# picoexperiment/AutoBub3hs

Hardware: AMD Instinct MI355X
Metric: frames/s end-to-end detect @1280x1024 8-bit (higher is better)
Workload: dtype u8

## Files before the change

### autobub3hs_amd/_lib.py

```python
import ctypes as C
import os
import subprocess

HERE = os.path.dirname(os.path.abspath(__file__))
SO = os.path.join(HERE, "libabub_hip.so")
HEADER = os.path.join(os.path.dirname(HERE), "include", "abub_hip.h")


class Job(C.Structure):
    _fields_ = [("cur", C.c_uint32), ("ref", C.c_uint32), ("model", C.c_uint32), ("out", C.c_uint32)]


class TrigSeg(C.Structure):
    _fields_ = [("hist", C.c_void_p), ("pending", C.c_void_p), ("first", C.c_int32), ("count", C.c_int32)]


class TrigStack(C.Structure):
    _fields_ = [("seg0", C.c_uint32), ("nseg", C.c_uint32), ("F", C.c_int32), ("start", C.c_int32), ("tss", C.c_int32),
                ("first_bad", C.c_int32)]


def build(force=False):
    srcs = [os.path.join(HERE, "csrc", f) for f in os.listdir(os.path.join(HERE, "csrc"))
            if f.endswith((".hip", ".h", ".hpp")) or f == "Makefile"] + [HEADER]
    stale = force or not os.path.exists(SO) or any(os.path.getmtime(s) > os.path.getmtime(SO) for s in srcs)
    if stale:
        subprocess.check_call(["make", "-C", os.path.join(HERE, "csrc"), "-s"])
    return SO


_vp, _i, _sz = C.c_void_p, C.c_int, C.c_size_t
SIGNATURES = {
    "abub_last_error": (C.c_char_p, []),
    "abub_device_count": (_i, []),
    "abub_device_info": (_i, [_i, C.c_char_p, _i, C.POINTER(_i), C.POINTER(C.c_uint64)]),
    "abub_sigma6_dev": (_i, [_vp, _vp, _sz, _vp]),
    "abub_fill_stack_jobs_dev": (_i, [_vp, _i, _i, _i, _i, _i, _i, _vp]),
    "abub_diff_hist_dev": (_i, [_vp, _vp, _vp, _i, _i, _i, _vp, _vp, _i, _vp]),
    "abub_diff_roi_dev": (_i, [_vp, _vp, _vp, _i, _i, _i, _i, _i, _i, _vp, _vp, _vp]),
    "abub_train_dev": (_i, [_vp, _vp, _i, _i, _i, _vp, _vp, _vp]),
    "abub_pair_hist_dev": (_i, [_vp, _vp, _i, _i, _i, _vp, _vp]),
    "abub_posttrig_dev": (_i, [_vp, _vp, _vp, _vp, _i, _i, _i, _vp, _vp, _vp]),
    "abub_fg_compact_dev": (_i, [_vp, _i, _i, _i, _vp, _vp, _i, _vp, _vp]),
    "abub_fast_path": (_i, [_i]),
    "abub_scratch_release": (_i, [_vp]),
    "abub_bound_counts_dev": (_i, [_vp, C.POINTER(C.c_uint32)]),
    "abub_diff_hist_chained_dev": (_i, [_vp, _vp, _vp, _i, _i, _i, _vp, _i, _i, _vp]),
    "abub_diff_hist_chained_store_dev": (_i, [_vp, _vp, _vp, _i, _i, _i, _vp, _vp, _i, _i, _vp]),
    "abub_k2_set_option": (_i, [C.c_char_p, _i]),
    "abub_k2_deferred_ok": (_i, [_i, _i]),
    "abub_k3_set_option": (_i, [C.c_char_p, _i]),
    "abub_k2_pieces_cap": (_sz, [_i, _i, _i]),
    "abub_png_raw_stride": (_sz, [_i, _i]),
    "abub_png_decode_dev": (_i, [_vp, _sz, _vp, _i, _vp, _i, _vp, _i, _i, _i, _vp, _sz, _vp, _sz, _vp, _sz, _vp, _vp]),
    "abub_diff_hist_chained_deferred_dev": (_i, [_vp, _vp, _vp, _i, _i, _i, _vp, _i, _i, _vp, C.c_uint32, _vp, _vp, _vp]),
    "abub_diff_hist_pieces_dev": (_i, [_vp, _vp, _vp, _i, _i, _i, _vp, _vp, _vp, _vp, _vp]),
    "abub_diff_hist_compact_dev": (_i, [_vp, _vp, _vp, _i, _i, _i, _vp, _vp, _vp, _vp, C.c_uint32, _vp, C.c_uint32, _vp]),
    "abub_posttrig_compact_dev": (_i, [_vp, _vp, _vp, _vp, _i, _i, _i, _vp, _vp, _vp, _vp, C.c_uint32, _vp, C.c_uint32, _vp]),
    "abub_pairs_group_dev": (_i, [_vp, _vp, C.c_uint32, _i, _vp, _vp, _vp, _vp, _vp]),
    "abub_pairs_group_hist_dev": (_i, [_vp, _vp, C.c_uint32, _i, _vp, _vp, _vp, _vp, _vp, _vp, _vp]),
    "abub_fg_compact_pairs_dev": (_i, [_vp, _i, _i, _i, _vp, _vp, C.c_uint32, _vp, _vp]),
    "abub_match_ccorr_dev": (_i, [_vp, _i, _i, _vp, _i, _i, _vp, _vp, _vp]),
    "abub_subsat_hist_dev": (_i, [_vp, _vp, _i, _i, _vp, _vp]),
    "abub_match_ccorr_batch_dev": (_i, [_vp, _i, _i, _vp, _i, _vp, _i, _i, _vp, _vp, _vp]),
    "abub_match_best_batch_dev": (_i, [_vp, _i, _i, _vp, _i, _vp, _i, _i, _vp, _vp, _sz, _vp]),
    "abub_match_best_scratch_bytes": (_sz, [_i, _i, _i, _i, _i]),
    "abub_binarize_thr_dev": (_i, [_vp, _vp, _i, _i, _i, _vp, _vp]),
    "abub_label_blobs_dev": (_i, [_vp, _vp, _vp, C.c_uint32, _i, _i, _i, _vp, _vp, _vp, _vp, C.c_uint32, _vp, _vp, _vp, _vp,
                                  C.c_uint32, _vp, _vp, _sz, _vp]),
    "abub_label_blobs_scratch_bytes": (_sz, [_i, _i, _i, C.c_uint32, _i]),
    "abub_trace_contours_dev": (_i, [_vp, _vp, C.c_uint32, _i, _i, _i, _vp, _vp, _vp, _vp, C.c_uint32, _vp, _vp, C.c_uint32,
                                     _vp, _vp, _sz, _vp]),
    "abub_trace_contours_scratch_bytes": (_sz, [_i, C.c_uint32]),
    "abub_trace_contours_limits": (_i, [C.POINTER(_i), C.POINTER(_i)]),
    "abub_trigger_search_dev": (_i, [_vp, _vp, _i, _i, _i, _i, _vp, _sz, _vp, _vp, _i, _vp]),
    "abub_trigger_search_desc_bytes": (_sz, [_i, _i]),
    "abub_trigger_clear_pending_dev": (_i, [_vp, _vp, _sz, _vp]),
    "abub_trigger_search_limits": (_i, [C.POINTER(_i), C.POINTER(_i)]),
    "abub_ctx_create": (_i, [C.POINTER(_vp), _i, _i, _i, _i]),
    "abub_ctx_destroy": (None, [_vp]),
    "abub_ctx_train": (_i, [_vp, C.POINTER(_vp), _i, _vp, _vp]),
    "abub_ctx_pair_hist": (_i, [_vp, _vp, _vp, _vp]),
    "abub_ctx_set_model": (_i, [_vp, _vp, _vp]),
    "abub_ctx_upload_stack": (_i, [_vp, C.POINTER(_vp), _i]),
    "abub_ctx_diff_hist_batch": (_i, [_vp, _i, _i, _i, _vp]),
    "abub_ctx_diff_frame": (_i, [_vp, _i, _i, _vp, _vp]),
    "abub_ctx_diff_frame_roi": (_i, [_vp, _i, _i, _i, _i, _i, _i, _vp, _vp]),
    "abub_ctx_posttrig": (_i, [_vp, _i, _vp, _vp]),
    "abub_ctx_foreground": (_i, [_vp, _i, _vp, _i, C.POINTER(_i)]),
    "abub_ctx_match_template": (_i, [_vp, _i, _vp, _i, _i, _vp, _vp]),
    "abub_ctx_subtract_image": (_i, [_vp, _vp, _vp]),
    "abub_ctx_set_image": (_i, [_vp, _vp]),
    "abub_ctx_fetch_image": (_i, [_vp, _vp]),
}

_lib = None


def lib():
    global _lib
    if _lib is None:
        if not os.path.exists(SO):
            raise RuntimeError(
                f"{SO} is missing: build it with `python -c 'import __graft_entry__ as g; g.build()'` "
                "(there is no CPU fallback for the hot path)")
        try:
            import torch
        except ImportError:
            pass
        L = C.CDLL(SO)
        for name, (res, args) in SIGNATURES.items():
            fn = getattr(L, name)
            fn.restype = res
            fn.argtypes = args
        _lib = L
    return _lib


class AbubError(RuntimeError):
    pass


def check(rc, what=""):
    if rc != 0:
        raise AbubError(f"{what} failed rc={rc}: {lib().abub_last_error().decode(errors='replace')}")
```

### autobub3hs_amd/csrc/abub_dev.hpp

```cpp
#pragma once
#include <hip/hip_runtime.h>
#include <stdint.h>
#include <stdio.h>
#include <stdlib.h>
#include <string.h>

#include <map>
#include <mutex>
#include <utility>

#include "../../include/abub_hip.h"

int abub_set_err_(int code, const char *what, hipError_t e);
static int set_err(int code, const char *what, hipError_t e = hipSuccess) { return abub_set_err_(code, what, e); }
#define HIPCHK(x)                                   \
    do {                                            \
        hipError_t e_ = (x);                        \
        if (e_ != hipSuccess)                       \
            return set_err(ABUB_E_HIP, #x, e_);     \
    } while (0)

typedef unsigned short u16x2 __attribute__((ext_vector_type(2)));
typedef short s16x2 __attribute__((ext_vector_type(2)));

// ... 293 lines not shown
                                                     const uint2 *__restrict__ glist, const uint32_t *__restrict__ gcount,
                                                     uint32_t gcap, const int32_t *__restrict__ cthr, uint32_t *pairs,
                                                     uint32_t pcap, uint32_t *pcount, uint32_t slot_base)
{
    __shared__ uint32_t wtot[4], bbase;
    __shared__ uint32_t lh[4][256];
    uint32_t n = *gcount;
    if (n > gcap)
        n = gcap;
    const size_t P = (size_t)W * H;
    const uint32_t ngroups = (uint32_t)W / 4;
    const int tid = threadIdx.x, lane = tid & 63, wv = tid >> 6;
    uint32_t KE = (n + gridDim.x * 256u - 1u) / (gridDim.x * 256u);
    KE = KE < 1u ? 1u : (KE > SUSL_UB ? (uint32_t)SUSL_UB : KE);
    const uint32_t PER = 256u * KE;
#pragma unroll
    for (int q = 0; q < 4; q++)
        lh[wv][4 * lane + q] = 0;
    for (uint32_t e0 = blockIdx.x * PER; e0 < n; e0 += gridDim.x * PER) {
        uint32_t Ov[SUSL_UB], pix0[SUSL_UB], slot[SUSL_UB];
        int thr[SUSL_UB];
        uint32_t c = 0;
        uint32_t job0 = 0xffffffffu;
        {
            const uint32_t ef = e0 + (uint32_t)(wv * 64) * KE;
            if (ef < n)
                job0 = glist[ef].x;
            job0 = (uint32_t)__builtin_amdgcn_readfirstlane((int)job0);
        }
        uint2 ens[SUSL_UB];
        abub_job jbs[SUSL_UB];
#pragma unroll
        for (int u = 0; u < SUSL_UB; u++) {
            const uint32_t e = e0 + (uint32_t)tid * KE + (uint32_t)u;
            ens[u] = make_uint2(0xffffffffu, 0u);
            if ((uint32_t)u < KE && e < n)
                ens[u] = glist[e];
        }
#pragma unroll
        for (int u = 0; u < SUSL_UB; u++)
            jbs[u] = jobs[ens[u].x != 0xffffffffu ? ens[u].x : 0u];
#pragma unroll
        for (int u = 0; u < SUSL_UB; u++) {
            Ov[u] = 0;
            pix0[u] = 0;
            slot[u] = 0;
            thr[u] = 255;
            const uint2 en = ens[u];
            if (en.x != 0xffffffffu) {
                const abub_job jb = jbs[u];
                const int y = (int)(en.y / ngroups), x0 = (int)(en.y % ngroups) * 4;
                uint32_t packed;
                if (KIND == 2)
                    packed = k2_exact_group(frames + (size_t)jb.cur * P, frames + (size_t)jb.ref * P,
                                            sigma6 + (size_t)jb.model * P, y, x0, W, H);
                else
                    packed = k3_exact_group(frames + (size_t)jb.cur * P, mu + (size_t)jb.model * P,
                                            sigma6 + (size_t)jb.model * P, y, x0, W, H);
                if (COMPACT)
                    thr[u] = compact_thr(cthr, jb.out);
#pragma unroll
                for (int q = 0; q < 4; q++) {
                    const uint32_t v = (packed >> (8 * q)) & 0xffu;
                    if (v) {
                        if (en.x == job0)
                            atomicAdd(&lh[wv][v], 1u);
                        else
                            atomicAdd(&hist[(size_t)jb.out * 256 + v], 1u);
                    }
                    c += COMPACT && (int)v > thr[u];
                }
                if (STORE)
                    *reinterpret_cast<uint32_t *>(img + (size_t)jb.out * P + (size_t)y * W + x0) = packed;
                Ov[u] = packed;
                pix0[u] = (uint32_t)(y * W + x0);
                slot[u] = jb.out + slot_base;
            }
        }
        if (job0 != 0xffffffffu) {
            wave_lds_fence();
            const size_t hb = (size_t)jobs[job0].out * 256;
#pragma unroll
            for (int q = 0; q < 4; q++) {
                const uint32_t cnt = lh[wv][4 * lane + q];
                if (cnt) {
                    atomicAdd(&hist[hb + 4 * lane + q], cnt);
                    lh[wv][4 * lane + q] = 0;
                }
            }
            wave_lds_fence();
        }
        if (COMPACT) {
            uint32_t inc = c;
#pragma unroll
            for (int o = 1; o < 64; o <<= 1) {
                const uint32_t t = __shfl_up(inc, o);
                if (lane >= o)
                    inc += t;
            }
            if (lane == 63)
                wtot[wv] = inc;
            __syncthreads();
            if (tid == 0) {
                const uint32_t tot = wtot[0] + wtot[1] + wtot[2] + wtot[3];
                bbase = tot ? atomicAdd(pcount, tot) : 0u;
            }
            __syncthreads();
            uint32_t pos = bbase + inc - c;
            for (int w = 0; w < wv; w++)
                pos += wtot[w];
#pragma unroll
            for (int u = 0; u < SUSL_UB; u++)
#pragma unroll
                for (int q = 0; q < 4; q++) {
                    const uint32_t v = (Ov[u] >> (8 * q)) & 0xffu;
                    if ((int)v > thr[u]) {
                        if (pos < pcap) {
                            pairs[2 * (size_t)pos] = slot[u] | (v << 24);
                            pairs[2 * (size_t)pos + 1] = pix0[u] + q;
                        }
                        ++pos;
                    }
                }
            __syncthreads();
        }
    }
}

static inline int pick_ndw(int W)
{
    if (W < 4 || (W & 3))
        return 0;
    int nd = W / 4;
    for (int ndw = 1; ndw <= 8; ndw++)
        if (nd % ndw == 0 && nd / ndw <= 64)
            return ndw;
    return 0;
}

void *abub_k2_scratch(hipStream_t st, size_t bytes, std::unique_lock<std::mutex> &hold);
static inline void *k2_scratch(hipStream_t st, size_t bytes, std::unique_lock<std::mutex> &hold) { return abub_k2_scratch(st, bytes, hold); }

struct CompactArgs {
    const int32_t *cthr;
    uint32_t *pairs;
    uint32_t cap;
    uint32_t *count;
    uint32_t slot_base;
    int chain_len = 0, chain_stride = 0;
    uint2 *df_pieces = nullptr;
    uint32_t df_cap = 0;
    uint32_t *df_count = nullptr;
    uint8_t *df_incomplete = nullptr;
};
```

### autobub3hs_amd/csrc/abub_k2.hip

```cpp
#include "abub_dev.hpp"

template <int NDW>
struct K2Acc {
    uint32_t pa0[2 * NDW], pa1[2 * NDW], pa2[2 * NDW];
    uint32_t na0[2 * NDW], na1[2 * NDW], na2[2 * NDW];
};
template <int NDW>
struct K2Row {
    uint32_t hp[2 * NDW], hn[2 * NDW];
};

template <int NDW>
__device__ __forceinline__ void k2_planes(const RowIn<NDW> &in, uint32_t (&Xp)[2 * NDW], uint32_t (&Xn)[2 * NDW])
{
#pragma unroll
    for (int d = 0; d < NDW; d++) {
        uint32_t c0 = widen_lo(in.c[d]), c1 = widen_hi(in.c[d]);
        uint32_t r0 = widen_lo(in.r[d]), r1 = widen_hi(in.r[d]);
        uint32_t s0 = widen_lo(in.s[d]), s1 = widen_hi(in.s[d]);
        Xp[2 * d] = pk_subsat(c0, r0 + s0);
        Xn[2 * d] = pk_subsat(r0, c0 + s0);
        Xp[2 * d + 1] = pk_subsat(c1, r1 + s1);
        Xn[2 * d + 1] = pk_subsat(r1, c1 + s1);
    }
// ... 410 lines not shown
            const uint32_t below = __builtin_amdgcn_mbcnt_hi((uint32_t)(b >> 32), __builtin_amdgcn_mbcnt_lo((uint32_t)b, 0u));
            if (mine[g]) {
#pragma unroll
                for (int q = 0; q < nq; q++)
                    pend[base + (uint32_t)nq * below + q] = code0 + q;
            }
            base += (uint32_t)nq * (uint32_t)__builtin_popcountll(b);
        }
    }
    J.npend = base;
}

template <bool COMPACT>
__device__ __forceinline__ void k2b_tail(const uint32_t *pend, uint32_t npend, const abub_job jb, const uint8_t *__restrict__ frames,
                                         const uint8_t *__restrict__ sigma6, int W, int H, uint32_t *__restrict__ hist,
                                         uint8_t *__restrict__ diff, const Compact &cp, int lane)
{
    if (npend == 0)
        return;
    wave_lds_fence();
    const size_t P = (size_t)W * H;
    const uint32_t ngroups = (uint32_t)W / 4;
    const uint8_t *cur = frames + (size_t)jb.cur * P;
    const uint8_t *ref = frames + (size_t)jb.ref * P;
    const uint8_t *sg = sigma6 + (size_t)jb.model * P;
    const uint32_t nloop = COMPACT ? (npend + 63u) & ~63u : npend;
#pragma unroll 1
    for (uint32_t e = lane; e < nloop; e += 64) {
        uint32_t packed = 0, pix0 = 0;
        if (e < npend) {
            const uint32_t code = pend[e];
            const int y = (int)(code / ngroups), x0 = (int)(code % ngroups) * 4;
            packed = k2_exact_group(cur, ref, sg, y, x0, W, H);
#pragma unroll
            for (int k = 0; k < 4; k++) {
                const uint32_t d = (packed >> (8 * k)) & 0xffu;
                if (d)
                    atomicAdd(&hist[(size_t)jb.out * 256 + d], 1u);
            }
            if (diff)
                *reinterpret_cast<uint32_t *>(diff + (size_t)jb.out * P + (size_t)y * W + x0) = packed;
            pix0 = (uint32_t)(y * W + x0);
        }
        if (COMPACT) {
            uint32_t c = 0;
#pragma unroll
            for (int k = 0; k < 4; k++)
                c += (int)((packed >> (8 * k)) & 0xffu) > cp.thr;
            uint32_t pos = compact_reserve(cp, c);
#pragma unroll
            for (int k = 0; k < 4; k++)
                compact_put(cp, pos, (packed >> (8 * k)) & 0xffu, pix0 + k);
        }
    }
}

template <int NDW, bool COMPACT>
__global__ __launch_bounds__(64) void k2_bound_scan(const uint8_t *__restrict__ frames,
                                                    const uint8_t *__restrict__ sigma6,
                                                    const abub_job *__restrict__ jobs, int W, int H,
                                                    int rows_per_chunk, int nchunks, uint32_t budget,
                                                    uint2 *__restrict__ units, uint32_t *__restrict__ nunits,
                                                    uint32_t *__restrict__ hist, uint8_t *__restrict__ diff,
                                                    const int32_t *__restrict__ cthr, uint32_t *pairs, uint32_t pcap,
                                                    uint32_t *pcount, uint32_t slot_base, SusList gl,
                                                    uint8_t *__restrict__ incomplete)
{
    constexpr int NP = 2 * NDW;
    __shared__ uint32_t pend[K2B_PEND];
    const int lane = threadIdx.x;
    const int unit = blockIdx.x;
    const int job = unit / nchunks;
    const int chunk = unit - job * nchunks;
    const abub_job jb = jobs[job];
    const size_t P = (size_t)W * H;
    const uint8_t *cur = frames + (size_t)jb.cur * P;
    const uint8_t *ref = frames + (size_t)jb.ref * P;
    const uint8_t *sg = sigma6 + (size_t)jb.model * P;
    const int nl = W / (4 * NDW);
    const bool active = lane < nl;
    const int xoff = active ? lane * 4 * NDW : 0;
    const int y0 = chunk * rows_per_chunk;
    int y1 = y0 + rows_per_chunk;
    if (y1 > H)
        y1 = H;
    const int T = y1 - y0 + 4;
    const uint32_t ngroups = (uint32_t)W / 4;

    ScanMap<NDW, false> map;
    map.init(W);
    K2BoundJob<NDW> J;
#pragma unroll
    for (int g = 0; g < K2BoundJob<NDW>::NG; g++)
#pragma unroll
        for (int q = 0; q < 4; q++)
            J.P[q][0][g] = J.P[q][K2BoundJob<NDW>::CASCADE ? 1 : 0][g] = 0;
    J.npend = J.hot = 0;
    J.jidx = (uint32_t)job;
    J.handover = -1;

    RowIn<NDW> ring[2];
    k2_load_row<NDW>(ring[0], cur, ref, sg, reflect101(y0 - 2, H), W, xoff);
    const int Tpad = (T + 1) & ~1;
    for (int t = 0; t < Tpad && J.handover < 0; t += 2) {
#pragma unroll
        for (int u = 0; u < 2; u++) {
            const int tt = t + u;
            int tn = tt + 1 < T ? tt + 1 : T - 1;
            k2_load_row<NDW>(ring[u ^ 1], cur, ref, sg, reflect101(y0 - 2 + tn, H), W, xoff);
            if (J.handover < 0) {
                uint32_t Xp[NP], Xn[NP];
                k2_planes<NDW>(ring[u], Xp, Xn);
                uint32_t m[NDW];
#pragma unroll
                for (int g = 0; g < NDW; g++)
                    m[g] = (Xp[2 * g] + Xn[2 * g]) + (Xp[2 * g + 1] + Xn[2 * g + 1]);
                k2b_row<NDW, false>(J, u, m, tt >= 4 && tt < T, y0 + tt - 4, map, lane, ngroups, budget, pend, gl);
            }
        }
    }
    if (J.handover >= 0)
        k2b_hand_over(units, nunits, (uint32_t)unit, J.handover, y1, lane, incomplete, (uint32_t)job);
    if (J.npend) {
        wave_lds_fence();
        uint32_t gb = 0;
        if (sus_reserve(J.npend, gl.list, gl.count, gl.cap, gb, lane)) {
            sus_copy_out(pend, J.npend, J.jidx, gl.list, gb, lane);
            return;
        }
    }
    Compact cp;
    cp.pairs = COMPACT ? pairs : nullptr;
    cp.count = pcount;
    cp.cap = pcap;
    cp.slot = jb.out + slot_base;
    cp.thr = COMPACT ? compact_thr(cthr, jb.out) : 255;
    k2b_tail<COMPACT>(pend, J.npend, jb, frames, sigma6, W, H, hist, diff, cp, lane);
}

#define K2C_MAXW 8
#ifndef K2C_DEFAULT_WG
#define K2C_DEFAULT_WG 1
#endif
#ifndef K2C_DEFAULT_SYNC
#define K2C_DEFAULT_SYNC 0
#endif
template <int NDW, int K, bool SPLIT, int PF = 1>
__global__ __launch_bounds__(64 * K2C_MAXW) void k2_sad_chain(const uint8_t *__restrict__ frames,
                                                   const uint8_t *__restrict__ sigma6,
                                                   const abub_job *__restrict__ jobs, int L, int S, int nwgs, int W,
                                                   int H, int rows_per_chunk, int nchunks, uint32_t budget,
                                                   uint2 *__restrict__ units, uint32_t *__restrict__ nunits,
                                                   uint32_t *__restrict__ hist, uint8_t *__restrict__ diff, SusList gl,
                                                   int syncD, uint8_t *__restrict__ incomplete)
{
    using Job = K2BoundJob<NDW, false, true>;
    extern __shared__ uint32_t k2c_lds[];
    const int NW = (int)(blockDim.x >> 6);
    const int lane = (int)(threadIdx.x & 63u);
    const int wave = __builtin_amdgcn_readfirstlane((int)(threadIdx.x >> 6));
    uint32_t(*pend)[K2B_PEND] = reinterpret_cast<uint32_t(*)[K2B_PEND]>(k2c_lds + (size_t)wave * K * K2B_PEND);
    const int progBase = NW * K * K2B_PEND;
#define K2C_PUBLISH(V)                                                                                         \
    {                                                                                                          \
        if (NW > 1 && lane == 0)                                                                               \
            __hip_atomic_store(&k2c_lds[progBase + wave], (uint32_t)(V), __ATOMIC_RELAXED, __HIP_MEMORY_SCOPE_WORKGROUP); \
    }
    const int chunk = blockIdx.x % nchunks;
    const int bs = blockIdx.x / nchunks;
    const int blk = bs / nwgs;
    int wg = bs - blk * nwgs;
    int r = 0, nr = 0, ns = 0;
    for (r = 0; r < S; r++) {
        nr = (L - r + S - 1) / S;
        ns = (nr + K - 1) / K;
        const int nw = (ns + NW - 1) / NW;
        if (wg < nw)
            break;
        wg -= nw;
    }
    const int slot = wg * NW + wave;
    if (r >= S || slot >= ns) {
        K2C_PUBLISH(0x7fffffff);
        return;
    }
    const int k = nr - slot * K < K ? nr - slot * K : K;
    Job J[K];
    abub_job jb[K];
    const uint32_t jidx0 = (uint32_t)(blk * L + r + S * slot * K);
#pragma unroll
    for (int t = 0; t < K; t++)
        jb[t] = jobs[jidx0 + (uint32_t)(S * (t < k ? t : k - 1))];
    const int y0 = chunk * rows_per_chunk;
    int y1 = y0 + rows_per_chunk;
    if (y1 > H)
        y1 = H;
    bool chained = true;
#pragma unroll
    for (int t = 1; t < K; t++)
        if (t < k && (jb[t].ref != jb[t - 1].cur || jb[t].model != jb[0].model))
            chained = false;
    if (!chained) {
#pragma unroll
        for (int t = 0; t < K; t++)
            if (t < k)
                k2b_hand_over(units, nunits, (jidx0 + (uint32_t)(S * t)) * (uint32_t)nchunks + (uint32_t)chunk, y0, y1, lane, incomplete,
                              jidx0 + (uint32_t)(S * t));
        K2C_PUBLISH(0x7fffffff);
        return;
    }
    const size_t P = (size_t)W * H;
    const uint8_t *fp[K + 1];
    fp[0] = frames + (size_t)jb[0].ref * P;
#pragma unroll
    for (int t = 0; t < K; t++)
        fp[t + 1] = frames + (size_t)jb[t].cur * P;
    const uint8_t *sg = sigma6 + (size_t)jb[0].model * P;
    ScanMap<NDW, SPLIT> map;
    map.init(W);
    const int T = y1 - y0 + 4;
    const uint32_t ngroups = (uint32_t)W / 4;
#pragma unroll
    for (int t = 0; t < K; t++) {
#pragma unroll
        for (int g = 0; g < Job::NG; g++)
#pragma unroll
            for (int q = 0; q < 4; q++)
                J[t].P[q][0][g] = 0;
#pragma unroll
        for (int g = 0; g < Job::NG; g++)
            J[t].Mp[0][g] = J[t].Mp[1][g] = 0;
        J[t].npend = J[t].hot = 0;
        J[t].handover = t < k ? -1 : 0x7fffffff;
    }
    constexpr int RING = PF + 1, U = (RING % 2 == 0) ? RING : 2 * RING;
    uint32_t raw[RING][K + 2][NDW];
#define K2C_LOAD(SL, Y)                                                                       \
    {                                                                                         \
        const size_t o_ = (size_t)(Y) * W;                                                    \
        _Pragma("unroll") for (int f = 0; f <= K; f++) map.load(raw[SL][f], fp[f] + o_, lane); \
        map.load(raw[SL][K + 1], sg + o_, lane);                                              \
    }
#pragma unroll
    for (int q = 0; q < PF; q++) {
        const int tq = q < T ? q : T - 1;
        K2C_LOAD(q, reflect101(y0 - 2 + tq, H));
    }
    const int Tpad = (T + U - 1) / U * U;
    for (int t0 = 0; t0 < Tpad; t0 += U) {
        bool all_done = true;
#pragma unroll
        for (int t = 0; t < K; t++)
            all_done = all_done && J[t].handover >= 0;
        if (all_done)
            break;
        if (NW > 1) {
            K2C_PUBLISH(t0);
            if (syncD > 0) {
                for (;;) {
                    int mn = 0x7fffffff;
                    for (int w = 0; w < NW; w++) {
                        const int pw_ = (int)__hip_atomic_load(&k2c_lds[progBase + w], __ATOMIC_RELAXED, __HIP_MEMORY_SCOPE_WORKGROUP);
                        mn = pw_ < mn ? pw_ : mn;
                    }
                    if (t0 <= __builtin_amdgcn_readfirstlane(mn) + syncD)
                        break;
                    __builtin_amdgcn_s_sleep(8);
                }
            }
        }
#pragma unroll
        for (int uu = 0; uu < U; uu++) {
            const int tt = t0 + uu;
            const int tn = tt + PF < T ? tt + PF : T - 1;
            K2C_LOAD((uu + PF) % RING, reflect101(y0 - 2 + tn, H));
            const int u = uu % RING;
            const int par = uu & 1;
            const bool emit = tt >= 4 && tt < T;
            const int y = y0 + tt - 4;
            uint32_t s8[2 * NDW];
#pragma unroll
            for (int d = 0; d < NDW; d++) {
                s8[2 * d] = widen8_lo(raw[u][K + 1][d]);
                s8[2 * d + 1] = widen8_hi(raw[u][K + 1][d]);
            }
#pragma unroll
            for (int h = 1; h <= K; h += 2) {
                const bool ja = J[h - 1].handover < 0, jc = h < K && J[h < K ? h : K - 1].handover < 0;
                if (!(ja || jc))
                    continue;
                uint32_t HI[NDW], LO[NDW], nS[NDW];
#pragma unroll
                for (int d = 0; d < NDW; d++) {
                    const uint32_t r0 = widen8_lo(raw[u][h][d]), r1 = widen8_hi(raw[u][h][d]);
                    HI[d] = pack8(pk_addsat(r0, s8[2 * d]), pk_addsat(r1, s8[2 * d + 1]));
                    LO[d] = pack8(pk_subsat(r0, s8[2 * d]), pk_subsat(r1, s8[2 * d + 1]));
                    nS[d] = 0u - __builtin_amdgcn_sad_u8(HI[d], LO[d], 0u);
                }
#pragma unroll
                for (int q = 0; q < 2; q++) {
                    const int t = h - 1 + q, fc = q ? h + 1 : h - 1;
                    if (t >= K)
                        continue;
                    if (J[t].handover < 0) {
                        uint32_t m[NDW];
#pragma unroll
                        for (int d = 0; d < NDW; d++)
                            m[d] = __builtin_amdgcn_sad_u8(raw[u][fc][d], LO[d], __builtin_amdgcn_sad_u8(raw[u][fc][d], HI[d], nS[d]));
// ... 85 lines not shown
        for (int i = 0; i < 5; i++) {
            uint32_t rowacc = 0;
#pragma unroll
            for (int j = 0; j < 5; j++)
                rowacc += w[j] * tile[(ly + i) * (G_TW + 4) + lx + j];
            acc += w[i] * rowacc;
        }
        acc += 0x00800080u;
        int a = (acc >> 8) & 0xff, b = acc >> 24;
        int d = a > b ? a - b : b - a;
        if (diff)
            diff[(size_t)jb.out * P + (size_t)(y + ry) * W + (x + rx)] = (uint8_t)d;
        if (d)
            atomicAdd(&lh[d], 1u);
    }
    __syncthreads();
    uint32_t v = lh[tid];
    if (v && tid)
        atomicAdd(&hist[(size_t)jb.out * 256 + tid], v);
}

template <int NDW, int PF>
static void launch_k2_rows_pf(const uint8_t *frames, const uint8_t *sigma6, const abub_job *jobs,
                              int njobs, int W, int H, int R, int nchunks, uint32_t *hist, uint8_t *diff,
                              const CompactArgs &ca, hipStream_t st)
{
    dim3 grid((unsigned)njobs * nchunks), block(64);
#define K2_LAUNCH(ST, CO)                                                                                        \
    hipLaunchKernelGGL((k2_rows<NDW, ST, PF, CO>), grid, block, 0, st, frames, sigma6, jobs, W, H, R, nchunks, \
                       hist, diff, ca.cthr, ca.pairs, ca.cap, ca.count, ca.slot_base, nullptr, nullptr)
    if (ca.cthr) {
        if (diff)
            K2_LAUNCH(true, true);
        else
            K2_LAUNCH(false, true);
    } else {
        if (diff)
            K2_LAUNCH(true, false);
        else
            K2_LAUNCH(false, false);
    }
#undef K2_LAUNCH
}

struct K2Options {
    int bound = 1;
    int chain = -1;
    int budget = 512;
    int pf = 1;
    int scanpf = -1;
    int split = 1;
    int list = 0;
    int wg = -1;
    int sync = -1;
    int chunks = 0;
    bool loaded = false;
};
static K2Options g_k2opt;
static std::mutex g_k2optMu;
static K2Options k2_options()
{
    std::lock_guard<std::mutex> lock(g_k2optMu);
    if (!g_k2opt.loaded) {
        if (const char *e = getenv("ABUB_K2_BOUND"))
            g_k2opt.bound = atoi(e);
        if (const char *e = getenv("ABUB_K2_CHAIN"))
            g_k2opt.chain = atoi(e);
        if (const char *e = getenv("ABUB_K2_BUDGET"))
            if (atoi(e) > 0)
                g_k2opt.budget = atoi(e);
        if (const char *e = getenv("ABUB_K2_PF"))
            g_k2opt.pf = atoi(e);
        if (const char *e = getenv("ABUB_K2_SPLIT"))
            g_k2opt.split = atoi(e);
        if (const char *e = getenv("ABUB_K2_LIST"))
            g_k2opt.list = atoi(e);
        if (const char *e = getenv("ABUB_K2_WG"))
            g_k2opt.wg = atoi(e);
        if (const char *e = getenv("ABUB_K2_SYNC"))
            g_k2opt.sync = atoi(e);
        if (const char *e = getenv("ABUB_K2_SCANPF"))
            g_k2opt.scanpf = atoi(e);
        if (const char *e = getenv("ABUB_K2_CHUNKS"))
            if (atoi(e) >= 0 && atoi(e) <= K_MAX_CHUNKS)
                g_k2opt.chunks = atoi(e);
        g_k2opt.loaded = true;
    }
    return g_k2opt;
}

extern "C" int abub_k2_set_option(const char *name, int value)
{
    if (!name)
        return set_err(ABUB_E_INVALID, "abub_k2_set_option: null name");
    (void)k2_options();
    std::lock_guard<std::mutex> lock(g_k2optMu);
    if (!strcmp(name, "bound"))
        g_k2opt.bound = value;
    else if (!strcmp(name, "chain"))
        g_k2opt.chain = value;
    else if (!strcmp(name, "budget") && value > 0)
        g_k2opt.budget = value;
    else if (!strcmp(name, "pf"))
        g_k2opt.pf = value;
    else if (!strcmp(name, "split"))
        g_k2opt.split = value;
    else if (!strcmp(name, "list"))
        g_k2opt.list = value;
    else if (!strcmp(name, "wg"))
        g_k2opt.wg = value;
    else if (!strcmp(name, "sync"))
        g_k2opt.sync = value;
    else if (!strcmp(name, "scanpf"))
        g_k2opt.scanpf = value;
    else if (!strcmp(name, "chunks") && value >= 0 && value <= K_MAX_CHUNKS)
        g_k2opt.chunks = value;
    else
        return set_err(ABUB_E_INVALID, "abub_k2_set_option: unknown option or bad value");
    return ABUB_OK;
}

template <int NDW>
static int launch_k2_rows(const uint8_t *frames, const uint8_t *sigma6, const abub_job *jobs,
                           int njobs, int W, int H, int R, int nchunks, uint32_t *hist, uint8_t *diff,
                           const CompactArgs &ca, hipStream_t st)
{
    const K2Options opt = k2_options();
    if (opt.bound && (size_t)H * (size_t)(W / 4) < ((size_t)1 << 32) && H < 65536) {
        if (diff)
            HIPCHK(hipMemsetAsync(diff, 0, (size_t)njobs * (size_t)W * (size_t)H, st));
        const size_t nunits = (size_t)njobs * nchunks;
        const uint32_t budget = (uint32_t)(opt.budget < K2B_PEND ? opt.budget : K2B_PEND);
        const size_t unitCap = nunits * (size_t)((R + K2B_SUB - 1) / K2B_SUB);
        const size_t unitBytes = (unitCap * sizeof(uint2) + 255) & ~(size_t)255;
        size_t gcap = (size_t)njobs * 1024;
        gcap = gcap < ((size_t)1 << 16) ? ((size_t)1 << 16) : (gcap > ((size_t)1 << 24) ? ((size_t)1 << 24) : gcap);
        if (!opt.list)
            gcap = 0;
        const size_t bytes = 256 + unitBytes + gcap * sizeof(uint2) + 256;
        std::unique_lock<std::mutex> hold;
        uint8_t *scr = (uint8_t *)k2_scratch(st, bytes, hold);
        if (!scr)
            return set_err(ABUB_E_HIP, "abub_diff_hist_dev: scratch allocation failed");
        uint32_t *counters = (uint32_t *)scr;
        uint2 *units = (uint2 *)(scr + 256);
        uint32_t *npieces = counters;
        const bool deferred = ca.df_pieces != nullptr;
        if (deferred) {
            if (diff || ca.cthr || !ca.df_count || !ca.df_incomplete || (size_t)ca.df_cap < unitCap)
                return set_err(ABUB_E_INVALID, "deferred pieces: trigger-only launches with a list of abub_k2_pieces_cap() entries");
            units = ca.df_pieces;
            npieces = ca.df_count;
            HIPCHK(hipMemsetAsync(npieces, 0, sizeof(uint32_t), st));
            HIPCHK(hipMemsetAsync(ca.df_incomplete, 0, (size_t)njobs, st));
        }
        SusList gl;
        gl.list = gcap ? (uint2 *)(scr + 256 + unitBytes) : nullptr;
        gl.count = counters + 32;
        gl.cap = (uint32_t)gcap;
        const unsigned tgrid = (unsigned)((gcap + 256 * SUSL_UB - 1) / (256 * SUSL_UB) < 2048 ? (gcap + 256 * SUSL_UB - 1) / (256 * SUSL_UB) : 2048);
        HIPCHK(hipMemsetAsync(counters, 0, 256, st));
        const int L = ca.chain_len, S = ca.chain_stride;
        const int chainK = opt.chain < 0 ? 4 : opt.chain;
        if (chainK >= 2 && L > 0 && S > 0 && S <= 8 && njobs % L == 0 && !ca.cthr) {
            const int Kc = chainK >= 3 ? 4 : 2;
            const int NW = opt.wg < 0 ? K2C_DEFAULT_WG : (opt.wg < 1 ? 1 : (opt.wg > K2C_MAXW ? K2C_MAXW : opt.wg));
            int nwgs = 0;
            for (int r = 0; r < S; r++) {
                const int nr = (L - r + S - 1) / S;
                const int ns = nr > 0 ? (nr + Kc - 1) / Kc : 0;
                nwgs += (ns + NW - 1) / NW;
            }
            const dim3 grid((unsigned)((size_t)(njobs / L) * nwgs * nchunks));
            const size_t ldsBytes = ((size_t)NW * Kc * K2B_PEND + 64) * sizeof(uint32_t);
            const int syncD = opt.sync < 0 ? K2C_DEFAULT_SYNC : opt.sync;
            constexpr bool CAN_SPLIT = NDW >= 5 && NDW <= 7;
            const bool split = CAN_SPLIT && opt.split;
            const bool pf2 = NDW == 5 && split && Kc == 4 && (opt.scanpf < 0 || opt.scanpf == 2);
#define K2C_ARGS frames, sigma6, jobs, L, S, nwgs, W, H, R, nchunks, budget, units, npieces, hist, diff, gl, syncD, ca.df_incomplete
#define K2C_LAUNCH_SP(KK, SP, PFD) \
    hipLaunchKernelGGL((k2_sad_chain<NDW, KK, SP, PFD>), grid, dim3(64 * NW), ldsBytes, st, K2C_ARGS)
#define K2C_LAUNCH(KK)                                                                                              \
    if (split) {                                                                                                    \
        K2C_LAUNCH_SP(KK, CAN_SPLIT, 1);                                                                            \
    } else {                                                                                                        \
        K2C_LAUNCH_SP(KK, false, 1);                                                                                \
    }
            if (pf2) {
                if constexpr (NDW == 5)
                    K2C_LAUNCH_SP(4, true, 2);
            } else if (Kc == 4) {
                K2C_LAUNCH(4);
            } else {
                K2C_LAUNCH(2);
            }
#undef K2C_LAUNCH_SP
#undef K2C_ARGS
#undef K2C_LAUNCH
        } else {
#define K2S_LAUNCH(CO)                                                                                              \
    hipLaunchKernelGGL((k2_bound_scan<NDW, CO>), dim3((unsigned)nunits), dim3(64), 0, st, frames, sigma6, jobs, W, H, \
                       R, nchunks, budget, units, npieces, hist, diff, ca.cthr, ca.pairs, ca.cap, ca.count,         \
                       ca.slot_base, gl, ca.df_incomplete)
            if (ca.cthr) {
                K2S_LAUNCH(true);
            } else {
                K2S_LAUNCH(false);
            }
#undef K2S_LAUNCH
        }
        if (gl.list) {
#define K2T_LAUNCH(CO, ST)                                                                                          \
    hipLaunchKernelGGL((sus_tail_list<2, CO, ST>), dim3(tgrid), dim3(256), 0, st, frames, (const uint8_t *)nullptr,  \
                       sigma6, jobs, W, H, hist, diff, gl.list, gl.count, gl.cap, ca.cthr, ca.pairs, ca.cap, ca.count, \
                       ca.slot_base)
            if (ca.cthr) {
                if (diff) {
                    K2T_LAUNCH(true, true);
                } else {
                    K2T_LAUNCH(true, false);
                }
            } else {
                if (diff) {
                    K2T_LAUNCH(false, true);
                } else {
                    K2T_LAUNCH(false, false);
                }
            }
#undef K2T_LAUNCH
        }
        if (deferred)
            return ABUB_OK;
        const unsigned g3 = (unsigned)(unitCap < 4096 ? unitCap : 4096);
#define K2R_LAUNCH(ST, CO)                                                                                          \
    hipLaunchKernelGGL((k2_rows<NDW, ST, 1, CO>), dim3(g3), dim3(64), 0, st, frames, sigma6, jobs, W, H, R, nchunks, \
                       hist, diff, ca.cthr, ca.pairs, ca.cap, ca.count, ca.slot_base, units, counters)
        if (ca.cthr) {
            if (diff)
                K2R_LAUNCH(true, true);
            else
                K2R_LAUNCH(false, true);
        } else {
            if (diff)
                K2R_LAUNCH(true, false);
            else
                K2R_LAUNCH(false, false);
        }
#undef K2R_LAUNCH
        return ABUB_OK;
    }
    if (ca.df_pieces)
        return set_err(ABUB_E_INVALID, "deferred pieces need the bound-and-verify pass (option \"bound\" on)");
    if (opt.pf == 2)
        launch_k2_rows_pf<NDW, 2>(frames, sigma6, jobs, njobs, W, H, R, nchunks, hist, diff, ca, st);
    else
        launch_k2_rows_pf<NDW, 1>(frames, sigma6, jobs, njobs, W, H, R, nchunks, hist, diff, ca, st);
    return ABUB_OK;
}

static int k2_auto_rows(int njobs, int H)
{
    int nch = 8;
    if ((long long)njobs * nch < 8192)
        nch = (8192 + njobs - 1) / njobs;
    const int chunks = k2_options().chunks;
    if (chunks > 0)
        nch = chunks;
    nch = (nch + 7) / 8 * 8;
    int R = (H + nch - 1) / nch;
    if (R < 16)
        R = 16;
    return R;
}

static int diff_hist_impl(const uint8_t *frames, const uint8_t *sigma6, const abub_job *jobs, int njobs,
                          int W, int H, uint32_t *hist, uint8_t *diff, int rows_per_chunk,
                          const CompactArgs &ca, void *stream)
{
    if (!frames || !sigma6 || !jobs || !hist || W <= 0 || H <= 0 || njobs < 0 || rows_per_chunk < 0)
        return set_err(ABUB_E_INVALID, "abub_diff_hist_dev: bad arguments");
    if (njobs == 0)
        return ABUB_OK;
    hipStream_t st = (hipStream_t)stream;
    HIPCHK(hipMemsetAsync(hist, 0, (size_t)njobs * 256 * sizeof(uint32_t), st));
    int ndw = pick_ndw(W);
    if (ndw) {
        const int R = rows_per_chunk ? rows_per_chunk : k2_auto_rows(njobs, H);
        int nchunks = (H + R - 1) / R;
        int rc = ABUB_OK;
        switch (ndw) {
        case 1: rc = launch_k2_rows<1>(frames, sigma6, jobs, njobs, W, H, R, nchunks, hist, diff, ca, st); break;
        case 2: rc = launch_k2_rows<2>(frames, sigma6, jobs, njobs, W, H, R, nchunks, hist, diff, ca, st); break;
        case 3: rc = launch_k2_rows<3>(frames, sigma6, jobs, njobs, W, H, R, nchunks, hist, diff, ca, st); break;
        case 4: rc = launch_k2_rows<4>(frames, sigma6, jobs, njobs, W, H, R, nchunks, hist, diff, ca, st); break;
        case 5: rc = launch_k2_rows<5>(frames, sigma6, jobs, njobs, W, H, R, nchunks, hist, diff, ca, st); break;
        case 6: rc = launch_k2_rows<6>(frames, sigma6, jobs, njobs, W, H, R, nchunks, hist, diff, ca, st); break;
        case 7: rc = launch_k2_rows<7>(frames, sigma6, jobs, njobs, W, H, R, nchunks, hist, diff, ca, st); break;
        default: rc = launch_k2_rows<8>(frames, sigma6, jobs, njobs, W, H, R, nchunks, hist, diff, ca, st); break;
        }
        if (rc != ABUB_OK)
            return rc;
    } else {
        if (ca.cthr)
            return set_err(ABUB_E_INVALID, "fused compaction needs the fast path (W % 4 == 0, W <= 2048)");
        abub_job dummy = {0, 0, 0, 0};
        dim3 grid((W + G_TW - 1) / G_TW, (H + G_TH - 1) / G_TH, njobs), block(256);
        if (grid.z > 65535)
            return set_err(ABUB_E_INVALID, "abub_diff_hist_dev: too many jobs for the generic kernel");
        hipLaunchKernelGGL(k2_generic, grid, block, 0, st, frames, sigma6, jobs, dummy, 0, W, H, 0, 0,
                           W, H, hist, diff);
    }
    HIPCHK(hipGetLastError());
    hipLaunchKernelGGL(k_hist_bin0, dim3(njobs), dim3(64), 0, st, hist, (uint32_t)((size_t)W * H));
    HIPCHK(hipGetLastError());
    return ABUB_OK;
}

extern "C" int abub_diff_hist_dev(const uint8_t *frames, const uint8_t *sigma6, const abub_job *jobs,
                                  int njobs, int W, int H, uint32_t *hist, uint8_t *diff,
                                  int rows_per_chunk, void *stream)
{
    CompactArgs ca = {nullptr, nullptr, 0, nullptr, 0};
    return diff_hist_impl(frames, sigma6, jobs, njobs, W, H, hist, diff, rows_per_chunk, ca, stream);
}

extern "C" int abub_diff_hist_chained_dev(const uint8_t *frames, const uint8_t *sigma6, const abub_job *jobs,
                                          int njobs, int W, int H, uint32_t *hist, int chain_len, int chain_stride,
                                          void *stream)
{
    if (chain_len < 0 || chain_stride < 0)
        return set_err(ABUB_E_INVALID, "abub_diff_hist_chained_dev: bad arguments");
    CompactArgs ca = {nullptr, nullptr, 0, nullptr, 0};
    ca.chain_len = chain_len;
    ca.chain_stride = chain_stride;
    return diff_hist_impl(frames, sigma6, jobs, njobs, W, H, hist, nullptr, 0, ca, stream);
}

extern "C" int abub_diff_hist_chained_store_dev(const uint8_t *frames, const uint8_t *sigma6, const abub_job *jobs,
                                                int njobs, int W, int H, uint32_t *hist, uint8_t *diff, int chain_len,
                                                int chain_stride, void *stream)
{
    if (chain_len < 0 || chain_stride < 0 || !diff)
        return set_err(ABUB_E_INVALID, "abub_diff_hist_chained_store_dev: bad arguments");
    CompactArgs ca = {nullptr, nullptr, 0, nullptr, 0};
    ca.chain_len = chain_len;
    ca.chain_stride = chain_stride;
    return diff_hist_impl(frames, sigma6, jobs, njobs, W, H, hist, diff, 0, ca, stream);
}

extern "C" size_t abub_k2_pieces_cap(int njobs, int W, int H)
{
    if (njobs <= 0 || H <= 0)
        return 0;
    const int R = k2_auto_rows(njobs, H), nchunks = (H + R - 1) / R;
    return (size_t)njobs * nchunks * (size_t)((R + K2B_SUB - 1) / K2B_SUB);
}

extern "C" int abub_k2_deferred_ok(int W, int H)
{
    return W > 0 && H > 0 && H < 65536 && (size_t)H * (size_t)(W / 4) < ((size_t)1 << 32) && pick_ndw(W) != 0 &&
           k2_options().bound != 0;
}

extern "C" int abub_diff_hist_chained_deferred_dev(const uint8_t *frames, const uint8_t *sigma6, const abub_job *jobs, int njobs,
                                                   int W, int H, uint32_t *hist, int chain_len, int chain_stride,
                                                   void *pieces, uint32_t pieces_cap, uint32_t *npieces,
                                                   uint8_t *incomplete, void *stream)
{
    if (chain_len < 0 || chain_stride < 0 || !pieces || !npieces || !incomplete || !pick_ndw(W) || !k2_options().bound)
        return set_err(ABUB_E_INVALID, "abub_diff_hist_chained_deferred_dev: bad arguments (or no bound-and-verify pass for this width)");
    CompactArgs ca = {nullptr, nullptr, 0, nullptr, 0};
    ca.chain_len = chain_len;
    ca.chain_stride = chain_stride;
    ca.df_pieces = (uint2 *)pieces;
    ca.df_cap = pieces_cap;
    ca.df_count = npieces;
    ca.df_incomplete = incomplete;
    return diff_hist_impl(frames, sigma6, jobs, njobs, W, H, hist, nullptr, 0, ca, stream);
}

template <int NDW>
static void launch_pieces(const uint8_t *frames, const uint8_t *sigma6, const abub_job *jobs, int W, int H, int R, int nchunks,
                          uint32_t *hist, const uint2 *pieces, const uint32_t *npieces, const uint8_t *want, unsigned grid,
                          hipStream_t st)
{
    hipLaunchKernelGGL((k2_rows<NDW, false, 1, false>), dim3(grid), dim3(64), 0, st, frames, sigma6, jobs, W, H, R, nchunks, hist,
                       (uint8_t *)nullptr, (const int32_t *)nullptr, (uint32_t *)nullptr, 0u, (uint32_t *)nullptr, 0u, pieces,
                       npieces, want);
}

extern "C" int abub_diff_hist_pieces_dev(const uint8_t *frames, const uint8_t *sigma6, const abub_job *jobs, int njobs, int W,
                                         int H, uint32_t *hist, const void *pieces_, const uint32_t *npieces,
                                         const uint8_t *want, void *stream)
{
    const uint2 *pieces = (const uint2 *)pieces_;
    if (!frames || !sigma6 || !jobs || !hist || !pieces || !npieces || !want || njobs <= 0 || W <= 0 || H <= 0)
        return set_err(ABUB_E_INVALID, "abub_diff_hist_pieces_dev: bad arguments");
    const int ndw = pick_ndw(W);
    if (!ndw)
        return set_err(ABUB_E_INVALID, "abub_diff_hist_pieces_dev: no fast path for this width");
    hipStream_t st = (hipStream_t)stream;
    const int R = k2_auto_rows(njobs, H), nchunks = (H + R - 1) / R;
    const size_t cap = abub_k2_pieces_cap(njobs, W, H);
    const unsigned grid = (unsigned)(cap < 4096 ? cap : 4096);
    switch (ndw) {
    case 1: launch_pieces<1>(frames, sigma6, jobs, W, H, R, nchunks, hist, pieces, npieces, want, grid, st); break;
    case 2: launch_pieces<2>(frames, sigma6, jobs, W, H, R, nchunks, hist, pieces, npieces, want, grid, st); break;
    case 3: launch_pieces<3>(frames, sigma6, jobs, W, H, R, nchunks, hist, pieces, npieces, want, grid, st); break;
    case 4: launch_pieces<4>(frames, sigma6, jobs, W, H, R, nchunks, hist, pieces, npieces, want, grid, st); break;
    case 5: launch_pieces<5>(frames, sigma6, jobs, W, H, R, nchunks, hist, pieces, npieces, want, grid, st); break;
    case 6: launch_pieces<6>(frames, sigma6, jobs, W, H, R, nchunks, hist, pieces, npieces, want, grid, st); break;
    case 7: launch_pieces<7>(frames, sigma6, jobs, W, H, R, nchunks, hist, pieces, npieces, want, grid, st); break;
    default: launch_pieces<8>(frames, sigma6, jobs, W, H, R, nchunks, hist, pieces, npieces, want, grid, st); break;
    }
    HIPCHK(hipGetLastError());
    hipLaunchKernelGGL(k_hist_bin0, dim3(njobs), dim3(64), 0, st, hist, (uint32_t)((size_t)W * H), want, jobs);
    HIPCHK(hipGetLastError());
    return ABUB_OK;
}

extern "C" int abub_fast_path(int W) { return pick_ndw(W) != 0; }

extern "C" int abub_diff_hist_compact_dev(const uint8_t *frames, const uint8_t *sigma6, const abub_job *jobs,
                                          int njobs, int W, int H, uint32_t *hist, uint8_t *diff,
                                          const int32_t *cthr, uint32_t *pairs, uint32_t cap,
                                          uint32_t *count, uint32_t slot_base, void *stream)
{
    if (!cthr || !pairs || !count || cap == 0)
        return set_err(ABUB_E_INVALID, "abub_diff_hist_compact_dev: bad arguments");
    CompactArgs ca = {cthr, pairs, cap, count, slot_base};
    return diff_hist_impl(frames, sigma6, jobs, njobs, W, H, hist, diff, 0, ca, stream);
}

extern "C" int abub_diff_roi_dev(const uint8_t *cur, const uint8_t *ref, const uint8_t *sigma6, int W,
                                 int H, int rx, int ry, int rw, int rh, uint8_t *diff, uint32_t *hist,
                                 void *stream)
{
    if (!cur || !ref || !sigma6 || !diff || !hist || W <= 0 || H <= 0 || rx < 0 || ry < 0 ||
        rw < 0 || rh < 0 || rx + rw > W || ry + rh > H)
        return set_err(ABUB_E_INVALID, "abub_diff_roi_dev: bad arguments");
    hipStream_t st = (hipStream_t)stream;
    size_t P = (size_t)W * H;
    HIPCHK(hipMemsetAsync(diff, 0, P, st));
    HIPCHK(hipMemsetAsync(hist, 0, 256 * sizeof(uint32_t), st));
    if (rw > 0 && rh > 0) {
        abub_job jb = {0, 0, 0, 0};
        dim3 grid((rw + G_TW - 1) / G_TW, (rh + G_TH - 1) / G_TH, 1), block(256);
        ptrdiff_t dref = ref - cur;
        if (dref % (ptrdiff_t)P != 0 || dref < 0)
            return set_err(ABUB_E_INVALID, "abub_diff_roi_dev: ref must follow cur in the same slab at a multiple of W*H");
        jb.ref = (uint32_t)(dref / (ptrdiff_t)P);
        hipLaunchKernelGGL(k2_generic, grid, block, 0, st, cur, sigma6, (const abub_job *)nullptr, jb, 1,
                           W, H, rx, ry, rw, rh, hist, diff);
        HIPCHK(hipGetLastError());
    }
    hipLaunchKernelGGL(k_hist_bin0, dim3(1), dim3(64), 0, st, hist, (uint32_t)P);
    HIPCHK(hipGetLastError());
    return ABUB_OK;
}
```

### autobub3hs_amd/csrc/abub_trigger.hip

```cpp
#include "abub_dev.hpp"

#define TRIG_MAXF 512
#define TRIG_MAXSEG 32
#define TRIG_BC 64
#define TRIG_PITCH 65

namespace {

struct TrigShared {
    uint32_t tile[64 * TRIG_PITCH];
    long long baseS[256], baseS2[256];
    int prevM[256];
    long long prevQ[256];
    const uint32_t *row[TRIG_MAXF];
    double sig[3][TRIG_MAXF];
    int8_t loc[TRIG_MAXF];
    uint8_t rd[TRIG_MAXF];
};

__device__ __forceinline__ double trig_term(double sig, float count, long long S, long long S2, int n0)
{
    const double mean = (double)S / n0;
    const double sd = sqrt((double)S2 / n0 - mean * mean);
    if ((double)count != mean || sd > 0)
        sig += ((double)count - mean) / sd;
    if (sig < 0)
        sig = 0;
    return sig;
}

__device__ __forceinline__ long long wave_scan_incl(long long v, int lane)
{
#pragma unroll
    for (int d = 1; d < 64; d <<= 1) {
        const long long o = __shfl_up(v, d, 64);
        if (lane >= d)
            v += o;
    }
    return v;
}

template <int PASS>
__device__ __forceinline__ void trig_pass(TrigShared &sh, int nf, int P, int tss, int n, float thr, int lane)
{
    for (int b = lane; b < 256; b += 64) {
        sh.baseS[b] = 0;
        sh.baseS2[b] = 0;
        sh.prevM[b] = 0;
        sh.prevQ[b] = 0;
    }
    __syncthreads();
    for (int base = 1; base < nf; base += 64) {
        const int j = base + lane;
        const bool active = j < nf;
        bool need1 = false, need2 = false;
        if (PASS == 1) {
            if (active && j - 1 >= 2 && j - 1 != n - 1)
                need1 = (float)sh.sig[0][j - 1] > thr;
            if (active && j - 2 >= 2)
                need2 = (float)sh.sig[0][j - 2] > thr;
        }
        int rem = P, firstOver = -1, lastbin = 0;
        double s0 = 0, s1 = 0, s2 = 0;
        bool done = !active || rem <= 0;
        int visited = 0;
        for (int cb = 0; cb < 256 / TRIG_BC; ++cb) {
            if (__ballot(!done) == 0)
                break;
            __syncthreads();
#pragma unroll 8
            for (int r = 0; r < 64; ++r) {
                const uint32_t *p = base + r < nf ? sh.row[base + r] : nullptr;
                sh.tile[r * TRIG_PITCH + lane] = p ? p[cb * TRIG_BC + lane] : 0u;
            }
            __syncthreads();
            for (int bb = 0; bb < TRIG_BC; ++bb) {
                if (__ballot(!done) == 0)
                    break;
                const int bin = cb * TRIG_BC + bb;
                visited = bin + 1;
                const bool live = !done;
                const float count = live ? (float)sh.tile[lane * TRIG_PITCH + bb] : 0.f;
                const int ci = (int)count;
                const long long m = ci, q = (long long)(int)((unsigned)ci * (unsigned)ci);
                const long long S = sh.baseS[bin] + wave_scan_incl(m, lane);
                const long long S2 = sh.baseS2[bin] + wave_scan_incl(q, lane);
                long long mp = __shfl_up(m, 1, 64), qp = __shfl_up(q, 1, 64);
                if (lane == 0) {
                    mp = sh.prevM[bin];
                    qp = sh.prevQ[bin];
                }
                if (lane == 63) {
                    sh.baseS[bin] = S;
                    sh.baseS2[bin] = S2;
                    sh.prevM[bin] = ci;
                    sh.prevQ[bin] = q;
                }
                if (live) {
                    if (bin > 1) {
                        if (PASS == 0)
                            s0 = trig_term(s0, count, S, S2, j);
                        else {
                            if (need1)
                                s1 = trig_term(s1, count, S - m, S2 - q, j - 1);
                            if (need2)
                                s2 = trig_term(s2, count, S - m - mp, S2 - q - qp, j - 2);
                        }
                    }
                    if (PASS == 0) {
                        if (s0 > 3.5 && firstOver < 0)
                            firstOver = bin;
                        lastbin = bin;
                    }
                    rem = (int)((float)rem - count);
                    done = rem <= 0;
                }
            }
        }
        for (int b = visited + lane; b < 256; b += 64) {
            sh.prevM[b] = 0;
            sh.prevQ[b] = 0;
        }
        if (active) {
            if (PASS == 0) {
                int t = max(firstOver - 1, lastbin - 1);
                if (t < 2)
                    t = 2;
                if (t > 3 || tss < 6)
                    t = 3;
                sh.sig[0][j] = s0;
                sh.loc[j] = (int8_t)t;
            } else {
                sh.sig[1][j] = s1;
                sh.sig[2][j] = s2;
            }
        }
        __syncthreads();
    }
}

__global__ __launch_bounds__(64) void k_trigger_search(const abub_trig_stack *__restrict__ stacks,
                                                       const abub_trig_seg *__restrict__ segs, int nsegs, int P,
                                                       abub_trig_result *__restrict__ out, double *__restrict__ sig_main,
                                                       int sig_pitch)
{
    __shared__ TrigShared sh;
    const int lane = threadIdx.x;
    const abub_trig_stack sd = stacks[blockIdx.x];
    const int n = min(max(sd.F, 0), TRIG_MAXF);
    abub_trig_result res;
    res.state = ABUB_TRIG_DONE;
    res.status = -3;
    res.trig = 0;
    res.loc_thres = -1;
    res.need_frame = 0;
    res.evaluated = 0;
    res.sig = 0.f;
    res.reserved = 0;
    if (n < 5) {
        res.status = -9;
        if (lane == 0)
            out[blockIdx.x] = res;
        return;
    }
    const int start = max(sd.start, 1), tss = sd.tss;
    const int firstBad = min(max(sd.first_bad, 0), n);
    float thr = 3.5f;
    if (tss < 6)
        thr = (float)((double)thr * (5 / 3.5));

    for (int j = lane; j < n; j += 64) {
        sh.rd[j] = 1;
        sh.row[j] = nullptr;
    }
    __syncthreads();
    const uint32_t seg1 = min(sd.seg0 + min(sd.nseg, (uint32_t)TRIG_MAXSEG), (uint32_t)nsegs);
    for (uint32_t k = sd.seg0; k < seg1; ++k) {
        const abub_trig_seg sg = segs[k];
        for (int q = lane; q < sg.count; q += 64) {
            const int j = sg.first + q;
            if (j < 1 || j >= n || j >= firstBad || !sg.hist)
                continue;
            const bool pend = sg.pending && sg.pending[q];
            sh.rd[j] = pend ? 2 : 0;
            sh.row[j] = pend ? nullptr : sg.hist + (size_t)q * 256;
        }
    }
    __syncthreads();
    int u = n;
    for (int b0 = 1; b0 < n && u == n; b0 += 64) {
        const int j = b0 + lane;
        const unsigned long long bad = __ballot(j < n && j < firstBad && sh.rd[j] != 0);
        if (bad)
            u = b0 + __ffsll((long long)bad) - 1;
    }
    const int nf = min(u, max(firstBad, 1));

    trig_pass<0>(sh, nf, P, tss, n, thr, lane);
    bool any = false;
    for (int b0 = 2; b0 < nf; b0 += 64) {
        const int i = b0 + lane;
        any = any || __ballot(i < nf && i != n - 1 && (float)sh.sig[0][i] > thr) != 0;
    }
    if (any)
        trig_pass<1>(sh, nf, P, tss, n, thr, lane);
    if (lane != 0)
        return;

    auto needs = [&](int frame) {
        res.state = sh.rd[frame] == 2 ? ABUB_TRIG_NEED_FINAL : ABUB_TRIG_NEED_FRAMES;
        res.status = -3;
        res.trig = 0;
        res.loc_thres = -1;
        res.need_frame = frame;
        res.evaluated = 0;
        res.sig = 0.f;
    };
    double *sm = sig_main ? sig_main + (size_t)blockIdx.x * sig_pitch : nullptr;
    bool stop = false;
    if (u < n && u < start) {
        needs(u);
        stop = true;
    }
    for (int i = start; i < n && !stop; ++i) {
        if (i >= firstBad) {
            res.status = -9;
            break;
        }
        if (i >= u) {
            needs(i);
            break;
        }
        float single = (float)sh.sig[0][i];
        res.loc_thres = sh.loc[i];
        res.sig = single;
        ++res.evaluated;
        if (single > thr && i >= 2 && i != n - 1) {
            double maxSoFar = single;
            for (int ii = 1; ii <= 2 && ii + i < n; ++ii) {
                if (i + ii >= firstBad) {
                    res.state = ABUB_TRIG_BAD_LOOKAHEAD;
                    stop = true;
                    break;
                }
                if (i + ii >= u) {
                    needs(i + ii);
                    stop = true;
                    break;
                }
                single = (float)sh.sig[ii][i + ii];
                if (single / (thr / 3.5 * 5) + single / maxSoFar <= 3)
                    break;
                else if (ii == 2) {
                    res.status = 0;
                    res.trig = i;
                }
                if (single > maxSoFar)
                    maxSoFar = single;
            }
            if (res.status == 0)
                break;
        }
    }
    for (int i = start; sm && i < start + res.evaluated && i < sig_pitch; ++i)
        sm[i] = sh.sig[0][i];
    out[blockIdx.x] = res;
}

__global__ __launch_bounds__(256) void k_trigger_clear_pending(uint8_t *__restrict__ pending, const uint8_t *__restrict__ done, size_t n)
{
    const size_t j = (size_t)blockIdx.x * 256 + threadIdx.x;
    if (j < n && done[j])
        pending[j] = 0;
}

}

extern "C" int abub_trigger_clear_pending_dev(uint8_t *pending, const uint8_t *done, size_t n, void *stream)
{
    if (!pending || !done || n > 0x7fffffffu * (size_t)256)
        return set_err(ABUB_E_INVALID, "abub_trigger_clear_pending_dev: bad arguments");
    if (n == 0)
        return ABUB_OK;
    hipLaunchKernelGGL(k_trigger_clear_pending, dim3((unsigned)((n + 255) / 256)), dim3(256), 0, (hipStream_t)stream, pending, done, n);
    HIPCHK(hipGetLastError());
    return ABUB_OK;
}

extern "C" int abub_trigger_search_limits(int *max_frames, int *max_segs)
{
    if (max_frames)
        *max_frames = TRIG_MAXF;
    if (max_segs)
        *max_segs = TRIG_MAXSEG;
    return ABUB_OK;
}

extern "C" size_t abub_trigger_search_desc_bytes(int nstacks, int nsegs)
{
    if (nstacks <= 0 || nsegs < 0)
        return 0;
    return (((size_t)nstacks * sizeof(abub_trig_stack) + 255) & ~(size_t)255) + (size_t)nsegs * sizeof(abub_trig_seg) + 256;
}

extern "C" int abub_trigger_search_dev(const abub_trig_stack *stacks, const abub_trig_seg *segs, int nstacks, int nsegs, int W,
                                       int H, void *desc, size_t desc_bytes, abub_trig_result *out, double *sig_main,
                                       int sig_pitch, void *stream)
{
    static_assert(sizeof(abub_trig_result) == 32 && sizeof(abub_trig_stack) == 24 && sizeof(abub_trig_seg) == 24, "record layout");
    if (!stacks || !out || !desc || nstacks < 0 || nsegs < 0 || (nsegs > 0 && !segs) || W <= 0 || H <= 0 ||
        (size_t)W * H > 0x7fffffffu || (sig_main && sig_pitch <= 0))
        return set_err(ABUB_E_INVALID, "abub_trigger_search_dev: bad arguments");
    if (nstacks == 0)
        return ABUB_OK;
    if (((uintptr_t)desc & 255) || desc_bytes < abub_trigger_search_desc_bytes(nstacks, nsegs))
        return set_err(ABUB_E_INVALID, "abub_trigger_search_dev: descriptor scratch too small or not 256-byte aligned");
    for (int s = 0; s < nstacks; ++s) {
        const abub_trig_stack &t = stacks[s];
        if (t.F < 0 || t.F > TRIG_MAXF)
            return set_err(ABUB_E_INVALID, "abub_trigger_search_dev: a stack has more frames than abub_trigger_search_limits allows");
        if (t.nseg > TRIG_MAXSEG)
            return set_err(ABUB_E_INVALID, "abub_trigger_search_dev: a stack has more segments than abub_trigger_search_limits allows");
        if ((uint64_t)t.seg0 + t.nseg > (uint64_t)nsegs || (sig_main && t.F > sig_pitch))
            return set_err(ABUB_E_INVALID, "abub_trigger_search_dev: bad stack descriptor");
        int end = 0;
        for (uint32_t k = t.seg0; k < t.seg0 + t.nseg; ++k) {
            const abub_trig_seg &g = segs[k];
            if (g.count < 0 || g.first < end || g.count > 0x7fffffff - g.first || (g.count > 0 && !g.hist))
                return set_err(ABUB_E_INVALID, "abub_trigger_search_dev: segments must be ascending and must not overlap");
            end = g.first + g.count;
        }
    }
    hipStream_t st = (hipStream_t)stream;
    abub_trig_stack *dst = (abub_trig_stack *)desc;
    abub_trig_seg *dsg = (abub_trig_seg *)((uint8_t *)desc + (((size_t)nstacks * sizeof(abub_trig_stack) + 255) & ~(size_t)255));
    HIPCHK(hipMemcpyAsync(dst, stacks, (size_t)nstacks * sizeof(abub_trig_stack), hipMemcpyHostToDevice, st));
    if (nsegs > 0)
        HIPCHK(hipMemcpyAsync(dsg, segs, (size_t)nsegs * sizeof(abub_trig_seg), hipMemcpyHostToDevice, st));
    hipLaunchKernelGGL(k_trigger_search, dim3(nstacks), dim3(64), 0, st, dst, dsg, nsegs, (int)((size_t)W * H), out, sig_main,
                       sig_pitch);
    HIPCHK(hipGetLastError());
    return ABUB_OK;
}
```

### autobub3hs_amd/hip.py

```python
import torch

from . import _lib


def _ptr(t):
    return None if t is None else t.data_ptr()


def _stream():
    return torch.cuda.current_stream().cuda_stream


def _need_cuda(*ts):
    for t in ts:
        if t is not None and not t.is_cuda:
            raise _lib.AbubError("device-pointer launcher called with a CPU tensor (no CPU fallback)")
        if t is not None and not t.is_contiguous():
            raise _lib.AbubError("tensor must be contiguous")


def sigma6(sigma):
    _need_cuda(sigma)
    out = torch.empty_like(sigma)
    _lib.check(_lib.lib().abub_sigma6_dev(_ptr(sigma), _ptr(out), sigma.numel(), _stream()), "abub_sigma6_dev")
    return out


def stack_jobs(nstacks, F, first, count, ref_offset, nmodels, device):
    jobs = torch.empty((nstacks * count, 4), dtype=torch.int32, device=device)
    _lib.check(_lib.lib().abub_fill_stack_jobs_dev(_ptr(jobs), nstacks, F, first, count, ref_offset,
                                                   nmodels, _stream()), "abub_fill_stack_jobs_dev")
    return jobs


def make_jobs(rows, device):
    return torch.tensor(list(rows), dtype=torch.int64).to(torch.int32).reshape(-1, 4).to(device)


def diff_hist(frames, sigma6_, jobs, W, H, store=False, rows_per_chunk=0, hist=None, diff=None, chain=None):
    _need_cuda(frames, sigma6_, jobs)
    n = jobs.shape[0]
    if hist is None:
        hist = torch.empty((n, 256), dtype=torch.int32, device=frames.device)
    if store and diff is None:
        diff = torch.empty((n, H, W), dtype=torch.uint8, device=frames.device)
    if chain is not None:
        assert rows_per_chunk == 0
        if store:
            _lib.check(_lib.lib().abub_diff_hist_chained_store_dev(_ptr(frames), _ptr(sigma6_), _ptr(jobs), n, W, H,
                                                                   _ptr(hist), _ptr(diff), int(chain[0]), int(chain[1]),
                                                                   _stream()), "abub_diff_hist_chained_store_dev")
            return hist, diff
        _lib.check(_lib.lib().abub_diff_hist_chained_dev(_ptr(frames), _ptr(sigma6_), _ptr(jobs), n, W, H, _ptr(hist),
                                                         int(chain[0]), int(chain[1]), _stream()),
                   "abub_diff_hist_chained_dev")
        return hist, None
    _lib.check(_lib.lib().abub_diff_hist_dev(_ptr(frames), _ptr(sigma6_), _ptr(jobs), n, W, H, _ptr(hist),
                                             _ptr(diff) if store else None, rows_per_chunk, _stream()),
               "abub_diff_hist_dev")
    return hist, (diff if store else None)


def diff_hist_deferred(frames, sigma6_, jobs, W, H, chain):
    _need_cuda(frames, sigma6_, jobs)
    n = jobs.shape[0]
    hist = torch.empty((n, 256), dtype=torch.int32, device=frames.device)
    cap = int(_lib.lib().abub_k2_pieces_cap(n, W, H))
    pieces = torch.empty((max(cap, 1), 2), dtype=torch.int32, device=frames.device)
    npieces = torch.zeros((1,), dtype=torch.int32, device=frames.device)
    incomplete = torch.empty((n,), dtype=torch.uint8, device=frames.device)
    _lib.check(_lib.lib().abub_diff_hist_chained_deferred_dev(_ptr(frames), _ptr(sigma6_), _ptr(jobs), n, W, H, _ptr(hist),
                                                              int(chain[0]), int(chain[1]), _ptr(pieces), cap, _ptr(npieces),
                                                              _ptr(incomplete), _stream()),
               "abub_diff_hist_chained_deferred_dev")
    return hist, (pieces, npieces, incomplete)


def diff_hist_pieces(frames, sigma6_, jobs, W, H, hist, state, want):
    _need_cuda(frames, sigma6_, jobs, want)
    pieces, npieces, _ = state
    _lib.check(_lib.lib().abub_diff_hist_pieces_dev(_ptr(frames), _ptr(sigma6_), _ptr(jobs), jobs.shape[0], W, H, _ptr(hist),
                                                    _ptr(pieces), _ptr(npieces), _ptr(want), _stream()),
               "abub_diff_hist_pieces_dev")
    return hist


def k2_set_option(name, value):
    _lib.check(_lib.lib().abub_k2_set_option(name.encode(), int(value)), "abub_k2_set_option")


def k3_set_option(name, value):
    _lib.check(_lib.lib().abub_k3_set_option(name.encode(), int(value)), "abub_k3_set_option")


def bound_counts(stream=None):
    import ctypes as C

    st = torch.cuda.current_stream().cuda_stream if stream is None else stream
    out = (C.c_uint32 * 2)()
    _lib.check(_lib.lib().abub_bound_counts_dev(st, out), "abub_bound_counts_dev")
    return int(out[0]), int(out[1])


def diff_roi(slab, cur, ref, sigma6_, W, H, roi):
    _need_cuda(slab, sigma6_)
    rx, ry, rw, rh = roi
    diff = torch.empty((H, W), dtype=torch.uint8, device=slab.device)
    hist = torch.empty((256,), dtype=torch.int32, device=slab.device)
    P = W * H
    base = slab.data_ptr()
    _lib.check(_lib.lib().abub_diff_roi_dev(base + cur * P, base + ref * P, _ptr(sigma6_), W, H, rx, ry, rw, rh,
                                            _ptr(diff), _ptr(hist), _stream()), "abub_diff_roi_dev")
    return diff, hist


def train(frames, W, H, idx=None):
    _need_cuda(frames, idx)
    N = frames.shape[0] if idx is None else idx.numel()
    mu = torch.empty((H, W), dtype=torch.uint8, device=frames.device)
    sg = torch.empty((H, W), dtype=torch.uint8, device=frames.device)
    _lib.check(_lib.lib().abub_train_dev(_ptr(frames), _ptr(idx), N, W, H, _ptr(mu), _ptr(sg), _stream()),
               "abub_train_dev")
    return mu, sg


def pair_hist(frames, pairs, W, H):
    _need_cuda(frames, pairs)
    n = pairs.shape[0]
    hist = torch.empty((n, 256), dtype=torch.int32, device=frames.device)
    _lib.check(_lib.lib().abub_pair_hist_dev(_ptr(frames), _ptr(pairs), n, W, H, _ptr(hist), _stream()),
               "abub_pair_hist_dev")
    return hist


def posttrig(frames, mu, sigma6_, jobs, W, H, store=True):
    _need_cuda(frames, mu, sigma6_, jobs)
    n = jobs.shape[0]
    hist = torch.empty((n, 256), dtype=torch.int32, device=frames.device)
    img = torch.empty((n, H, W), dtype=torch.uint8, device=frames.device) if store else None
    _lib.check(_lib.lib().abub_posttrig_dev(_ptr(frames), _ptr(mu), _ptr(sigma6_), _ptr(jobs), n, W, H,
                                            _ptr(hist), _ptr(img), _stream()), "abub_posttrig_dev")
    return hist, img


def fg_compact(img, thr, cap):
    _need_cuda(img, thr)
    n, H, W = img.shape
    idx = torch.empty((n, cap), dtype=torch.int32, device=img.device)
    cnt = torch.empty((n,), dtype=torch.int32, device=img.device)
    _lib.check(_lib.lib().abub_fg_compact_dev(_ptr(img), n, W, H, _ptr(thr), _ptr(idx), cap, _ptr(cnt),
                                              _stream()), "abub_fg_compact_dev")
    return idx, cnt



def binarize_thr(hist, tozero, W, H):
    _need_cuda(hist, tozero)
    n = tozero.numel()
    thr = torch.empty((n,), dtype=torch.int32, device=hist.device)
    _lib.check(_lib.lib().abub_binarize_thr_dev(_ptr(hist), _ptr(tozero), n, W, H, _ptr(thr), _stream()),
               "abub_binarize_thr_dev")
    return thr


def label_blobs(offsets, idx, val, thr, min_box_area, W, H, cap=None, comp=True, in_cap=None):
    _need_cuda(offsets, idx, val, thr, min_box_area)
    n = thr.numel()
    dev = idx.device
    in_cap = int(idx.numel()) if in_cap is None else int(in_cap)
    cap = max(in_cap, 1) if cap is None else int(cap)
    L = _lib.lib()
    need = int(L.abub_label_blobs_scratch_bytes(n, W, H, in_cap, 1 if comp else 0))
    scratch = torch.empty((max(need, 1),), dtype=torch.uint8, device=dev)
    out = {"kept_off": torch.empty((n + 1,), dtype=torch.int32, device=dev),
           "kept_idx": torch.empty((cap,), dtype=torch.int32, device=dev),
           "ncomp": torch.empty((n,), dtype=torch.int32, device=dev),
           "nkept_comp": torch.empty((n,), dtype=torch.int32, device=dev),
           "comp_off": torch.empty((n + 1,), dtype=torch.int32, device=dev),
           "comp": torch.empty((cap, 6), dtype=torch.int32, device=dev) if comp else None,
           "stats": torch.empty((4,), dtype=torch.int32, device=dev)}
    _lib.check(L.abub_label_blobs_dev(_ptr(offsets), _ptr(idx), _ptr(val), in_cap, n, W, H, _ptr(thr), _ptr(min_box_area),
                                      _ptr(out["kept_off"]), _ptr(out["kept_idx"]), cap, _ptr(out["ncomp"]),
                                      _ptr(out["nkept_comp"]), _ptr(out["comp_off"]), _ptr(out["comp"]), cap if comp else 0,
                                      _ptr(out["stats"]), _ptr(scratch), scratch.numel(), _stream()),
               "abub_label_blobs_dev")
    return out

def trace_contours_limits():
    import ctypes as C
    mp, mc = C.c_int(0), C.c_int(0)
    _lib.check(_lib.lib().abub_trace_contours_limits(C.byref(mp), C.byref(mc)), "abub_trace_contours_limits")
    return mp.value, mc.value


def trace_contours(kept_off, kept_idx, W, H, cont_cap=None, pts_cap=None, in_cap=None):
    _need_cuda(kept_off, kept_idx)
    n = kept_off.numel() - 1
    dev = kept_idx.device
    in_cap = int(kept_idx.numel()) if in_cap is None else int(in_cap)
    cont_cap = max(in_cap, 1) if cont_cap is None else int(cont_cap)
    pts_cap = max(4 * in_cap, 1) if pts_cap is None else int(pts_cap)
    L = _lib.lib()
    need = int(L.abub_trace_contours_scratch_bytes(n, in_cap))
    scratch = torch.empty((max(need, 1),), dtype=torch.uint8, device=dev)
    out = {"status": torch.empty((n,), dtype=torch.int32, device=dev),
           "ncont": torch.empty((n,), dtype=torch.int32, device=dev),
           "cont_off": torch.empty((n + 1,), dtype=torch.int32, device=dev),
           "cont_npts": torch.empty((cont_cap,), dtype=torch.int32, device=dev),
           "pt_off": torch.empty((n + 1,), dtype=torch.int32, device=dev),
           "pts": torch.empty((pts_cap,), dtype=torch.int32, device=dev),
           "stats": torch.empty((4,), dtype=torch.int32, device=dev)}
    _lib.check(L.abub_trace_contours_dev(_ptr(kept_off), _ptr(kept_idx), in_cap, n, W, H, _ptr(out["status"]),
                                         _ptr(out["ncont"]), _ptr(out["cont_off"]), _ptr(out["cont_npts"]), cont_cap,
                                         _ptr(out["pt_off"]), _ptr(out["pts"]), pts_cap, _ptr(out["stats"]), _ptr(scratch),
                                         scratch.numel(), _stream()), "abub_trace_contours_dev")
    return out

def trigger_search_limits():
    import ctypes as C
    mf, ms = C.c_int(0), C.c_int(0)
    _lib.check(_lib.lib().abub_trigger_search_limits(C.byref(mf), C.byref(ms)), "abub_trigger_search_limits")
    return mf.value, ms.value


TRIG_DONE, TRIG_NEED_FRAMES, TRIG_NEED_FINAL, TRIG_BAD_LOOKAHEAD = 0, 1, 2, 3


def trigger_search(stacks, W, H, sig_main=True):
    import ctypes as C
    import struct
    n = len(stacks)
    nseg = sum(len(s["segs"]) for s in stacks)
    st = (_lib.TrigStack * max(n, 1))()
    sg = (_lib.TrigSeg * max(nseg, 1))()
    k = 0
    dev = None
    for i, s in enumerate(stacks):
        st[i].seg0, st[i].nseg, st[i].F, st[i].tss = k, len(s["segs"]), s["F"], s["tss"]
        st[i].start, st[i].first_bad = s.get("start", 1), s.get("first_bad", s["F"])
        for first, hist, pending in s["segs"]:
            _need_cuda(hist, pending)
            dev = hist.device
            sg[k].hist, sg[k].pending, sg[k].first, sg[k].count = _ptr(hist), _ptr(pending), first, hist.shape[0]
            k += 1
    if dev is None:
        dev = torch.device("cuda")
    L = _lib.lib()
    nbytes = int(L.abub_trigger_search_desc_bytes(n, nseg))
    desc = torch.empty((max(nbytes, 1),), dtype=torch.uint8, device=dev)
    out = torch.zeros((max(n, 1), 8), dtype=torch.int32, device=dev)
    pitch = max([s["F"] for s in stacks] + [1])
    sm = torch.full((max(n, 1), pitch), float("nan"), dtype=torch.float64, device=dev) if sig_main else None
    _lib.check(L.abub_trigger_search_dev(C.addressof(st), C.addressof(sg), n, nseg, W, H, _ptr(desc), desc.numel(), _ptr(out),
                                         _ptr(sm), pitch, _stream()), "abub_trigger_search_dev")
    rows = out.cpu().numpy()
    names = ("state", "status", "trig", "loc_thres", "need_frame", "evaluated")
    res = []
    for i in range(n):
        r = {k_: int(rows[i, j]) for j, k_ in enumerate(names)}
        r["sig"] = struct.unpack("<f", struct.pack("<i", int(rows[i, 6])))[0]
        res.append(r)
    return res, (sm[:n] if sig_main else None)


def png_parse(data, W, H):
    import struct
    if len(data) < 33 or data[:8] != b"\x89PNG\r\n\x1a\n":
        return None
    o, segs, pal, hdr, end = 8, [], None, None, False
    while not end and o + 12 <= len(data):
        ln, = struct.unpack(">I", data[o:o + 4])
        typ = data[o + 4:o + 8]
        if o + 12 + ln > len(data):
            return None
        if typ == b"IHDR" and ln >= 13:
            hdr = struct.unpack(">IIBBBBB", data[o + 8:o + 21])
        elif typ == b"PLTE":
            pal = data[o + 8:o + 8 + ln]
        elif typ == b"IDAT":
            segs.append((o + 8, ln))
        elif typ == b"IEND":
            end = True
        o += 12 + ln
    if hdr is None or not segs or hdr[0] != W or hdr[1] != H or hdr[2] != 8 or hdr[3] not in (0, 3) or hdr[6] != 0:
        return None
    lut = None
    if hdr[3] == 3:
        n = min(len(pal or b"") // 3, 256)
        lut = bytes(((pal[3 * i] * 9797 + pal[3 * i + 1] * 19234 + pal[3 * i + 2] * 3737 + 16384) >> 15) & 255 if i < n else 0
                    for i in range(256))
    return segs, lut


def png_decode(files, W, H, device="cuda:0"):
    import numpy as np
    n = len(files)
    frames_np = np.zeros((max(n, 1), 8), dtype=np.uint32)
    segs, luts, blob, zoff = [], [], bytearray(), 0
    status_pre = np.zeros(n, dtype=np.int32)
    P = W * H
    for i, data in enumerate(files):
        parsed = png_parse(data, W, H)
        base = len(blob)
        if parsed is None:
            status_pre[i] = -1
            frames_np[i] = (len(segs), 0, zoff, 0, 0xFFFFFFFF, 0, (i * P) & 0xFFFFFFFF, (i * P) >> 32)
            zoff += 16
            continue
        sg, lut = parsed
        zlen = sum(l for _, l in sg)
        li = 0xFFFFFFFF
        if lut is not None:
            li = len(luts)
            luts.append(lut)
        frames_np[i] = (len(segs), len(sg), zoff, zlen, li, 0, (i * P) & 0xFFFFFFFF, (i * P) >> 32)
        segs += [(base + o, l) for o, l in sg]
        blob += data
        blob += b"\0" * ((-len(blob)) % 4)
        zoff += ((zlen + 15) & ~15) + 16
    blob += b"\0" * 8
    dev = torch.device(device)
    d_files = torch.frombuffer(bytearray(blob), dtype=torch.uint8).to(dev)
    d_frames = torch.from_numpy(frames_np.view(np.int32).copy()).to(dev)
    d_segs = torch.tensor(segs if segs else [(0, 0)], dtype=torch.int64).to(torch.int32).to(dev) if True else None
    d_luts = torch.frombuffer(bytearray(b"".join(luts) if luts else bytes(256)), dtype=torch.uint8).to(dev)
    stride = int(_lib.lib().abub_png_raw_stride(W, H))
    d_z = torch.empty((max(zoff, 16),), dtype=torch.uint8, device=dev)
    d_raw = torch.empty((max(n, 1) * stride,), dtype=torch.uint8, device=dev)
    out = torch.zeros((max(n, 1), H, W), dtype=torch.uint8, device=dev)
    status = torch.full((max(n, 1),), 99, dtype=torch.int32, device=dev)
    _lib.check(_lib.lib().abub_png_decode_dev(_ptr(d_files), d_files.numel(), _ptr(d_frames), n, _ptr(d_segs), len(segs),
                                              _ptr(d_luts), len(luts), W, H, _ptr(d_z), d_z.numel(), _ptr(d_raw), d_raw.numel(),
                                              _ptr(out), out.numel(), _ptr(status), _stream()), "abub_png_decode_dev")
    st = status.cpu().numpy()[:n].copy()
    st[status_pre != 0] = -1
    return out[:n], st


def match_terms(frames, frame_idx, tmpl):
    _need_cuda(frames, frame_idx, tmpl)
    H, W = frames.shape[-2:]
    th, tw = tmpl.shape
    n = frame_idx.numel()
    num = torch.empty((n, H - th + 1, W - tw + 1), dtype=torch.int64, device=frames.device)
    w2 = torch.empty_like(num)
    _lib.check(_lib.lib().abub_match_ccorr_batch_dev(_ptr(frames), W, H, _ptr(frame_idx), n, _ptr(tmpl), tw, th,
                                                     _ptr(num), _ptr(w2), _stream()), "abub_match_ccorr_batch_dev")
    return num, w2


def match_best(frames, frame_idx, tmpl, scratch=None):
    _need_cuda(frames, frame_idx, tmpl)
    H, W = frames.shape[-2:]
    th, tw = tmpl.shape
    n = frame_idx.numel()
    need = _lib.lib().abub_match_best_scratch_bytes(W, H, tw, th, n)
    if scratch is None:
        scratch = torch.empty(max(need, 1), dtype=torch.uint8, device=frames.device)
    out = torch.empty((n, 2), dtype=torch.float32, device=frames.device)
    _lib.check(_lib.lib().abub_match_best_batch_dev(_ptr(frames), W, H, _ptr(frame_idx), n, _ptr(tmpl), tw, th,
                                                    _ptr(out), _ptr(scratch), scratch.numel(), _stream()),
               "abub_match_best_batch_dev")
    return out
```

### autobub3hs_amd/host.py

```python
import ctypes as C
import os
import subprocess

import numpy as np

HERE = os.path.dirname(os.path.abspath(__file__))
SO = os.path.join(HERE, "libabub_host.so")

_u8p = C.POINTER(C.c_uint8)
_u32p = C.POINTER(C.c_uint32)
_u64p = C.POINTER(C.c_uint64)
_ip = C.POINTER(C.c_int)
_fp = C.POINTER(C.c_float)
_dp = C.POINTER(C.c_double)
_vp, _i, _s = C.c_void_p, C.c_int, C.c_char_p
SIGNATURES = {
    "abh_run_new": (_vp, []),
    "abh_run_open": (_vp, [_i, _s, _s, _s]),
    "abh_run_free": (None, [_vp]),
    "abh_run_events": (_s, [_vp]),
    "abh_run_frames": (_s, [_vp, _s, _i]),
    "abh_run_image": (_i, [_vp, _s, _s, _u8p, _i, _ip, _ip]),
    "abh_run_add_event": (_i, [_vp, _s, _i, _u8p, _i, _i, _i, _u8p]),
    "abh_train": (_i, [_vp, _i, _ip, _ip, _u8p, _u8p]),
    "abh_train_device": (_i, [_vp, _i, _ip, _ip, _u8p, _u8p, _i, _dp]),
    "abh_set_model": (_i, [_vp, _i, _u8p, _u8p, _i, _i, _i]),
    "abh_probe_frame_stats": (_i, [_vp, _s, _i, _u8p, _i, _i, _i, _dp]),
    "abh_run_batched": (_i, [_vp, _i, _s, _s, _s] + [_i] * 7 + [_dp]),
    "abh_analyze": (_i, [_vp, _s, _i, _s]),
    "abh_last_error": (_s, [_vp]),
    "abh_run_last": (_vp, [_vp]),
    "abh_result_state": (None, [_vp, _ip]),
    "abh_result_error": (_s, [_vp]),
    "abh_result_ndesc": (_i, [_vp, _i]),
    "abh_result_desc": (None, [_vp, _i, _i, _dp]),
    "abh_result_ndz": (_i, [_vp, _i]),
    "abh_result_dz": (C.c_float, [_vp, _i, _i]),
    "abh_result_dzdt": (C.c_float, [_vp, _i]),
    "abh_result_drdt": (C.c_float, [_vp, _i]),
    "abh_imdecode": (_i, [_u8p, _i, _u8p, _i, _ip, _ip]),
    "abh_png_walk": (_i, [_u8p, _i, _i, _i, _u32p, _i, _ip, _ip, _u8p]),
    "abh_imwrite": (_i, [_s, _u8p, _i, _i]),
    "abh_write_header": (None, [_s, _s, _i, _i]),
    "abh_event_to_file": (_i, [_vp, _s, _i, _i, _s, _s, _s, _i]),
    "abh_writer_probe": (None, [_s, _s, _i, _i, _i, _ip, _ip, _ip, _ip, _dp]),
    "abh_contours": (_i, [_u32p, _i, _i, _i, _ip, _ip, _i, _i]),
    "abh_binarize_threshold": (_i, [_u32p, _i, _i]),
    "abh_entropy": (C.c_float, [_u32p, _i, _i]),
    "abh_blob_stats": (None, [_ip, _i, _dp]),
    "abh_best_match": (None, [_u64p, _u64p, _i, _i, _u8p, _i, _i, _fp, _fp]),
    "abh_sig_new": (_vp, []),
    "abh_sig_free": (None, [_vp]),
    "abh_sig_eval": (C.c_double, [_vp, _u32p, _i, _i, _i, _ip]),
    "abh_pipe_new": (_vp, [_i] * 6 + [_ip, _i, _s]),
    "abh_pipe_free": (None, [_vp]),
    "abh_pipe_error": (_s, []),
    "abh_pipe_set_sigma": (None, [_vp, _vp]),
    "abh_pipe_run": (_i, [_vp] * 5),
    "abh_pipe_run_host": (_i, [_vp] * 4),
    "abh_pipe_stack": (_vp, [_vp, _i]),
    "abh_pipe_timing": (_i, [_vp, _dp]),
    "abh_pipe_set_option": (_i, [_vp, _s, _i]),
    "abh_pipe_blob_stats": (None, [_vp, _dp]),
    "abh_pipe_contour_stats": (None, [_vp, _dp]),
    "abh_pipe_trigger_stats": (None, [_vp, _dp]),
    "abh_pipe_trigger_totals": (None, [_dp]),
    "abh_pipe_bellows": (None, [_vp, _dp]),
}
_lib = None


def build(force=False):
    from . import _lib as hiplib

    hiplib.build(force)
    subprocess.check_call(["make", "-C", os.path.join(HERE, "host"), "-s"])
    return SO


def lib():
    global _lib
    if _lib is None:
        if not os.path.exists(SO):
            raise RuntimeError(f"{SO} is missing: run __graft_entry__.build()")
        from . import _lib as hiplib

        hiplib.lib()
        L = C.CDLL(SO)
        for name, (res, args) in SIGNATURES.items():
            fn = getattr(L, name)
            fn.restype = res
            fn.argtypes = args
        _lib = L
    return _lib


DESC_KEYS = ("x", "y", "w", "h", "area", "radius", "m00", "m10", "m01", "cx", "cy")


def _read_result(res, with_dz):
    L = lib()
    o = (C.c_int * 6)()
    L.abh_result_state(res, o)
    state = {"trig": o[1], "status": o[2], "ok": bool(o[4]), "loc_thres": o[3]}
    bubbles = []
    buf = (C.c_double * len(DESC_KEYS))()
    for b in range(o[5]):
        descs = []
        for d in range(L.abh_result_ndesc(res, b)):
            L.abh_result_desc(res, b, d, buf)
            dd = dict(zip(DESC_KEYS, list(buf)))
            for k in ("x", "y", "w", "h"):
                dd[k] = int(dd[k])
            descs.append(dd)
        bub = {"desc": descs, "dzdt": L.abh_result_dzdt(res, b), "drdt": L.abh_result_drdt(res, b)}
        if with_dz:
            bub["dz"] = [L.abh_result_dz(res, b, i) for i in range(L.abh_result_ndz(res, b))]
        bubbles.append(bub)
    return o[0], state, bubbles, L.abh_result_error(res).decode()


class Run:

    def __init__(self, kind=None, run_folder="", image_folder="Images", image_format="cam%d_image%u.png"):
        L = lib()
        if kind is None:
            self._h = L.abh_run_new()
        else:
            self._h = L.abh_run_open(0 if kind == "raw" else 1, run_folder.encode(), image_folder.encode(),
                                     image_format.encode())
            if not self._h:
                raise RuntimeError(f"cannot open run source {run_folder!r} (status -10 upstream)")

    def events(self):
        return [e for e in lib().abh_run_events(self._h).decode().split("\n") if e]

    def frames(self, event, cam):
        return [f for f in lib().abh_run_frames(self._h, str(event).encode(), cam).decode().split("\n") if f]

    def image(self, event, frame, cap=1 << 22):
        buf = np.empty(cap, np.uint8)
        w, h = C.c_int(), C.c_int()
        rc = lib().abh_run_image(self._h, str(event).encode(), frame.encode(), buf.ctypes.data_as(_u8p), cap,
                                 C.byref(w), C.byref(h))
        img = buf[: w.value * h.value].reshape(h.value, w.value).copy() if w.value * h.value else None
        return rc, img

    def close(self):
        if self._h:
            lib().abh_run_free(self._h)
            self._h = None

    def __del__(self):
        try:
            self.close()
        except Exception:
            pass

    def add_event(self, event, cam, frames, ok=None):
        frames = np.ascontiguousarray(frames, dtype=np.uint8)
        F, H, W = frames.shape
        okp = None
        if ok is not None:
            ok = np.ascontiguousarray(ok, dtype=np.uint8)
            okp = ok.ctypes.data_as(_u8p)
        lib().abh_run_add_event(self._h, str(event).encode(), cam, frames.ctypes.data_as(_u8p), F, W, H, okp)
        self._shape = (H, W)

    def train(self, cam, shape=None):
        H, W = shape if shape is not None else self._shape
        mu = np.zeros((H, W), np.uint8)
        sg = np.zeros((H, W), np.uint8)
        st, tss = C.c_int(), C.c_int()
        rc = lib().abh_train(self._h, cam, C.byref(st), C.byref(tss), mu.ctypes.data_as(_u8p), sg.ctypes.data_as(_u8p))
        if rc != 0:
            raise RuntimeError(lib().abh_last_error(self._h).decode())
        return st.value, tss.value, mu, sg

    def train_on_gpu(self, ncams, shape=None):
        H, W = shape if shape is not None else self._shape
        L = lib()
        mu = np.zeros((ncams, H, W), np.uint8)
        sg = np.zeros((ncams, H, W), np.uint8)
        st = np.zeros(ncams, np.int32)
        tss = np.zeros(ncams, np.int32)
        stats = np.zeros(4, np.float64)
        rc = L.abh_train_device(self._h, ncams, st.ctypes.data_as(_ip), tss.ctypes.data_as(_ip), mu.ctypes.data_as(_u8p),
                                sg.ctypes.data_as(_u8p), H * W, stats.ctypes.data_as(_dp))
        if rc < 0:
            raise RuntimeError(L.abh_last_error(self._h).decode())
        self.train_path = "device" if rc == 0 else "host"
        self.train_stats = {"frames_gpu_decoded": int(stats[0]), "frames_host_decoded": int(stats[1]),
                            "decode_launches": int(stats[2]), "seconds": float(stats[3])}
        return [(int(st[c]), int(tss[c]), mu[c], sg[c]) for c in range(ncams)]

    def set_model(self, cam, mu, sigma, tss):
        mu = np.ascontiguousarray(mu, dtype=np.uint8)
        sigma = np.ascontiguousarray(sigma, dtype=np.uint8)
        H, W = mu.shape
        lib().abh_set_model(self._h, cam, mu.ctypes.data_as(_u8p), sigma.ctypes.data_as(_u8p), W, H, int(tss))

    def probe_frame_stats(self, event, cam, imgs):
        L = lib()
        imgs = np.ascontiguousarray(imgs, dtype=np.uint8)
        n, H, W = imgs.shape
        out = np.zeros((n, 3), np.float64)
        rc = L.abh_probe_frame_stats(self._h, str(event).encode(), cam, imgs.ctypes.data_as(_u8p), n, W, H,
                                     out.ctypes.data_as(_dp))
        if rc != 0:
            raise RuntimeError(f"abh_probe_frame_stats rc={rc}: " + L.abh_last_error(self._h).decode())
        return out

    def run_batched(self, ncams, outdir, run_number, frame_offset, maskdir="", ngpus=1, nthreads=16, decode_threads=16,
                    batch_mb=0, shard=(0, 1)):
        L = lib()
        st = (C.c_double * 13)()
        rc = L.abh_run_batched(self._h, ncams, maskdir.encode(), outdir.encode(), run_number.encode(), frame_offset, ngpus,
                               nthreads, decode_threads, batch_mb, shard[0], shard[1], st)
        if rc != 0:
# ... 47 lines not shown
                                 outdir.encode(), run_number.encode(), frame_offset)
    if rc != 0:
        raise RuntimeError("abh_event_to_file failed")


def writer_probe(outdir, run_number, frame_offset, event, cams):
    L = lib()
    n = len(cams)
    status = (C.c_int * n)(*[c[0] for c in cams])
    frame0 = (C.c_int * n)(*[c[1] for c in cams])
    nbub = (C.c_int * n)(*[len(c[2]) for c in cams])
    nd = [len(b) for c in cams for b in c[2]]
    ndesc = (C.c_int * max(1, len(nd)))(*nd)
    rows = [float(v) for c in cams for b in c[2] for d in b for v in d]
    desc = (C.c_double * max(1, len(rows)))(*rows)
    L.abh_writer_probe(outdir.encode(), run_number.encode(), frame_offset, n, event, status, frame0, nbub, ndesc, desc)


def contours_from_indices(idx, W, H):
    idx = np.ascontiguousarray(idx, dtype=np.uint32)
    npts = np.zeros(4096, np.int32)
    xy = np.zeros((1 << 18, 2), np.int32)
    n = lib().abh_contours(idx.ctypes.data_as(_u32p), len(idx), W, H, npts.ctypes.data_as(_ip),
                           xy.ctypes.data_as(_ip), len(npts), len(xy))
    if n < 0:
        raise RuntimeError("contour probe capacity exceeded")
    out, o = [], 0
    for k in range(n):
        out.append(xy[o:o + npts[k]].copy())
        o += npts[k]
    return out


def binarize_threshold(hist, P, tozero):
    hist = np.ascontiguousarray(hist, dtype=np.uint32)
    return int(lib().abh_binarize_threshold(hist.ctypes.data_as(_u32p), int(P), int(tozero)))


def entropy(hist, nbins, P):
    hist = np.ascontiguousarray(hist, dtype=np.uint32)
    return float(lib().abh_entropy(hist.ctypes.data_as(_u32p), nbins, int(P)))


def blob_stats(xy):
    xy = np.ascontiguousarray(xy, dtype=np.int32)
    out = (C.c_double * 8)()
    lib().abh_blob_stats(xy.ctypes.data_as(_ip), len(xy), out)
    return dict(zip(("x", "y", "w", "h", "area", "m00", "m10", "m01"), list(out)))


def best_match(num, wsum2, tmpl):
    L = lib()
    num = np.ascontiguousarray(num, dtype=np.uint64)
    wsum2 = np.ascontiguousarray(wsum2, dtype=np.uint64)
    tmpl = np.ascontiguousarray(tmpl, dtype=np.uint8)
    rh, rw = num.shape
    bx, by = C.c_float(), C.c_float()
    L.abh_best_match(num.ctypes.data_as(_u64p), wsum2.ctypes.data_as(_u64p), rw, rh, tmpl.ctypes.data_as(_u8p),
                     tmpl.shape[1], tmpl.shape[0], C.byref(bx), C.byref(by))
    return bx.value, by.value


def trigger_totals():
    out = (C.c_double * 2)()
    lib().abh_pipe_trigger_totals(out)
    return int(out[0]), int(out[1])


class Significance:
    def __init__(self, tss):
        self._h = lib().abh_sig_new()
        self.tss = tss
        self.loc_thres = C.c_int(3)

    def __call__(self, hist, P, store):
        hist = np.ascontiguousarray(hist, dtype=np.uint32)
        return float(lib().abh_sig_eval(self._h, hist.ctypes.data_as(_u32p), int(P), 1 if store else 0, self.tss,
                                        C.byref(self.loc_thres)))

    def __del__(self):
        try:
            lib().abh_sig_free(self._h)
        except Exception:
            pass


class Pipeline:

    def __init__(self, device, W, H, F, E, ncams, tss, nthreads=16, maskdir=""):
        L = lib()
        t = (C.c_int * len(tss))(*tss)
        self.S = E * ncams
        self._h = L.abh_pipe_new(device, W, H, F, E, ncams, t, nthreads, maskdir.encode())
        if not self._h:
            raise RuntimeError("abh_pipe_new failed (see stderr)")

    def close(self):
        if self._h:
            lib().abh_pipe_free(self._h)
            self._h = None

    def __del__(self):
        try:
            self.close()
        except Exception:
            pass

    def set_sigma(self, sigma):
        lib().abh_pipe_set_sigma(self._h, sigma.data_ptr() if hasattr(sigma, "data_ptr") else int(sigma))

    def run(self, frames, mu, sigma6, stream=0, sigma=None):
        p = [x.data_ptr() if hasattr(x, "data_ptr") else int(x) for x in (frames, mu, sigma6)]
        if sigma is not None:
            self.set_sigma(sigma)
        rc = lib().abh_pipe_run(self._h, p[0], p[1], p[2], stream)
        if rc != 0:
            raise RuntimeError("pipeline: " + lib().abh_pipe_error().decode())

    def run_host(self, frames_host, mu, sigma6):
        L = lib()
        p =[x.data_ptr() if hasattr(x, "data_ptr") else int(x) for x in (frames_host, mu, sigma6)]
        if L.abh_pipe_run_host(self._h, p[0], p[1], p[2]) != 0:
            raise RuntimeError("pipeline: " + L.abh_pipe_error().decode())

    def timing(self):
        out = (C.c_double * 12)()
        rounds = lib().abh_pipe_timing(self._h, out)
        return dict(zip(("stage1_ms", "stage2_ms", "stage3_ms", "stage4_ms", "total_ms", "s3_gpu_ms", "s3_list_ms",
                         "s3_bucket_ms", "pairs", "trigger_jobs", "dropin_stacks", "jobs_completed_on_demand"), list(out)),
                    rounds=rounds)

    def set_option(self, name, value):
        L = lib()
        if L.abh_pipe_set_option(self._h, name.encode(), int(value)) != 0:
            raise ValueError(L.abh_pipe_error().decode())

    def blob_stats(self):
        out = (C.c_double * 8)()
        lib().abh_pipe_blob_stats(self._h, out)
        v = list(out)
        keys = ("candidates", "foreground", "kept", "components", "kept_components", "large_slots")
        d = {k: int(x) for k, x in zip(keys, v)}
        d.update(otsu_ms=v[6], k4b_ms=v[7])
        return d

    def contour_stats(self):
        out = (C.c_double * 5)()
        lib().abh_pipe_contour_stats(self._h, out)
        v = list(out)
        d = {k: int(x) for k, x in zip(("traced", "host_route", "contours", "vertices"), v)}
        d["k5_ms"] = v[4]
        return d

    def trigger_stats(self):
        out = (C.c_double * 6)()
        lib().abh_pipe_trigger_stats(self._h, out)
        v = list(out)
        d = {k: int(x) for k, x in zip(("device", "host_route", "launches", "need_frames", "need_final"), v)}
        d["k6_ms"] = v[5]
        return d

    def bellows_stats(self):
        out = (C.c_double * 5)()
        lib().abh_pipe_bellows(self._h, out)
        v = list(out)
        return {"vetoed": int(v[0]), "match_jobs": int(v[1]), "match_launches": int(v[2]), "residual_images": int(v[3]),
                "veto_ms": v[4]}

    def result(self, s):
        return _read_result(lib().abh_pipe_stack(self._h, s), with_dz=False)

    def summary(self):
        L = lib()
        o = (C.c_int * 6)()
        out = []
        for s in range(self.S):
            L.abh_result_state(L.abh_pipe_stack(self._h, s), o)
            out.append((o[0], o[1], o[5]))
        return out


class PipelineRing:

    def __init__(self, n, device, W, H, F, E, ncams, tss, nthreads=16, maskdir=""):
        self.device = device
        self.pipes = [Pipeline(device, W, H, F, E, ncams, tss, nthreads=nthreads, maskdir=maskdir) for _ in range(max(1, n))]

    def close(self):
        for p in self.pipes:
            p.close()

    def run_batches(self, batches, mu, sigma6, stream=0, on_done=None, host=False):
        import threading

        n = len(self.pipes)
        tms, errs = [], []
        lock = threading.Lock()

        def drive(i):
            try:
                try:
                    import torch

                    torch.cuda.set_device(self.device)
                except ImportError:
                    pass
                for k in range(i, len(batches), n):
                    if host:
                        self.pipes[i].run_host(batches[k], mu, sigma6)
                    else:
                        self.pipes[i].run(batches[k], mu, sigma6, stream)
                    if on_done:
                        on_done(k, self.pipes[i])
                    with lock:
                        tms.append(self.pipes[i].timing())
            except BaseException as e:
                errs.append(e)

        if n == 1:
            drive(0)
        else:
            th = [threading.Thread(target=drive, args=(i,)) for i in range(n)]
            for t in th:
                t.start()
            for t in th:
                t.join()
        if errs:
            raise errs[0]
        return tms
```

### autobub3hs_amd/host/pipeline.cpp

```cpp
#include <algorithm>
#include <atomic>
#include <condition_variable>
#include <deque>
#include <functional>
#include <mutex>
#include <cstdio>
#include <cstdlib>
#include <cstring>
#include <exception>
#include <memory>
#include <stdexcept>
#include <string>
#include <thread>
#include <vector>

#include <hip/hip_runtime_api.h>

#include "AlgorithmTraining/Trainer.hpp"
#include "AnalyzerUnit.hpp"
#include "BubbleLocalizer/L3Localizer.hpp"
#include "ParseFolder/Parser.hpp"
#include "common/CommonParameters.h"
#include "PICOFormatWriter/PICOFormatWriterV4.hpp"
#include "devctx.hpp"
// ... 94 lines not shown
        int k = 0;
        while (k + 1 < nblocks && i >= bstart[k + 1])
            ++k;
        if (!bh[k]) {
            needBlock = k;
            needPieces = false;
            throw NeedMoreFrames();
        }
        if (inc[k] && inc[k][i - bstart[k]]) {
            needBlock = k;
            needPieces = true;
            needFrame = i;
            throw NeedMoreFrames();
        }
        return bh[k] + (size_t)(i - bstart[k]) * 256;
    }
    const uint32_t *find(int kind, int i, int ref)
    {
        for (size_t k = 0; k < planned.size(); ++k)
            if (planned[k].kind == kind && planned[k].i == i && (kind == 1 || planned[k].ref == ref)) {
                cur = &planned[k];
                return roundHists + (size_t)planned[k].slot * 256;
            }
        throw std::runtime_error("BatchEventData: image was not planned for this round");
    }
    const uint32_t *diffFrame(int i, int ref, cv::Mat *) override { return find(0, i, ref); }
    const uint32_t *diffFrameROI(int, int, cv::Rect, cv::Mat *) override
    {
        throw std::runtime_error("BatchEventData: ROI diff is not available in the batched path");
    }
    const uint32_t *postTrig(int i, cv::Mat *) override { return find(1, i, 0); }
    void matchTerms(int, const cv::Mat &, std::vector<unsigned long long> &, std::vector<unsigned long long> &) override
    {
        throw NeedsDropInPath("bellows veto requested in the batched path");
    }
    const uint32_t *subtractFromCurrent(const cv::Mat &) override
    {
        throw NeedsDropInPath("bellows veto requested in the batched path");
    }
    static bool same(const cv::Rect &a, const cv::Rect &b)
    {
        return a.x == b.x && a.y == b.y && a.width == b.width && a.height == b.height;
    }
    MatchMemo *findMatch(int i, const cv::Mat &templ)
    {
        for (MatchMemo &m : matches)
            if (m.frame == i && sameTemplate(m.templ, templ))
                return &m;
        return nullptr;
    }
    void requestMatch(int i, const cv::Mat &templ)
    {
        if (!findMatch(i, templ))
            matches.push_back(MatchMemo{i, templ, false, cv::Point2f()});
    }
    cv::Point2f bestMatch(int i, const cv::Mat &templ) override
    {
        if (bellowsDropIn)
            throw NeedsDropInPath("bellows veto requested in the batched path");
        if (MatchMemo *m = findMatch(i, templ))
            if (m->ready)
                return m->xy;
        requestMatch(i, templ);
        for (const PlannedImage &p : planned)
            if (p.kind == 0 && p.i == i)
                requestMatch(p.ref, templ);
        throw NeedBellows();
    }
    const uint32_t *bellowsResidual(int trig, int pre, const cv::Mat &templ, cv::Rect rt, cv::Rect rp, cv::Rect roi) override
    {
        if (bellowsDropIn)
            throw NeedsDropInPath("bellows veto requested in the batched path");
        for (ResidualMemo &r : residuals)
            if (r.trig == trig && r.pre == pre && same(r.rt, rt) && same(r.rp, rp) && same(r.roi, roi) && r.templ.data == templ.data) {
                if (!r.ready)
                    throw NeedBellows();
                cur = &r.img;
                return r.hist;
            }
        ResidualMemo r{};
        r.trig = trig;
        r.pre = pre;
        r.rt = rt;
        r.rp = rp;
        r.roi = roi;
        r.templ = templ;
        r.ready = false;
        residuals.push_back(r);
        throw NeedBellows();
    }
    void foreground(int thr, std::vector<uint32_t> &idx) override
    {
        if (!cur || cur->thr != thr)
            throw std::runtime_error("BatchEventData::foreground: threshold differs from the planned one");
        const PlannedImage &p = *cur;
        idx.clear();
        for (uint32_t k = 0; k < p.nfg; ++k)
            if ((int)p.fgv[k] > thr)
                idx.push_back(p.fg[k]);
    }
    void foregroundKept(int thr, int minBoxArea, std::vector<uint32_t> &idx) override
    {
        if (!cur || cur->thr != thr || cur->minBox != minBoxArea)
            throw std::runtime_error("BatchEventData::foregroundKept: threshold or min box area differs from the planned one");
        const PlannedImage &p = *cur;
        if (!p.kept) {
            foreground(thr, idx);
            return;
        }
        if (p.otsuMismatch)
            throw std::runtime_error("BatchEventData::foregroundKept: device Otsu threshold differs from the host's");
        if (!p.keptShipped)
            throw std::runtime_error("BatchEventData::foregroundKept: the kept pixels of a traced image stayed on the device");
        idx.assign(p.kept, p.kept + p.nkept);
    }
    bool contoursKept(int thr, int minBoxArea, std::vector<std::vector<cv::Point>> &out) override
    {
        if (!cur || cur->thr != thr || cur->minBox != minBoxArea)
            throw std::runtime_error("BatchEventData::contoursKept: threshold or min box area differs from the planned one");
        const PlannedImage &p = *cur;
        if (!p.traced)
            return false;
        if (p.otsuMismatch)
            throw std::runtime_error("BatchEventData::contoursKept: device Otsu threshold differs from the host's");
        out.resize(p.ncont);
        const uint32_t *q = p.cpts;
        for (uint32_t k = 0; k < p.ncont; ++k) {
            std::vector<cv::Point> &c = out[k];
            c.resize(p.cnp[k]);
            for (uint32_t v = 0; v < p.cnp[k]; ++v, ++q)
                c[v] = cv::Point((int)(*q & 0xffffu), (int)(*q >> 16));
        }
        return true;
    }
};

struct StackState : StackResult {
    StackState()
    {
        loc_thres = 3;
        ok = 1;
    }
    std::unique_ptr<L3Localizer> analyzer;
    BatchEventData data;
    bool done = false;
    bool localize = false;
    bool dropIn = false;
    bool needMore = false;
    bool needBellows = false;
    bool trigReady = false;
    abub_trig_result trigRes{};
    const uint32_t *dbh[BatchEventData::MAXB] = {nullptr};
    const uint8_t *dinc[BatchEventData::MAXB] = {nullptr};
    bool vetoed = false;
};

class WorkerPool {
public:
    explicit WorkerPool(int nthreads)
    {
        for (int t = 0; t < nthreads; ++t)
            workers.emplace_back([this]() { workerLoop(); });
    }
    ~WorkerPool()
    {
        {
            std::lock_guard<std::mutex> lock(mu);
            stop = true;
        }
        cv.notify_all();
        for (auto &t : workers)
            t.join();
    }
    void parallelFor(int n, const std::function<void(int)> &fn)
    {
        if (n <= 0)
            return;
        if (n == 1 || workers.empty()) {
            for (int i = 0; i < n; ++i)
                fn(i);
            return;
        }
        auto batch = std::make_shared<Batch>();
        batch->n = n;
        batch->fn = &fn;
        batch->remaining = n;
        {
            std::lock_guard<std::mutex> lock(mu);
            batches.push_back(batch);
        }
        cv.notify_all();
        runBatch(*batch);
        std::unique_lock<std::mutex> lock(mu);
        batch->done.wait(lock, [&] { return batch->remaining == 0; });
        for (auto it = batches.begin(); it != batches.end(); ++it)
            if (it->get() == batch.get()) {
                batches.erase(it);
                break;
            }
    }

private:
    struct Batch {
        int n = 0;
        const std::function<void(int)> *fn = nullptr;
        std::atomic<int> next{0};
        int remaining = 0;
        std::condition_variable done;
    };
    void runBatch(Batch &b)
    {
        int finished = 0;
        for (;;) {
            const int i = b.next.fetch_add(1);
            if (i >= b.n)
                break;
            (*b.fn)(i);
            ++finished;
        }
        if (finished) {
            std::lock_guard<std::mutex> lock(mu);
            b.remaining -= finished;
            if (b.remaining == 0)
                b.done.notify_all();
        }
    }
    void workerLoop()
    {
        std::unique_lock<std::mutex> lock(mu);
        for (;;) {
            std::shared_ptr<Batch> pick;
            for (auto &b : batches)
                if (b->next.load() < b->n) {
                    pick = b;
                    break;
                }
            if (pick) {
                lock.unlock();
                runBatch(*pick);
                lock.lock();
                continue;
            }
            if (stop)
                return;
            cv.wait(lock);
        }
    }
    std::mutex mu;
    std::condition_variable cv;
    std::deque<std::shared_ptr<Batch>> batches;
    std::vector<std::thread> workers;
    bool stop = false;
};

}

struct CandidateList {
    uint32_t cap = 0;
    DeviceArray<uint32_t> pairs;
    DeviceArray<uint32_t> gscratch;
    Mirror<uint32_t> count, goff, gidx;
    Mirror<uint8_t> gval;
    int keptImages = 0, keptW = 0, keptH = 0;
    Mirror<uint32_t> kidx;
    DeviceArray<uint8_t> keptScratch;
    size_t keptScratchBytes = 0;

    void allocate(size_t nimg)
    {
        count.allocate(1);
        gscratch.allocate(2 * nimg);
        goff.allocate(nimg + 1);
    }
    void grow(uint32_t c)
    {
        cap = 0;
        pairs.allocate(2 * (size_t)c);
        gidx.allocate(c);
        gval.allocate(c);
        if (keptImages)
            growKept(c);
        cap = c;
    }
    void keep(int nimg, int W, int H)
    {
        keptImages = nimg;
        keptW = W;
        keptH = H;
        growKept(cap);
    }
    void growKept(uint32_t c)
    {
        keptScratchBytes = abub_label_blobs_scratch_bytes(keptImages, keptW, keptH, c, 0);
        if (keptScratchBytes == 0)
            throw std::runtime_error("RunPipeline: frame size not supported by the blob labelling");
        keptScratch.allocate(keptScratchBytes);
        kidx.allocate(c);
    }
    void group(int nimg, const uint32_t *d_hist, const int32_t *d_thr, hipStream_t s, const char *what)
    {
        check(abub_pairs_group_hist_dev(pairs, count.d, cap, nimg, gscratch, goff.d, gidx.d, gval.d, d_hist, d_thr, s), what);
    }
    void offsetsToHost(int nimg, hipStream_t s)
    {
        count.toHost(1, s);
        goff.toHost((size_t)nimg + 1, s);
    }
    bool fits(int attempt, const char *what)
    {
        const uint32_t n = *count.h;
        if (n <= cap)
            return true;
        if (attempt > 0 || n > (1u << 30))
            throw std::runtime_error(std::string("RunPipeline: ") + what);
        grow(n + n / 4 + 1024);
        return false;
    }
    void pairsToHost(hipStream_t s)
    {
        if (const uint32_t n = *count.h) {
            gidx.toHost(n, s);
            gval.toHost(n, s);
        }
    }
    void bind(PlannedImage &p, int k) const
    {
        p.fg = gidx.h + goff.h[k];
        p.fgv = gval.h + goff.h[k];
        p.nfg = goff.h[k + 1] - goff.h[k];
    }
};

struct PipeStats {
    double stage1Ms = 0, stage2Ms = 0, stage3Ms = 0, stage4Ms = 0, s3GpuMs = 0, s3ListMs = 0;
    int rounds = 0;
    uint32_t pairs = 0;
    double totalMs = 0;
    long long jobsLaunched = 0;
    long long jobsCompleted = 0;
    int dropIns = 0;
    int vetoed = 0, matchJobs = 0, matchLaunches = 0, residualImages = 0;
    double vetoMs = 0;
    long long blobCandidates = 0, blobForeground = 0, blobKept = 0, blobComponents = 0, blobKeptComponents = 0, blobLargeSlots = 0;
    double blobOtsuMs = 0, blobK4bMs = 0;
    long long contTraced = 0, contHost = 0, contContours = 0, contVertices = 0;
    double contK5Ms = 0;
    long long trigDevStacks = 0, trigHostStacks = 0, trigNeedFrames = 0, trigNeedFinal = 0, trigLaunches = 0;
    double trigK6Ms = 0;

    void reset() { *this = PipeStats(); }
    void merge(const PipeStats &g)
    {
        stage1Ms = std::max(stage1Ms, g.stage1Ms);
        stage2Ms = std::max(stage2Ms, g.stage2Ms);
        stage3Ms = std::max(stage3Ms, g.stage3Ms);
        stage4Ms = std::max(stage4Ms, g.stage4Ms);
        s3GpuMs = std::max(s3GpuMs, g.s3GpuMs);
        s3ListMs = std::max(s3ListMs, g.s3ListMs);
        rounds = std::max(rounds, g.rounds);
        pairs += g.pairs;
        vetoed += g.vetoed;
        matchJobs += g.matchJobs;
        matchLaunches += g.matchLaunches;
        residualImages += g.residualImages;
        vetoMs += g.vetoMs;
        blobCandidates += g.blobCandidates;
        blobForeground += g.blobForeground;
        blobKept += g.blobKept;
        blobComponents += g.blobComponents;
        blobKeptComponents += g.blobKeptComponents;
        blobLargeSlots += g.blobLargeSlots;
        blobOtsuMs += g.blobOtsuMs;
        blobK4bMs += g.blobK4bMs;
        contTraced += g.contTraced;
        contHost += g.contHost;
        contContours += g.contContours;
        contVertices += g.contVertices;
        contK5Ms += g.contK5Ms;
        trigDevStacks += g.trigDevStacks;
        trigHostStacks += g.trigHostStacks;
        trigNeedFrames += g.trigNeedFrames;
        trigNeedFinal += g.trigNeedFinal;
        trigK6Ms += g.trigK6Ms;
    }
};

struct Group {
    int s0 = 0, s1 = 0;
    Event stage1Done, kernelsDone, blockDone;
    struct Fetch {
        int first = 0, n = 0;
        size_t pieceOff = 0;
        bool deferred = false;
    };
    struct Block {
        Mirror<abub_job> jobs;
        Mirror<uint32_t> hist;
        DeviceArray<uint64_t> pieces;
        DeviceArray<uint32_t> pcount;
        Mirror<uint8_t> inc, want;
        size_t pieceCap = 0, pieceUsed = 0;
        int slots = 0;
        int used = 0;
        std::vector<Fetch> fetches;
    };
    std::vector<Block> blocks;
    Mirror<abub_job> jobs3;
    Mirror<uint32_t> hist3;
    DeviceArray<uint8_t> img;
    Mirror<int32_t> thr;
    CandidateList list;
    struct Blobs {
        bool ready = false;
        Mirror<int32_t> otsu, minbox;
        Mirror<uint32_t> koff, kstats;
        DeviceArray<uint32_t> ncomp, nkc, coff;
        Event ev[3];
    } blobs;
    struct Contours {
        bool ready = false;
        uint32_t inCap = 0, contCap = 0, ptsCap = 0;
        Mirror<uint32_t> status, ncont, coff, cnpts, poff, pts, cstats;
        DeviceArray<uint8_t> scratch;
        size_t scratchBytes = 0;
        Event ev[2];
    } contours;
    struct Trigger {
        bool ready = false, inflight = false;
        PinnedArray<abub_trig_stack> st;
        PinnedArray<abub_trig_seg> sg;
        DeviceArray<uint8_t> desc;
        size_t descBytes = 0;
        Mirror<abub_trig_result> res;
        std::vector<int> list;
        Event ev[2];
    } trig;
    struct Veto {
        int capJobs = 0;
        size_t scratchBytes = 0;
        Mirror<uint32_t> fidx;
        Mirror<float> xy;
        DeviceArray<uint8_t> scratch;
        int capImg = 0;
        Mirror<uint8_t> rend;
        DeviceArray<uint8_t> syn, img;
        DeviceArray<uint32_t> rhist;
        Mirror<uint32_t> hist;
        Mirror<abub_job> jobs;
        Mirror<int32_t> thr;
        CandidateList list;
        std::vector<std::pair<cv::Mat, DeviceArray<uint8_t>>> templates;
    } veto;
    int nthreads = 1;
    PipeStats stats;
    std::string error;
    Stream stream;
};

class RunPipeline {
public:
    int device, W, H, F, E, C, S, nthreads, ngroups;
    size_t P;
    std::vector<int> tss;
    std::string maskDir;
    DeviceArray<uint8_t> ownFrames;
    std::vector<Group> groups;
    std::unique_ptr<WorkerPool> pool;
    std::vector<int> blocks;
    bool deferPieces = false;
    bool bellowsDropIn = false;
    PipeStats stats;
    Stream stage1Stream;
    int chainStride = 0;
    bool ordered = true;
    int pairCap = 0;
    int blobs = 0;
    int contours = 0;
    int trigger = 0;
    bool trigOn = false;
    int trigMaxF = 0;
    std::mutex launchMu;
    std::vector<StackState> stacks;
    std::vector<std::unique_ptr<Trainer>> trainers;
    MemParser parser;
    std::vector<StackMeta> meta;
    MemParser metaParser;
    const uint8_t *d_sigmaRaw = nullptr;
    Stream copyStream;
    std::vector<Event> copied;
    bool waitCopies = false;

    void setStackMeta(std::vector<StackMeta> &&m)
    {
        if ((int)m.size() != S)
            throw std::runtime_error("RunPipeline::setStackMeta: one entry per stack expected");
        meta = std::move(m);
        metaParser = MemParser();
        for (int s = 0; s < S; ++s) {
            if ((int)meta[s].names.size() > F || meta[s].ok.size() != meta[s].names.size())
                throw std::runtime_error("RunPipeline::setStackMeta: stack longer than the pipeline's frame count");
            metaParser.AddNamedFrames(meta[s].eventID, s % C, meta[s].names);
        }
    }
    void writeEvent(int k, int eventNumber, OutputWriter &out)
    {
        StagedBubbles staged;
        for (int c = 0; c < C; ++c) {
            const StackState &ss = stacks[(size_t)k * C + c];
            if (!ss.error.empty())
                std::cout << ss.error << '\n';
            staged.stage(out, ss, c, eventNumber);
        }
        out.writeCameraOutput();
    }
    abub_job triggerJob(int s, int i, uint32_t out) const
    {
        const int c = s % C, off = refOffset(tss[c]);
        const int Fs = meta.empty() ? F : (int)meta[s].names.size();
        const int last = std::max(Fs - 1, 0);
        abub_job j;
        j.cur = (uint32_t)(s * F + std::min(i, last));
        j.ref = (uint32_t)(s * F + std::min(std::max(i - off, 0), last));
        j.model = (uint32_t)c;
        j.out = out;
        return j;
    }
    void bindBlock(Group::Block &B, int k, StackState &st_, int f, int q)
    {
        const Group::Fetch &fe = B.fetches[f];
        const size_t blen = (size_t)(blocks[k + 1] - blocks[k]), slot = (size_t)fe.first + q;
        st_.data.bh[k] = B.hist.h + slot * blen * 256;
        st_.data.inc[k] = fe.deferred ? B.inc.h + slot * blen : nullptr;
        st_.data.fetchOf[k] = f;
        st_.data.slotOf[k] = q;
    }
    void bindBlockDevice(Group::Block &B, int k, StackState &st_, int f, int q)
    {
        const Group::Fetch &fe = B.fetches[f];
        const size_t blen = (size_t)(blocks[k + 1] - blocks[k]), slot = (size_t)fe.first + q;
        st_.dbh[k] = B.hist.d + slot * blen * 256;
        st_.dinc[k] = fe.deferred ? B.inc.d + slot * blen : nullptr;
    }
    int stackFrames(int s) const { return meta.empty() ? F : (int)meta[s].names.size(); }
    bool trigHostRoute(int s) const { return stackFrames(s) > trigMaxF; }
    void launchSearch(Group &G, const std::vector<int> &list, hipStream_t stream)
    {
        Group::Trigger &T = G.trig;
        if (list.empty())
            return;
        if (T.inflight)
            throw std::runtime_error("RunPipeline: a trigger search was launched before the previous one was collected");
        const size_t ns = (size_t)(G.s1 - G.s0), nsg = ns * BatchEventData::MAXB;
        if (!T.ready) {
            T.st.allocate(ns);
            T.sg.allocate(nsg);
            T.descBytes = abub_trigger_search_desc_bytes((int)ns, (int)nsg);
            T.desc.allocate(T.descBytes);
            T.res.allocate(ns);
            T.ev[0].create(true);
            T.ev[1].create(true);
            T.ready = true;
        }
        const int nB = (int)blocks.size() - 1;
        uint32_t nseg = 0;
        for (size_t q = 0; q < list.size(); ++q) {
            const int s = list[q];
            const StackState &st_ = stacks[s];
            abub_trig_stack &d = T.st[q];
            const int Fs = stackFrames(s);
            d.seg0 = nseg;
            d.F = Fs;
            d.start = (st_.analyzer ? st_.analyzer->MatTrigFrame : 0) + 1;
            d.tss = tss[s % C];
            d.first_bad = Fs;
            if (!meta.empty())
                for (int i = 0; i < Fs; ++i)
                    if (!meta[s].ok[i]) {
                        d.first_bad = i;
                        break;
                    }
            for (int k = 0; k < nB; ++k)
                if (st_.dbh[k] && blocks[k + 1] > blocks[k]) {
                    abub_trig_seg &g = T.sg[nseg++];
                    g.hist = st_.dbh[k];
                    g.pending = st_.dinc[k];
                    g.first = blocks[k];
                    g.count = blocks[k + 1] - blocks[k];
                }
            d.nseg = nseg - d.seg0;
        }
        HIPOK(hipEventRecord(T.ev[0].get(), stream));
        check(abub_trigger_search_dev(T.st, T.sg, (int)list.size(), (int)nseg, W, H, T.desc, T.descBytes, T.res.d, nullptr, 0,
                                      stream),
              "trigger search K6");
        HIPOK(hipEventRecord(T.ev[1].get(), stream));
        T.res.toHost(list.size(), stream);
        T.list = list;
        T.inflight = true;
        ++stats.trigLaunches;
    }
    void collectSearch(Group &G)
    {
        Group::Trigger &T = G.trig;
        if (!T.inflight)
            return;
        for (size_t q = 0; q < T.list.size(); ++q) {
            StackState &st_ = stacks[T.list[q]];
            st_.trigRes = T.res.h[q];
            st_.trigReady = true;
        }
        float ms = 0;
        HIPOK(hipEventElapsedTime(&ms, T.ev[0].get(), T.ev[1].get()));
        G.stats.trigK6Ms += ms;
        T.inflight = false;
    }
    int launchBlock(Group::Block &B, int k, const std::vector<int> &list, const uint8_t *d_frames, const uint8_t *d_sigma6,
                    hipStream_t stream)
    {
        const int a = blocks[k], blen = blocks[k + 1] - blocks[k];
        const int first = B.used, n = (int)list.size();
        if (blen <= 0 || n == 0)
            return first;
        if (first + n > B.slots)
            throw std::runtime_error("RunPipeline: a frame block was requested twice for one stack");
        const size_t j0 = (size_t)first * blen;
        for (int q = 0; q < n; ++q)
            for (int i = 0; i < blen; ++i)
                B.jobs.h[j0 + (size_t)q * blen + i] = triggerJob(list[q], a + i, (uint32_t)((size_t)q * blen + i));
        abub_job *dj = B.jobs.d + j0;
        uint32_t *dh = B.hist.d + j0 * 256;
        const int nj = n * blen;
        B.jobs.toDevice(nj, stream, j0);
        Group::Fetch fe;
        fe.first = first;
        fe.n = n;
        const bool defer = deferPieces && abub_k2_deferred_ok(W, H);
        const size_t pcap = defer ? abub_k2_pieces_cap(nj, W, H) : 0;
        if (defer && B.fetches.size() < 64 && B.pieceUsed + pcap <= B.pieceCap) {
            fe.deferred = true;
            fe.pieceOff = B.pieceUsed;
            B.pieceUsed += pcap;
            check(abub_diff_hist_chained_deferred_dev(d_frames, d_sigma6, dj, nj, W, H, dh, blen, chainStride,
                                                      B.pieces + fe.pieceOff, (uint32_t)pcap, B.pcount + B.fetches.size(),
                                                      B.inc.d + j0, stream),
                  "trigger search K2 (deferred pieces)");
            B.inc.toHost(nj, stream, j0);
        } else {
            check(chainStride > 0 ? abub_diff_hist_chained_dev(d_frames, d_sigma6, dj, nj, W, H, dh, blen, chainStride, stream)
                                  : abub_diff_hist_dev(d_frames, d_sigma6, dj, nj, W, H, dh, nullptr, 0, stream),
                  "trigger search K2");
        }
        B.hist.toHost((size_t)nj * 256, stream, j0 * 256);
        B.fetches.push_back(fe);
        B.used = first + n;
        stats.jobsLaunched += nj;
        return first;
    }

    RunPipeline(int device_, int W_, int H_, int F_, int E_, int C_, const int *tss_, int nthreads_, const char *maskdir)
        : device(device_), W(W_), H(H_), F(F_), E(E_), C(C_), S(E_ * C_), nthreads(nthreads_), P((size_t)W_ * H_),
          tss(tss_, tss_ + C_), maskDir(maskdir ? maskdir : "")
    {
        if (W <= 0 || H <= 0 || F <= 0 || E <= 0 || C <= 0)
            throw std::runtime_error("RunPipeline: bad geometry");
        HIPOK(hipSetDevice(device));
        const char *eg = getenv("ABUB_PIPE_GROUPS");
        ngroups = eg ? atoi(eg) : 1;
        const char *ebw = getenv("ABUB_PIPE_BELLOWS");
        bellowsDropIn = ebw && std::string(ebw) == "dropin";
        const char *eo = getenv("ABUB_PIPE_ORDERED");
        ordered = eo ? atoi(eo) != 0 : true;
        const char *eb = getenv("ABUB_PIPE_BLOBS");
        blobs = eb ? atoi(eb) != 0 : 0;
        const char *ect = getenv("ABUB_PIPE_CONTOURS");
        contours = ect ? atoi(ect) != 0 : 0;
        const char *etr = getenv("ABUB_PIPE_TRIGGER");
        trigger = etr ? atoi(etr) != 0 : 0;
        int trigMaxSegs = 0;
        check(abub_trigger_search_limits(&trigMaxF, &trigMaxSegs), "abub_trigger_search_limits");
        if (trigMaxSegs < BatchEventData::MAXB)
            trigMaxF = 0;
        int prLow = 0, prHigh = 0;
        HIPOK(hipDeviceGetStreamPriorityRange(&prLow, &prHigh));
        stage1Stream.create(prLow);
        if (ngroups < 1)
            ngroups = 1;
        if (ngroups > S)
            ngroups = S;
        const int K = NumFramesBubbleTrack + 1;
        chainStride = chainStrideOf(tss.data(), C);
        groups.resize(ngroups);
        pool.reset(new WorkerPool(std::max(0, nthreads - ngroups)));
        {
            const char *el = getenv("ABUB_PIPE_LAZY");
            const bool lazy = el ? atoi(el) != 0 : true;
            const char *e0 = getenv("ABUB_PIPE_BLOCK0"), *e1 = getenv("ABUB_PIPE_BLOCK");
            int first = e0 && atoi(e0) > 0 ? atoi(e0) : F / 2 + 4, step = e1 && atoi(e1) > 0 ? atoi(e1) : std::max(4, F / 5);
            blocks.clear();
            blocks.push_back(1);
            if (lazy && F > 8)
                for (int b = std::min(first + 1, F); b < F && (int)blocks.size() < BatchEventData::MAXB; b += step)
                    blocks.push_back(b);
            blocks.push_back(std::max(F, 1));
            const char *ed = getenv("ABUB_PIPE_DEFER");
            deferPieces = (ed ? atoi(ed) != 0 : true) && chainStride > 0 && abub_fast_path(W) != 0;
        }
        const int nB = (int)blocks.size() - 1;
        const char *ec = getenv("ABUB_PIPE_PAIRCAP");
        pairCap = ec ? atoi(ec) : 0;
        for (int g = 0; g < ngroups; ++g) {
            Group &G = groups[g];
            G.s0 = (int)((long long)S * g / ngroups);
            G.s1 = (int)((long long)S * (g + 1) / ngroups);
            const size_t ns = (size_t)(G.s1 - G.s0), n3 = ns * K;
            G.nthreads = std::max(1, nthreads / ngroups);
            G.stream.create(prHigh);
            G.stage1Done.create(false);
            G.kernelsDone.create(false);
            G.blockDone.create(false);
            G.blocks.resize(nB);
            for (int k = 0; k < nB; ++k) {
                Group::Block &B = G.blocks[k];
                const size_t nj = ns * (size_t)std::max(blocks[k + 1] - blocks[k], 1);
                B.slots = (int)ns;
                B.jobs.allocate(nj);
                B.hist.allocate(nj * 256);
                B.pieceCap = deferPieces ? nj * (size_t)(H / 16 + 8) : 1;
                B.pieces.allocate(B.pieceCap);
                B.pcount.allocate(64);
                B.inc.allocate(nj);
                B.want.allocate(nj);
            }
            G.jobs3.allocate(n3);
            G.hist3.allocate(n3 * 256);
            G.img.allocate(abub_fast_path(W) ? 256 : n3 * P);
            G.thr.allocate(n3);
            G.list.allocate(n3);
            G.list.grow(pairCap > 0 ? (uint32_t)pairCap : (8u << 20) / ngroups);
        }
        for (int c = 0; c < C; ++c) {
            trainers.emplace_back(new Trainer(c, {}, "", "cam%d_image%u.png", "", parser.clone(), false));
            trainers.back()->TrainingSetSize = tss[c];
            trainers.back()->ModelId = 0;
        }
        std::vector<cv::Mat> none((size_t)F);
        for (int e = 0; e < E; ++e)
            for (int c = 0; c < C; ++c)
                parser.AddFrames(std::to_string(e), c, none, 10000);
    }

    ~RunPipeline()
    {
        (void)hipSetDevice(device);
        for (Group &G : groups)
            (void)abub_scratch_release(G.stream.get());
        (void)abub_scratch_release(stage1Stream.get());
    }

    void runFromHost(const uint8_t *h_frames, const uint8_t *d_mu, const uint8_t *d_sigma6)
    {
        HIPOK(hipSetDevice(device));
        if (!ownFrames) {
            ownFrames.allocate((size_t)S * F * P);
            copied.resize(ngroups);
            for (Event &e : copied)
                e.create(false);
        }
        for (int g = 0; g < ngroups; ++g) {
            const Group &G = groups[g];
            const size_t off = (size_t)G.s0 * F * P, n = (size_t)(G.s1 - G.s0) * F * P;
            HIPOK(hipMemcpyAsync(ownFrames + off, h_frames + off, n, hipMemcpyHostToDevice, copyStream.get()));
            HIPOK(hipEventRecord(copied[g].get(), copyStream.get()));
        }
        waitCopies = true;
        run(ownFrames, d_mu, d_sigma6, nullptr);
        waitCopies = false;
    }

    void run(const uint8_t *d_frames, const uint8_t *d_mu, const uint8_t *d_sigma6, hipStream_t callerStream)
    {
        HIPOK(hipSetDevice(device));
        if (!waitCopies)
            HIPOK(hipStreamSynchronize(callerStream));
        g_quietAnalyzers = true;
        double t0 = nowMs();
        stacks.clear();
        stacks.resize(S);
        trigOn = trigger != 0;
        stats.reset();
        for (size_t gi = 0; gi < groups.size(); ++gi) {
            Group &G = groups[gi];
            if (waitCopies)
                HIPOK(hipStreamWaitEvent(stage1Stream.get(), copied[gi].get(), 0));
            for (Group::Block &B : G.blocks) {
                B.used = 0;
                B.pieceUsed = 0;
                B.fetches.clear();
            }
            std::vector<int> all;
            for (int sI = G.s0; sI < G.s1; ++sI)
                all.push_back(sI);
            if (F > 1)
                launchBlock(G.blocks[0], 0, all, d_frames, d_sigma6, stage1Stream.get());
            if (trigOn) {
                G.trig.inflight = false;
                std::vector<int> dev;
                for (int sI : all)
                    if (!trigHostRoute(sI)) {
                        if (F > 1)
                            bindBlockDevice(G.blocks[0], 0, stacks[sI], 0, sI - G.s0);
                        dev.push_back(sI);
                    }
                launchSearch(G, dev, stage1Stream.get());
            }
            HIPOK(hipEventRecord(G.stage1Done.get(), stage1Stream.get()));
        }
        std::vector<std::thread> th;
        for (int g = 1; g < ngroups; ++g)
            th.emplace_back([&, g]() { runGroupNoThrow(groups[g], d_frames, d_mu, d_sigma6); });
        runGroupNoThrow(groups[0], d_frames, d_mu, d_sigma6);
        for (auto &t : th)
            t.join();
        for (int s = 0; s < S; ++s)
            if (stacks[s].dropIn) {
                ++stats.dropIns;
                runDropIn(s, d_frames, d_mu);
            }
        for (Group &G : groups) {
            if (!G.error.empty())
                throw std::runtime_error(G.error);
            stats.merge(G.stats);
        }
        g_trigTotals[0] += stats.trigDevStacks;
        g_trigTotals[1] += stats.trigHostStacks;
        stats.totalMs = nowMs() - t0;
    }

private:
    void runDropIn(int s, const uint8_t *d_frames, const uint8_t *d_mu)
    {
        StackState &st_ = stacks[s];
        st_.bubbles.clear();
        if (!d_sigmaRaw) {
            st_.staged = -6;
            st_.error = "bellows veto needs the drop-in path, but no sigma image was given to the pipeline";
            return;
        }
        const int e = s / C, c = s % C;
        try {
            const int Fs = meta.empty() ? F : (int)meta[s].names.size();
            std::vector<cv::Mat> frames((size_t)Fs);
            for (int i = 0; i < Fs; ++i) {
                if (!meta.empty() && !meta[s].ok[i])
                    continue;
                frames[i].create(H, W, CV_8U);
                HIPOK(hipMemcpy(frames[i].data, d_frames + ((size_t)s * F + i) * P, P, hipMemcpyDeviceToHost));
            }
            MemParser mp;
            const std::string evName = meta.empty() ? std::to_string(e) : meta[s].eventID;
            if (meta.empty())
                mp.AddFrames(evName, c, frames, 10000);
            else
                mp.AddNamedFrames(evName, c, meta[s].names, &frames);
            Trainer t(c, {}, "", "cam%d_image%u.png", "", mp.clone(), false);
            t.TrainedAvgImage.create(H, W, CV_8U);
            t.TrainedSigmaImage.create(H, W, CV_8U);
            HIPOK(hipMemcpy(t.TrainedAvgImage.data, d_mu + (size_t)c * P, P, hipMemcpyDeviceToHost));
            HIPOK(hipMemcpy(t.TrainedSigmaImage.data, d_sigmaRaw + (size_t)c * P, P, hipMemcpyDeviceToHost));
            t.TrainingSetSize = tss[c];
            t.ModelId = 0;
            Trainer *tp = &t;
            L3Localizer A(evName, "", c, true, &tp, maskDir, mp.clone());
            st_.staged = analyzeUntilBubble(&A, true, "", st_.error);
            if (st_.staged != -6)
                st_.capture(A);
        } catch (std::exception &ex) {
            st_.error = ex.what();
            st_.staged = -6;
        }
        DeviceContext::releaseThread();
    }

    void runGroupNoThrow(Group &G, const uint8_t *d_frames, const uint8_t *d_mu, const uint8_t *d_sigma6)
    {
        G.error.clear();
        try {
            (void)hipSetDevice(device);
            runGroup(G, d_frames, d_mu, d_sigma6);
        } catch (std::exception &e) {
            G.error = e.what();
        }
    }

    void runGroup(Group &G, const uint8_t *d_frames, const uint8_t *d_mu, const uint8_t *d_sigma6)
    {
        G.stats.reset();
        const int ns = G.s1 - G.s0;
        double t0 = nowMs();
        pool->parallelFor(ns, [&](int k) {
            const int s = G.s0 + k;
            StackState &st_ = stacks[s];
            const int e = s / C, c = s % C;
            Trainer *t = trainers[c].get();
            if (meta.empty()) {
                st_.analyzer.reset(new L3Localizer(std::to_string(e), "", c, true, &t, maskDir, parser.clone()));
                st_.data.F = F;
                st_.data.ok = nullptr;
            } else {
                st_.analyzer.reset(new L3Localizer(meta[s].eventID, "", c, true, &t, maskDir, metaParser.clone()));
                st_.data.F = (int)meta[s].names.size();
                st_.data.ok = meta[s].ok.data();
            }
            st_.data.W = W;
            st_.data.H = H;
            st_.data.refOffset = refOffset(tss[c]);
            st_.data.bellowsDropIn = bellowsDropIn;
            st_.data.clearVeto();
            st_.vetoed = false;
            st_.data.nblocks = (int)blocks.size() - 1;
            for (size_t b = 0; b < blocks.size(); ++b)
                st_.data.bstart[b] = blocks[b];
            for (int b = 0; b < st_.data.nblocks; ++b) {
                st_.data.bh[b] = nullptr;
                st_.data.inc[b] = nullptr;
            }
            if (F > 1)
                bindBlock(G.blocks[0], 0, st_, 0, k);
            st_.analyzer->AttachEventData(&st_.data);
        });
        HIPOK(hipEventSynchronize(G.stage1Done.get()));
        G.stats.stage1Ms = nowMs() - t0;

        std::vector<int> pending(ns);
        for (int k = 0; k < ns; ++k)
            pending[k] = G.s0 + k;
        if (trigOn)
            for (int sI : pending)
                ++(trigHostRoute(sI) ? G.stats.trigHostStacks : G.stats.trigDevStacks);
        while (!pending.empty()) {
            ++G.stats.rounds;
            double t2 = nowMs();
            std::vector<int> todo(pending);
            while (!todo.empty()) {
                if (trigOn) {
                    collectSearch(G);
                    std::vector<int> ask;
                    for (int sI : todo)
                        if (!trigHostRoute(sI) && !stacks[sI].trigReady)
                            ask.push_back(sI);
                    if (!ask.empty()) {
                        {
                            std::lock_guard<std::mutex> lock(launchMu);
                            hipStream_t stream = ordered ? stage1Stream.get() : G.stream.get();
                            launchSearch(G, ask, stream);
                            HIPOK(hipEventRecord(G.blockDone.get(), stream));
                        }
                        HIPOK(hipEventSynchronize(G.blockDone.get()));
                        collectSearch(G);
                    }
                }
                pool->parallelFor((int)todo.size(), [&](int k) { triggerAndPlan(stacks[todo[k]]); });
                std::vector<int> need;
                for (int sI : todo) {
                    if (trigOn && !trigHostRoute(sI) && stacks[sI].needMore)
                        ++(stacks[sI].data.needPieces ? G.stats.trigNeedFinal : G.stats.trigNeedFrames);
                    if (stacks[sI].needMore)
                        need.push_back(sI);
                }
                if (need.empty())
                    break;
                fetchBlocks(G, need, d_frames, d_sigma6);
                todo.swap(need);
            }
            G.stats.stage2Ms += nowMs() - t2;
            double t3 = nowMs();
            std::vector<int> loc;
            for (int s : pending)
                if (stacks[s].localize)
                    loc.push_back(s);
            if (!loc.empty())
                batchImages(G, loc, d_frames, d_mu, d_sigma6);
            G.stats.stage3Ms += nowMs() - t3;
            double t4 = nowMs();
            pool->parallelFor((int)loc.size(), [&](int k) { localize(stacks[loc[k]]); });
            vetoRound(G, loc, d_frames, d_sigma6);
            G.stats.stage4Ms += nowMs() - t4;
            std::vector<int> next;
            for (int s : pending)
                if (!stacks[s].done)
                    next.push_back(s);
            pending.swap(next);
        }
        pool->parallelFor(ns, [&](int k) {
            StackState &st_ = stacks[G.s0 + k];
            st_.capture(*st_.analyzer);
            st_.analyzer.reset();
        });
    }

    void fetchBlocks(Group &G, const std::vector<int> &need, const uint8_t *d_frames, const uint8_t *d_sigma6)
    {
        hipStream_t stream = ordered ? stage1Stream.get() : G.stream.get();
        const int nB = (int)blocks.size() - 1;
        std::vector<std::vector<int>> byBlock((size_t)nB);
        std::vector<std::vector<std::vector<int>>> byFetch((size_t)nB);
        for (int sI : need) {
            const BatchEventData &d = stacks[sI].data;
            if (!d.needPieces)
                byBlock[(size_t)d.needBlock].push_back(sI);
            else {
                auto &v = byFetch[(size_t)d.needBlock];
                if (v.size() <= (size_t)d.fetchOf[d.needBlock])
                    v.resize((size_t)d.fetchOf[d.needBlock] + 1);
                v[(size_t)d.fetchOf[d.needBlock]].push_back(sI);
            }
        }
        std::vector<int> newFetch((size_t)nB, -1);
        {
            std::lock_guard<std::mutex> lock(launchMu);
            for (int k = 0; k < nB; ++k) {
                Group::Block &B = G.blocks[k];
                if (!byBlock[k].empty()) {
                    launchBlock(B, k, byBlock[k], d_frames, d_sigma6, stream);
                    newFetch[k] = (int)B.fetches.size() - 1;
                    if (trigOn)
                        for (size_t q = 0; q < byBlock[k].size(); ++q)
                            bindBlockDevice(B, k, stacks[byBlock[k][q]], newFetch[k], (int)q);
                }
                const size_t blen = (size_t)(blocks[k + 1] - blocks[k]);
                for (size_t f = 0; f < byFetch[k].size(); ++f) {
                    if (byFetch[k][f].empty())
                        continue;
                    const Group::Fetch &fe = B.fetches[f];
                    const size_t nj = (size_t)fe.n * blen, base = (size_t)fe.first * blen;
                    uint8_t *hw = B.want.h + base;
                    std::memset(hw, 0, nj);
                    for (int sI : byFetch[k][f]) {
                        BatchEventData &d = stacks[sI].data;
                        for (size_t j = (size_t)(d.needFrame - blocks[k]); j < blen; ++j)
                            if (d.inc[k][j]) {
                                hw[(size_t)d.slotOf[k] * blen + j] = 1;
                                ++stats.jobsCompleted;
                            }
                    }
                    B.want.toDevice(nj, stream, base);
                    check(abub_diff_hist_pieces_dev(d_frames, d_sigma6, B.jobs.d + base, (int)nj, W, H, B.hist.d + base * 256,
                                                    B.pieces + fe.pieceOff, B.pcount + f, B.want.d + base, stream),
                          "trigger search K2 (pieces)");
                    for (int sI : byFetch[k][f]) {
                        BatchEventData &d = stacks[sI].data;
                        const size_t j0 = (size_t)(d.needFrame - blocks[k]), o = (base + (size_t)d.slotOf[k] * blen + j0) * 256;
                        B.hist.toHost((blen - j0) * 256, stream, o);
                    }
                    if (trigOn)
                        check(abub_trigger_clear_pending_dev(B.inc.d + base, B.want.d + base, nj, stream), "trigger search flags");
                }
            }
            if (trigOn) {
                std::vector<int> dev;
                for (int sI : need)
                    if (!trigHostRoute(sI))
                        dev.push_back(sI);
                launchSearch(G, dev, stream);
            }
            HIPOK(hipEventRecord(G.blockDone.get(), stream));
        }
        HIPOK(hipEventSynchronize(G.blockDone.get()));
        for (int k = 0; k < nB; ++k) {
            for (size_t q = 0; q < byBlock[k].size(); ++q) {
                StackState &st_ = stacks[byBlock[k][q]];
                bindBlock(G.blocks[k], k, st_, newFetch[k], (int)q);
                st_.needMore = false;
            }
            const size_t blen = (size_t)(blocks[k + 1] - blocks[k]);
            for (auto &v : byFetch[k])
                for (int sI : v) {
                    StackState &st_ = stacks[sI];
                    for (size_t j = (size_t)(st_.data.needFrame - blocks[k]); j < blen; ++j)
                        st_.data.inc[k][j] = 0;
                    st_.needMore = false;
                }
        }
    }

    bool applySearch(StackState &st_)
    {
        AnalyzerUnit *A = st_.analyzer.get();
        BatchEventData &d = st_.data;
        const abub_trig_result r = st_.trigRes;
        st_.trigReady = false;
        if (r.state == ABUB_TRIG_NEED_FRAMES || r.state == ABUB_TRIG_NEED_FINAL) {
            int k = 0;
            while (k + 1 < d.nblocks && r.need_frame >= d.bstart[k + 1])
                ++k;
            d.needBlock = k;
            d.needPieces = r.state == ABUB_TRIG_NEED_FINAL;
            d.needFrame = r.need_frame;
            if (d.needPieces ? !d.inc[k] : d.bh[k] != nullptr)
                throw std::runtime_error("RunPipeline: the device trigger search asked for a frame that is there");
            st_.needMore = true;
            return false;
        }
        if (r.state == ABUB_TRIG_BAD_LOOKAHEAD)
            throw std::runtime_error("AnalyzerUnit::FindTriggerFrame: undecodable look-ahead frame");
        if (r.state != ABUB_TRIG_DONE)
            throw std::runtime_error("RunPipeline: unknown answer of the device trigger search");
        const int s = (int)(&st_ - stacks.data());
        if (r.status == -9 && d.F >= 5 && !meta.empty()) {
            const int i = A->MatTrigFrame + 1 + r.evaluated;
            if (i >= 0 && i < (int)meta[s].names.size())
                std::cout << "Image " << meta[s].names[i] << " is corrupted/empty of camera " << s % C << " for the event "
                          << meta[s].eventID << "." << std::endl;
        }
        A->TriggerFrameIdentificationStatus = r.status;
        if (r.loc_thres >= 0)
            A->loc_thres = r.loc_thres;
        if (r.status == 0)
            A->MatTrigFrame = r.trig;
        else
            A->okToProceed = false;
        return true;
    }

    void triggerAndPlan(StackState &st_)
    {
        st_.localize = false;
        st_.needMore = false;
        AnalyzerUnit *A = st_.analyzer.get();
        try {
            size_t pixSize[256];
            const bool havePix = A->pix_counts.size() == 256;
            for (int b = 0; havePix && b < 256; ++b)
                pixSize[b] = A->pix_counts[b].size();
            const int trig0 = A->MatTrigFrame, loc0 = A->loc_thres, status0 = A->TriggerFrameIdentificationStatus;
            const bool ok0 = A->okToProceed;
            try {
                if (trigOn && !trigHostRoute((int)(&st_ - stacks.data()))) {
                    if (!st_.trigReady)
                        throw std::runtime_error("RunPipeline: no answer of the device trigger search for this stack");
                    if (!applySearch(st_))
                        return;
                } else
                    A->FindTriggerFrame(true, A->MatTrigFrame + 1);
            } catch (NeedMoreFrames &) {
                for (int b = 0; havePix && b < 256 && A->pix_counts.size() == 256; ++b)
                    A->pix_counts[b].resize(pixSize[b]);
                A->MatTrigFrame = trig0;
                A->loc_thres = loc0;
                A->TriggerFrameIdentificationStatus = status0;
                A->okToProceed = ok0;
                st_.needMore = true;
                return;
            }
            if (!A->okToProceed) {
                st_.staged = A->TriggerFrameIdentificationStatus;
                st_.done = true;
                return;
            }
            const int F = st_.data.F;
            if (F <= 5) {
                A->LocalizeOMatic("");
                st_.staged = -8;
                st_.done = true;
                return;
            }
            const int t = A->MatTrigFrame;
            const int off = refOffset(A->TrainedData->TrainingSetSize);
            st_.data.planned.clear();
            st_.data.cur = nullptr;
            st_.data.clearVeto();
            PlannedImage g;
            g.kind = 0;
            g.i = t;
            g.ref = std::max(t - off, 0);
            g.tozero = A->loc_thres;
            g.slot = -1;
            g.thr = 0;
            g.minBox = -1;
            st_.data.planned.push_back(g);
            const int last = (t < 29) ? NumFramesBubbleTrack : (39 - t);
            for (int k = 1; k <= last; ++k) {
                if (t + k >= F)
                    break;
                PlannedImage p;
                p.kind = 1;
                p.i = t + k;
                p.ref = 0;
                p.tozero = 3;
                p.slot = -1;
                p.thr = 0;
                p.minBox = kTrackMinBoxArea;
                st_.data.planned.push_back(p);
            }
            st_.localize = true;
        } catch (std::exception &e) {
            st_.error = e.what();
            st_.staged = -6;
            st_.done = true;
        }
    }

    void batchImages(Group &G, const std::vector<int> &loc, const uint8_t *d_frames, const uint8_t *d_mu,
                     const uint8_t *d_sigma6)
    {
        hipStream_t stream = ordered ? stage1Stream.get() : G.stream.get();
        hipStream_t back = G.stream.get();
        int nd = 0, np = 0;
        for (int s : loc)
            for (PlannedImage &p : stacks[s].data.planned)
                (p.kind == 0 ? nd : np)++;
        std::vector<int> order(loc);
        std::stable_sort(order.begin(), order.end(), [&](int a, int b) { return a % C < b % C; });
        int di = 0, pi = nd;
        for (int s : order) {
            const int c = s % C;
            for (PlannedImage &p : stacks[s].data.planned) {
                p.slot = p.kind == 0 ? di++ : pi++;
                abub_job &j = G.jobs3.h[p.slot];
                j.cur = (uint32_t)(s * F + p.i);
                j.ref = (uint32_t)(s * F + p.ref);
                j.model = (uint32_t)c;
                j.out = (uint32_t)(p.kind == 0 ? p.slot : p.slot - nd);
            }
        }
// ... 398 lines not shown
        B.ready = true;
    }

    void fitContours(Group &G, int nimg)
    {
        Group::Contours &K = G.contours;
        if (!K.ready) {
            const size_t n3 = (size_t)(G.s1 - G.s0) * (NumFramesBubbleTrack + 1);
            K.status.allocate(n3);
            K.ncont.allocate(n3);
            K.coff.allocate(n3 + 1);
            K.poff.allocate(n3 + 1);
            K.cstats.allocate(4);
            for (Event &e : K.ev)
                e.create(true);
            K.ready = true;
        }
        if (K.inCap != G.list.cap) {
            K.scratchBytes = abub_trace_contours_scratch_bytes((int)((size_t)(G.s1 - G.s0) * (NumFramesBubbleTrack + 1)), G.list.cap);
            if (K.scratchBytes == 0 || W > 65535 || H > 65535)
                throw std::runtime_error("RunPipeline: frame size not supported by the contour tracing");
            K.scratch.allocate(K.scratchBytes);
            K.inCap = G.list.cap;
        }
        (void)nimg;
        if (K.contCap == 0)
            growContours(K, G.list.cap / 4 + 64, G.list.cap / 4 + 64);
    }
    void growContours(Group::Contours &K, uint32_t nc, uint32_t nv)
    {
        if (nc > K.contCap) {
            K.contCap = 0;
            K.cnpts.allocate((size_t)nc + nc / 4 + 64);
            K.contCap = nc + nc / 4 + 64;
        }
        if (nv > K.ptsCap) {
            K.ptsCap = 0;
            K.pts.allocate((size_t)nv + nv / 4 + 64);
            K.ptsCap = nv + nv / 4 + 64;
        }
    }

    void localize(StackState &st_)
    {
        st_.needBellows = false;
        AnalyzerUnit *A = st_.analyzer.get();
        try {
            A->LocalizeOMatic("");
            if (!A->okToProceed) {
                st_.staged = -8;
                st_.done = true;
                return;
            }
            st_.staged = A->BubbleList.empty() ? -1 : 0;
            st_.done = !A->BubbleList.empty();
        } catch (NeedBellows &) {
            st_.needBellows = true;
        } catch (NeedsDropInPath &) {
            st_.dropIn = true;
            st_.done = true;
        } catch (std::exception &e) {
            st_.error = e.what();
            st_.staged = -6;
            st_.done = true;
        }
    }
};

void RunPipelineDelete::operator()(RunPipeline *p) const { delete p; }

RunPipelinePtr newRunPipeline(int device, int W, int H, int F, int E, int C, const int *tss, int nthreads, const char *maskDir)
{
    return RunPipelinePtr(new RunPipeline(device, W, H, F, E, C, tss, nthreads, maskDir));
}
void setSigmaRaw(RunPipeline &p, const uint8_t *d_sigma) { p.d_sigmaRaw = d_sigma; }
bool setTrainingSetSizes(RunPipeline &p, const int *tss)
{
    if (chainStrideOf(tss, p.C) != p.chainStride)
        return false;
    for (int c = 0; c < p.C; ++c) {
        p.tss[c] = tss[c];
        p.trainers[c]->TrainingSetSize = tss[c];
    }
    return true;
}
void setStackMeta(RunPipeline &p, std::vector<StackMeta> &&meta) { p.setStackMeta(std::move(meta)); }
void run(RunPipeline &p, const uint8_t *d_frames, const uint8_t *d_mu, const uint8_t *d_sigma6, hipStream_t stream)
{
    p.run(d_frames, d_mu, d_sigma6, stream);
}
void writeEvent(RunPipeline &p, int k, int eventNumber, OutputWriter &out) { p.writeEvent(k, eventNumber, out); }
int bellowsVetoed(const RunPipeline &p) { return p.stats.vetoed; }

}

extern "C" {

void *abh_pipe_new(int device, int W, int H, int F, int E, int C, const int *tss, int nthreads, const char *maskdir)
{
    try {
        return new abub::RunPipeline(device, W, H, F, E, C, tss, nthreads, maskdir);
    } catch (std::exception &e) {
        fprintf(stderr, "abh_pipe_new: %s\n", e.what());
        return nullptr;
    }
}

void abh_pipe_free(void *p) { delete (abub::RunPipeline *)p; }

static thread_local std::string g_pipeErr;
const char *abh_pipe_error() { return g_pipeErr.c_str(); }

void abh_pipe_set_sigma(void *p, const void *sigma_dev) { ((abub::RunPipeline *)p)->d_sigmaRaw = (const uint8_t *)sigma_dev; }

int abh_pipe_run(void *p, const void *frames_dev, const void *mu_dev, const void *sigma6_dev, void *stream)
{
    try {
        ((abub::RunPipeline *)p)->run((const uint8_t *)frames_dev, (const uint8_t *)mu_dev, (const uint8_t *)sigma6_dev,
                                      (hipStream_t)stream);
        return 0;
    } catch (std::exception &e) {
        g_pipeErr = e.what();
        return -1;
    }
}

int abh_pipe_run_host(void *p, const void *frames_host, const void *mu_dev, const void *sigma6_dev)
{
    try {
        ((abub::RunPipeline *)p)->runFromHost((const uint8_t *)frames_host, (const uint8_t *)mu_dev, (const uint8_t *)sigma6_dev);
        return 0;
    } catch (std::exception &e) {
        g_pipeErr = e.what();
        return -1;
    }
}

const void *abh_pipe_stack(void *p, int s)
{
    const abub::StackResult &res = ((abub::RunPipeline *)p)->stacks[s];
    return &res;
}

void abh_pipe_bellows(void *p, double *out)
{
    const abub::PipeStats &st = ((abub::RunPipeline *)p)->stats;
    const double v[5] = {(double)st.vetoed, (double)st.matchJobs, (double)st.matchLaunches, (double)st.residualImages, st.vetoMs};
    std::memcpy(out, v, sizeof v);
}

int abh_pipe_set_option(void *p, const char *name, int value)
{
    const std::string opt = name ? name : "";
    if (opt != "blobs" && opt != "contours" && opt != "trigger") {
        g_pipeErr = std::string("abh_pipe_set_option: unknown option ") + (name ? name : "(null)");
        return -1;
    }
    if (value != 0 && value != 1) {
        g_pipeErr = "abh_pipe_set_option: " + opt + " takes 0 or 1";
        return -1;
    }
    if (!p) {
        g_pipeErr = "abh_pipe_set_option: no pipeline";
        return -1;
    }
    abub::RunPipeline *rp = (abub::RunPipeline *)p;
    (opt == "blobs" ? rp->blobs : opt == "contours" ? rp->contours : rp->trigger) = value;
    return 0;
}

void abh_pipe_trigger_stats(void *p, double *out)
{
    const abub::PipeStats &st = ((abub::RunPipeline *)p)->stats;
    const double v[6] = {(double)st.trigDevStacks, (double)st.trigHostStacks, (double)st.trigLaunches, (double)st.trigNeedFrames,
                         (double)st.trigNeedFinal, st.trigK6Ms};
    std::memcpy(out, v, sizeof v);
}

void abh_pipe_trigger_totals(double *out)
{
    out[0] = (double)abub::g_trigTotals[0].load();
    out[1] = (double)abub::g_trigTotals[1].load();
}

void abh_pipe_contour_stats(void *p, double *out)
{
    const abub::PipeStats &st = ((abub::RunPipeline *)p)->stats;
    const double v[5] = {(double)st.contTraced, (double)st.contHost, (double)st.contContours, (double)st.contVertices,
                         st.contK5Ms};
    std::memcpy(out, v, sizeof v);
}

void abh_pipe_blob_stats(void *p, double *out)
{
    const abub::PipeStats &st = ((abub::RunPipeline *)p)->stats;
    const double v[8] = {(double)st.blobCandidates, (double)st.blobForeground, (double)st.blobKept, (double)st.blobComponents,
                         (double)st.blobKeptComponents, (double)st.blobLargeSlots, st.blobOtsuMs, st.blobK4bMs};
    std::memcpy(out, v, sizeof v);
}

int abh_pipe_timing(void *p, double *out)
{
    const abub::PipeStats &st = ((abub::RunPipeline *)p)->stats;
    const double v[12] = {st.stage1Ms, st.stage2Ms, st.stage3Ms, st.stage4Ms, st.totalMs, st.s3GpuMs, st.s3ListMs,
                          0.0,
                          (double)st.pairs, (double)st.jobsLaunched, (double)st.dropIns, (double)st.jobsCompleted};
    std::memcpy(out, v, sizeof v);
    return st.rounds;
}
}
```

### include/abub_hip.h

```cpp
#ifndef ABUB_HIP_H
#define ABUB_HIP_H

#include <stddef.h>
#include <stdint.h>

#ifdef __cplusplus
extern "C" {
#endif

#define ABUB_OK 0
#define ABUB_E_INVALID (-1)
#define ABUB_E_HIP (-2)
#define ABUB_E_NODEVICE (-3)
#define ABUB_E_OVERFLOW (-4)

typedef struct {
    uint32_t cur;
    uint32_t ref;
    uint32_t model;
    uint32_t out;
} abub_job;

const char *abub_last_error(void);
int abub_device_count(void);
int abub_device_info(int device, char *name, int name_cap, int *cus, uint64_t *hbm_bytes);


int abub_sigma6_dev(const uint8_t *sigma, uint8_t *sigma6, size_t n, void *stream);

int abub_fill_stack_jobs_dev(abub_job *jobs, int nstacks, int F, int first, int count, int ref_offset,
                             int nmodels, void *stream);

int abub_diff_hist_dev(const uint8_t *frames, const uint8_t *sigma6, const abub_job *jobs, int njobs,
                       int W, int H, uint32_t *hist, uint8_t *diff, int rows_per_chunk, void *stream);

int abub_diff_roi_dev(const uint8_t *cur, const uint8_t *ref, const uint8_t *sigma6, int W, int H,
                      int rx, int ry, int rw, int rh, uint8_t *diff, uint32_t *hist, void *stream);

int abub_train_dev(const uint8_t *frames, const uint32_t *idx, int N, int W, int H, uint8_t *mu,
                   uint8_t *sigma, void *stream);

int abub_pair_hist_dev(const uint8_t *frames, const abub_job *pairs, int npairs, int W, int H,
                       uint32_t *hist, void *stream);

int abub_posttrig_dev(const uint8_t *frames, const uint8_t *mu, const uint8_t *sigma6,
                      const abub_job *jobs, int njobs, int W, int H, uint32_t *hist, uint8_t *img,
                      void *stream);

int abub_fg_compact_dev(const uint8_t *img, int nimg, int W, int H, const int32_t *thr,
                        uint32_t *idx, int cap, uint32_t *count, void *stream);

int abub_fast_path(int W);

int abub_diff_hist_chained_dev(const uint8_t *frames, const uint8_t *sigma6, const abub_job *jobs, int njobs, int W,
                               int H, uint32_t *hist, int chain_len, int chain_stride, void *stream);

int abub_diff_hist_chained_store_dev(const uint8_t *frames, const uint8_t *sigma6, const abub_job *jobs, int njobs, int W,
                                     int H, uint32_t *hist, uint8_t *diff, int chain_len, int chain_stride, void *stream);

size_t abub_k2_pieces_cap(int njobs, int W, int H);
int abub_diff_hist_chained_deferred_dev(const uint8_t *frames, const uint8_t *sigma6, const abub_job *jobs, int njobs, int W,
                                        int H, uint32_t *hist, int chain_len, int chain_stride, void *pieces,
                                        uint32_t pieces_cap, uint32_t *npieces, uint8_t *incomplete, void *stream);
int abub_diff_hist_pieces_dev(const uint8_t *frames, const uint8_t *sigma6, const abub_job *jobs, int njobs, int W, int H,
                              uint32_t *hist, const void *pieces, const uint32_t *npieces, const uint8_t *want, void *stream);

int abub_k2_set_option(const char *name, int value);

int abub_k2_deferred_ok(int W, int H);

int abub_k3_set_option(const char *name, int value);

int abub_scratch_release(void *stream);

int abub_bound_counts_dev(void *stream, uint32_t counts[2]);
int abub_diff_hist_compact_dev(const uint8_t *frames, const uint8_t *sigma6, const abub_job *jobs, int njobs,
                               int W, int H, uint32_t *hist, uint8_t *diff, const int32_t *cthr,
                               uint32_t *pairs, uint32_t cap, uint32_t *count, uint32_t slot_base,
                               void *stream);
int abub_posttrig_compact_dev(const uint8_t *frames, const uint8_t *mu, const uint8_t *sigma6,
                              const abub_job *jobs, int njobs, int W, int H, uint32_t *hist, uint8_t *img,
                              const int32_t *cthr, uint32_t *pairs, uint32_t cap, uint32_t *count,
                              uint32_t slot_base, void *stream);

int abub_pairs_group_dev(const uint32_t *pairs, const uint32_t *count, uint32_t cap, int nslots,
                         uint32_t *scratch , uint32_t *offsets ,
                         uint32_t *idx_out , uint8_t *val_out , void *stream);

int abub_pairs_group_hist_dev(const uint32_t *pairs, const uint32_t *count, uint32_t cap, int nslots,
                              uint32_t *scratch, uint32_t *offsets, uint32_t *idx_out, uint8_t *val_out,
                              const uint32_t *hist , const int32_t *cthr ,
                              void *stream);

int abub_fg_compact_pairs_dev(const uint8_t *img, int nimg, int W, int H, const int32_t *thr,
                              uint32_t *pairs, uint32_t cap, uint32_t *count, void *stream);

int abub_binarize_thr_dev(const uint32_t *hist, const int32_t *tozero, int nslots, int W, int H, int32_t *thr, void *stream);

typedef struct abub_blob {
    uint32_t first;
    int32_t x0, y0, x1, y1;
    uint32_t npix;
} abub_blob;

int abub_label_blobs_dev(const uint32_t *offsets, const uint32_t *idx, const uint8_t *val, uint32_t in_cap, int nslots, int W,
                         int H, const int32_t *thr, const int32_t *min_box_area, uint32_t *kept_off, uint32_t *kept_idx,
                         uint32_t cap, uint32_t *ncomp, uint32_t *nkept_comp, uint32_t *comp_off, abub_blob *comp,
                         uint32_t comp_cap, uint32_t *stats, void *scratch, size_t scratch_bytes, void *stream);
size_t abub_label_blobs_scratch_bytes(int nslots, int W, int H, uint32_t in_cap, int with_comp);

int abub_trace_contours_dev(const uint32_t *kept_off, const uint32_t *kept_idx, uint32_t in_cap, int nslots, int W, int H,
                            uint32_t *status, uint32_t *ncont, uint32_t *cont_off, uint32_t *cont_npts, uint32_t cont_cap,
                            uint32_t *pt_off, uint32_t *pts, uint32_t pts_cap, uint32_t *stats, void *scratch,
                            size_t scratch_bytes, void *stream);
size_t abub_trace_contours_scratch_bytes(int nslots, uint32_t in_cap);
int abub_trace_contours_limits(int *max_pixels, int *max_chain);

typedef struct abub_trig_seg {
    const uint32_t *hist;
    const uint8_t *pending;
    int32_t first, count;
} abub_trig_seg;
typedef struct abub_trig_stack {
    uint32_t seg0, nseg;
    int32_t F;
    int32_t start;
    int32_t tss;
    int32_t first_bad;
} abub_trig_stack;
#define ABUB_TRIG_DONE 0
#define ABUB_TRIG_NEED_FRAMES 1
#define ABUB_TRIG_NEED_FINAL 2
#define ABUB_TRIG_BAD_LOOKAHEAD 3
typedef struct abub_trig_result {
    int32_t state;
    int32_t status, trig;
    int32_t loc_thres;
    int32_t need_frame;
    int32_t evaluated;
    float sig;
    int32_t reserved;
} abub_trig_result;
int abub_trigger_search_dev(const abub_trig_stack *stacks, const abub_trig_seg *segs, int nstacks, int nsegs, int W, int H,
                            void *desc, size_t desc_bytes, abub_trig_result *out, double *sig_main, int sig_pitch,
                            void *stream);
int abub_trigger_clear_pending_dev(uint8_t *pending, const uint8_t *done, size_t n, void *stream);
size_t abub_trigger_search_desc_bytes(int nstacks, int nsegs);
int abub_trigger_search_limits(int *max_frames, int *max_segs);

int abub_match_ccorr_dev(const uint8_t *img, int W, int H, const uint8_t *tmpl, int tw, int th,
                         unsigned long long *num, unsigned long long *wsum2, void *stream);
int abub_match_ccorr_batch_dev(const uint8_t *frames, int W, int H, const uint32_t *frame_idx, int njobs,
                               const uint8_t *tmpl, int tw, int th, unsigned long long *num, unsigned long long *wsum2,
                               void *stream);
int abub_match_best_batch_dev(const uint8_t *frames, int W, int H, const uint32_t *frame_idx, int njobs,
                              const uint8_t *tmpl, int tw, int th, float *best_xy, void *scratch, size_t scratch_bytes,
                              void *stream);
size_t abub_match_best_scratch_bytes(int W, int H, int tw, int th, int njobs);
int abub_subsat_hist_dev(uint8_t *img, const uint8_t *sub, int W, int H, uint32_t *hist, void *stream);


typedef struct abub_ctx abub_ctx;

int abub_ctx_create(abub_ctx **out, int device, int W, int H, int max_frames);
void abub_ctx_destroy(abub_ctx *ctx);

int abub_ctx_train(abub_ctx *ctx, const uint8_t *const *frames, int N, uint8_t *mu_out,
                   uint8_t *sigma_out);
int abub_ctx_pair_hist(abub_ctx *ctx, const uint8_t *f0, const uint8_t *f1, uint32_t hist[256]);

int abub_ctx_set_model(abub_ctx *ctx, const uint8_t *mu, const uint8_t *sigma);

int abub_ctx_upload_stack(abub_ctx *ctx, const uint8_t *const *frames, int F);

int abub_ctx_diff_hist_batch(abub_ctx *ctx, int ref_offset, int first, int count, uint32_t *hist_out);

int abub_ctx_diff_frame(abub_ctx *ctx, int i, int ref, uint8_t *D_out, uint32_t *hist_out);

int abub_ctx_diff_frame_roi(abub_ctx *ctx, int i, int ref, int rx, int ry, int rw, int rh, uint8_t *D_out,
                            uint32_t *hist_out);

int abub_ctx_posttrig(abub_ctx *ctx, int i, uint8_t *O_out, uint32_t *hist_out);

int abub_ctx_foreground(abub_ctx *ctx, int thr, uint32_t *idx_out, int cap, int *n);

int abub_ctx_match_template(abub_ctx *ctx, int i, const uint8_t *tmpl, int tw, int th, unsigned long long *num_out,
                            unsigned long long *wsum2_out);
int abub_ctx_subtract_image(abub_ctx *ctx, const uint8_t *sub, uint32_t *hist_out);
int abub_ctx_set_image(abub_ctx *ctx, const uint8_t *img);

int abub_ctx_fetch_image(abub_ctx *ctx, uint8_t *out);

typedef struct abub_png_seg {
    uint32_t off;
    uint32_t len;
} abub_png_seg;
typedef struct abub_png_frame {
    uint32_t seg_begin;
    uint32_t seg_count;
    uint32_t zoff;
    uint32_t zlen;
    uint32_t lut;
    uint32_t reserved;
    uint64_t dst;
} abub_png_frame;
#define ABUB_PNG_E_DESC 1
#define ABUB_PNG_E_HEADER 2
#define ABUB_PNG_E_TRUNCATED 3
#define ABUB_PNG_E_BLOCKTYPE 4
#define ABUB_PNG_E_STORED 5
#define ABUB_PNG_E_SYMBOLS 6
#define ABUB_PNG_E_CODES 7
#define ABUB_PNG_E_NOEOB 8
#define ABUB_PNG_E_CODE 9
#define ABUB_PNG_E_DISTANCE 10
#define ABUB_PNG_E_TOOMUCH 11
#define ABUB_PNG_E_TOOLITTLE 12
#define ABUB_PNG_E_ADLER 13
#define ABUB_PNG_E_FILTER 14
#define ABUB_PNG_E_INTERNAL 15
size_t abub_png_raw_stride(int W, int H);
int abub_png_decode_dev(const uint8_t *files, size_t files_bytes, const abub_png_frame *frames, int nframes,
                        const abub_png_seg *segs, int nsegs, const uint8_t *luts, int nluts, int W, int H,
                        uint8_t *zbuf, size_t zbuf_bytes, uint8_t *rawbuf, size_t rawbuf_bytes, uint8_t *out,
                        size_t out_bytes, int32_t *status, void *stream);

#ifdef __cplusplus
}
#endif
#endif
```

Baseline: 3.272 million.

## Chain trigger search and gated diff-hist blocks on device to skip fetch rounds

Adds a device-side gate. After each trigger search, a small kernel marks which stacks need the next frame block, and the chained diff-hist kernel launches for every stack but returns early for the ones not marked. Hist clearing and the bin-0 fixup are gated the same way, and the trigger search skips segments whose validity flag is unset. This aims to remove host round trips and per-round fetch launches by running the stage-1 search, gate and diff loop entirely on the stream. The cost is extra launches and some wasted grid blocks, plus added bookkeeping for evaluated masks on the host.

Result: slower. 3.158 million (-3.5%).

```diff
diff --git a/autobub3hs_amd/_lib.py b/autobub3hs_amd/_lib.py
--- a/autobub3hs_amd/_lib.py
+++ b/autobub3hs_amd/_lib.py
@@ -49,6 +49,7 @@
     "abub_diff_hist_chained_store_dev": (_i, [_vp, _vp, _vp, _i, _i, _i, _vp, _vp, _i, _i, _vp]),
     "abub_k2_set_option": (_i, [C.c_char_p, _i]),
     "abub_k2_deferred_ok": (_i, [_i, _i]),
+    "abub_k2_gated_ok": (_i, [_i, _i]),
     "abub_k3_set_option": (_i, [C.c_char_p, _i]),
     "abub_k2_pieces_cap": (_sz, [_i, _i, _i]),
     "abub_png_raw_stride": (_sz, [_i, _i]),
@@ -74,6 +75,9 @@
     "abub_trace_contours_scratch_bytes": (_sz, [_i, C.c_uint32]),
     "abub_trace_contours_limits": (_i, [C.POINTER(_i), C.POINTER(_i)]),
     "abub_trigger_search_dev": (_i, [_vp, _vp, _i, _i, _i, _i, _vp, _sz, _vp, _vp, _i, _vp]),
+    "abub_trigger_search_gated_dev": (_i, [_vp, _vp, _vp, _i, _i, _i, _i, _vp, _sz, _vp, _vp, _i, _vp]),
+    "abub_trigger_gate_dev": (_i, [_vp, _vp, _i, _i, _i, _vp, _vp, _i, _vp]),
+    "abub_diff_hist_chained_gated_dev": (_i, [_vp, _vp, _vp, _i, _i, _i, _vp, _i, _i, _vp, C.c_uint32, _vp, _vp, _vp, _vp]),
     "abub_trigger_search_desc_bytes": (_sz, [_i, _i]),
     "abub_trigger_clear_pending_dev": (_i, [_vp, _vp, _sz, _vp]),
     "abub_trigger_search_limits": (_i, [C.POINTER(_i), C.POINTER(_i)]),
diff --git a/autobub3hs_amd/csrc/abub_dev.hpp b/autobub3hs_amd/csrc/abub_dev.hpp
--- a/autobub3hs_amd/csrc/abub_dev.hpp
+++ b/autobub3hs_amd/csrc/abub_dev.hpp
@@ -469,4 +469,5 @@
     uint32_t df_cap = 0;
     uint32_t *df_count = nullptr;
     uint8_t *df_incomplete = nullptr;
+    const uint8_t *run = nullptr;
 };
diff --git a/autobub3hs_amd/csrc/abub_k2.hip b/autobub3hs_amd/csrc/abub_k2.hip
--- a/autobub3hs_amd/csrc/abub_k2.hip
+++ b/autobub3hs_amd/csrc/abub_k2.hip
@@ -586,8 +586,11 @@
                                                    int H, int rows_per_chunk, int nchunks, uint32_t budget,
                                                    uint2 *__restrict__ units, uint32_t *__restrict__ nunits,
                                                    uint32_t *__restrict__ hist, uint8_t *__restrict__ diff, SusList gl,
-                                                   int syncD, uint8_t *__restrict__ incomplete)
-{
+                                                   int syncD, uint8_t *__restrict__ incomplete,
+                                                   const uint8_t *__restrict__ run)
+{
+    if (run && !run[(blockIdx.x / (unsigned)nchunks) / (unsigned)nwgs])
+        return;
     using Job = K2BoundJob<NDW, false, true>;
     extern __shared__ uint32_t k2c_lds[];
     const int NW = (int)(blockDim.x >> 6);
@@ -979,7 +982,8 @@
             units = ca.df_pieces;
             npieces = ca.df_count;
             HIPCHK(hipMemsetAsync(npieces, 0, sizeof(uint32_t), st));
-            HIPCHK(hipMemsetAsync(ca.df_incomplete, 0, (size_t)njobs, st));
+            if (!ca.run)
+                HIPCHK(hipMemsetAsync(ca.df_incomplete, 0, (size_t)njobs, st));
         }
         SusList gl;
         gl.list = gcap ? (uint2 *)(scr + 256 + unitBytes) : nullptr;
@@ -1004,7 +1008,7 @@
             constexpr bool CAN_SPLIT = NDW >= 5 && NDW <= 7;
             const bool split = CAN_SPLIT && opt.split;
             const bool pf2 = NDW == 5 && split && Kc == 4 && (opt.scanpf < 0 || opt.scanpf == 2);
-#define K2C_ARGS frames, sigma6, jobs, L, S, nwgs, W, H, R, nchunks, budget, units, npieces, hist, diff, gl, syncD, ca.df_incomplete
+#define K2C_ARGS frames, sigma6, jobs, L, S, nwgs, W, H, R, nchunks, budget, units, npieces, hist, diff, gl, syncD, ca.df_incomplete, ca.run
 #define K2C_LAUNCH_SP(KK, SP, PFD) \
     hipLaunchKernelGGL((k2_sad_chain<NDW, KK, SP, PFD>), grid, dim3(64 * NW), ldsBytes, st, K2C_ARGS)
 #define K2C_LAUNCH(KK)                                                                                              \
@@ -1025,6 +1029,8 @@
 #undef K2C_ARGS
 #undef K2C_LAUNCH
         } else {
+            if (ca.run)
+                return set_err(ABUB_E_INVALID, "gated launches need the chained scan (options \"chain\" >= 2)");
 #define K2S_LAUNCH(CO)                                                                                              \
     hipLaunchKernelGGL((k2_bound_scan<NDW, CO>), dim3((unsigned)nunits), dim3(64), 0, st, frames, sigma6, jobs, W, H, \
                        R, nchunks, budget, units, npieces, hist, diff, ca.cthr, ca.pairs, ca.cap, ca.count,         \
@@ -1100,6 +1106,32 @@
     return R;
 }
 
+static __global__ __launch_bounds__(64) void k2_gated_clear(uint32_t *__restrict__ hist, uint8_t *__restrict__ incomplete,
+                                                            const uint8_t *__restrict__ run, int L,
+                                                            const abub_job *__restrict__ jobs)
+{
+    if (!run[blockIdx.x / (unsigned)L])
+        return;
+    uint4 *h = reinterpret_cast<uint4 *>(hist + (size_t)jobs[blockIdx.x].out * 256);
+    h[threadIdx.x] = make_uint4(0u, 0u, 0u, 0u);
+    if (threadIdx.x == 0)
+        incomplete[blockIdx.x] = 0;
+}
+
+static __global__ __launch_bounds__(64) void k2_gated_bin0(uint32_t *hist, uint32_t P, const uint8_t *__restrict__ run, int L,
+                                                           const abub_job *__restrict__ jobs)
+{
+    if (!run[blockIdx.x / (unsigned)L])
+        return;
+    uint32_t *h = hist + (size_t)jobs[blockIdx.x].out * 256;
+    const int l = threadIdx.x;
+    uint32_t s = h[l + 64] + h[l + 128] + h[l + 192] + (l ? h[l] : 0u);
+    for (int o = 32; o > 0; o >>= 1)
+        s += __shfl_xor(s, o);
+    if (l == 0)
+        h[0] = P - s;
+}
+
 static int diff_hist_impl(const uint8_t *frames, const uint8_t *sigma6, const abub_job *jobs, int njobs,
                           int W, int H, uint32_t *hist, uint8_t *diff, int rows_per_chunk,
                           const CompactArgs &ca, void *stream)
@@ -1109,7 +1141,10 @@
     if (njobs == 0)
         return ABUB_OK;
     hipStream_t st = (hipStream_t)stream;
-    HIPCHK(hipMemsetAsync(hist, 0, (size_t)njobs * 256 * sizeof(uint32_t), st));
+    if (ca.run)
+        hipLaunchKernelGGL(k2_gated_clear, dim3((unsigned)njobs), dim3(64), 0, st, hist, ca.df_incomplete, ca.run, ca.chain_len, jobs);
+    else
+        HIPCHK(hipMemsetAsync(hist, 0, (size_t)njobs * 256 * sizeof(uint32_t), st));
     int ndw = pick_ndw(W);
     if (ndw) {
         const int R = rows_per_chunk ? rows_per_chunk : k2_auto_rows(njobs, H);
@@ -1138,7 +1173,10 @@
                            W, H, hist, diff);
     }
     HIPCHK(hipGetLastError());
-    hipLaunchKernelGGL(k_hist_bin0, dim3(njobs), dim3(64), 0, st, hist, (uint32_t)((size_t)W * H));
+    if (ca.run)
+        hipLaunchKernelGGL(k2_gated_bin0, dim3(njobs), dim3(64), 0, st, hist, (uint32_t)((size_t)W * H), ca.run, ca.chain_len, jobs);
+    else
+        hipLaunchKernelGGL(k_hist_bin0, dim3(njobs), dim3(64), 0, st, hist, (uint32_t)((size_t)W * H));
     HIPCHK(hipGetLastError());
     return ABUB_OK;
 }
@@ -1203,6 +1241,33 @@
     ca.df_cap = pieces_cap;
     ca.df_count = npieces;
     ca.df_incomplete = incomplete;
+    return diff_hist_impl(frames, sigma6, jobs, njobs, W, H, hist, nullptr, 0, ca, stream);
+}
+
+extern "C" int abub_k2_gated_ok(int W, int H)
+{
+    const int c = k2_options().chain;
+    return abub_k2_deferred_ok(W, H) && (c < 0 || c >= 2);
+}
+
+extern "C" int abub_diff_hist_chained_gated_dev(const uint8_t *frames, const uint8_t *sigma6, const abub_job *jobs, int njobs,
+                                                int W, int H, uint32_t *hist, int chain_len, int chain_stride, void *pieces,
+                                                uint32_t pieces_cap, uint32_t *npieces, uint8_t *incomplete,
+                                                const uint8_t *run, void *stream)
+{
+    const K2Options opt = k2_options();
+    if (chain_len <= 0 || chain_stride <= 0 || chain_stride > 8 || njobs < 0 || njobs % chain_len != 0 || !pieces || !npieces ||
+        !incomplete || !run || !pick_ndw(W) || !opt.bound || (opt.chain >= 0 && opt.chain < 2) || H <= 0 || H >= 65536)
+        return set_err(ABUB_E_INVALID, "abub_diff_hist_chained_gated_dev: bad arguments (or no chained scan for this width and "
+                                       "these options)");
+    CompactArgs ca = {nullptr, nullptr, 0, nullptr, 0};
+    ca.chain_len = chain_len;
+    ca.chain_stride = chain_stride;
+    ca.df_pieces = (uint2 *)pieces;
+    ca.df_cap = pieces_cap;
+    ca.df_count = npieces;
+    ca.df_incomplete = incomplete;
+    ca.run = run;
     return diff_hist_impl(frames, sigma6, jobs, njobs, W, H, hist, nullptr, 0, ca, stream);
 }
 
diff --git a/autobub3hs_amd/csrc/abub_trigger.hip b/autobub3hs_amd/csrc/abub_trigger.hip
--- a/autobub3hs_amd/csrc/abub_trigger.hip
+++ b/autobub3hs_amd/csrc/abub_trigger.hip
@@ -142,7 +142,7 @@
 __global__ __launch_bounds__(64) void k_trigger_search(const abub_trig_stack *__restrict__ stacks,
                                                        const abub_trig_seg *__restrict__ segs, int nsegs, int P,
                                                        abub_trig_result *__restrict__ out, double *__restrict__ sig_main,
-                                                       int sig_pitch)
+                                                       int sig_pitch, const uint8_t *const *__restrict__ valid)
 {
     __shared__ TrigShared sh;
     const int lane = threadIdx.x;
@@ -177,6 +177,8 @@
     const uint32_t seg1 = min(sd.seg0 + min(sd.nseg, (uint32_t)TRIG_MAXSEG), (uint32_t)nsegs);
     for (uint32_t k = sd.seg0; k < seg1; ++k) {
         const abub_trig_seg sg = segs[k];
+        if (valid && valid[k] && !*valid[k])
+            continue;
         for (int q = lane; q < sg.count; q += 64) {
             const int j = sg.first + q;
             if (j < 1 || j >= n || j >= firstBad || !sg.hist)
@@ -267,6 +269,21 @@
     out[blockIdx.x] = res;
 }
 
+__global__ __launch_bounds__(256) void k_trigger_gate(const abub_trig_result *__restrict__ res, const uint32_t *__restrict__ slot,
+                                                      int nstacks, int first, int count, uint8_t *__restrict__ run,
+                                                      uint32_t *__restrict__ evaluated, int bit)
+{
+    const int q = (int)(blockIdx.x * 256 + threadIdx.x);
+    if (q >= nstacks)
+        return;
+    const abub_trig_result r = res[q];
+    const bool on = r.state == ABUB_TRIG_NEED_FRAMES && r.need_frame >= first && r.need_frame - first < count;
+    const uint32_t s = slot ? slot[q] : (uint32_t)q;
+    run[s] = on ? 1 : 0;
+    if (on)
+        evaluated[s] |= 1u << bit;
+}
+
 __global__ __launch_bounds__(256) void k_trigger_clear_pending(uint8_t *__restrict__ pending, const uint8_t *__restrict__ done, size_t n)
 {
     const size_t j = (size_t)blockIdx.x * 256 + threadIdx.x;
@@ -287,6 +304,19 @@
     return ABUB_OK;
 }
 
+extern "C" int abub_trigger_gate_dev(const abub_trig_result *res, const uint32_t *slot, int nstacks, int first, int count,
+                                     uint8_t *run, uint32_t *evaluated, int bit, void *stream)
+{
+    if (!res || !run || !evaluated || nstacks < 0 || first < 0 || count < 0 || bit < 0 || bit >= TRIG_MAXSEG)
+        return set_err(ABUB_E_INVALID, "abub_trigger_gate_dev: bad arguments");
+    if (nstacks == 0)
+        return ABUB_OK;
+    hipLaunchKernelGGL(k_trigger_gate, dim3((unsigned)((nstacks + 255) / 256)), dim3(256), 0, (hipStream_t)stream, res, slot, nstacks,
+                       first, count, run, evaluated, bit);
+    HIPCHK(hipGetLastError());
+    return ABUB_OK;
+}
+
 extern "C" int abub_trigger_search_limits(int *max_frames, int *max_segs)
 {
     if (max_frames)
@@ -300,12 +330,21 @@
 {
     if (nstacks <= 0 || nsegs < 0)
         return 0;
-    return (((size_t)nstacks * sizeof(abub_trig_stack) + 255) & ~(size_t)255) + (size_t)nsegs * sizeof(abub_trig_seg) + 256;
+    return (((size_t)nstacks * sizeof(abub_trig_stack) + 255) & ~(size_t)255) +
+           (((size_t)nsegs * sizeof(abub_trig_seg) + 255) & ~(size_t)255) + (size_t)nsegs * sizeof(void *) + 256;
 }
 
 extern "C" int abub_trigger_search_dev(const abub_trig_stack *stacks, const abub_trig_seg *segs, int nstacks, int nsegs, int W,
                                        int H, void *desc, size_t desc_bytes, abub_trig_result *out, double *sig_main,
                                        int sig_pitch, void *stream)
+{
+    return abub_trigger_search_gated_dev(stacks, segs, nullptr, nstacks, nsegs, W, H, desc, desc_bytes, out, sig_main, sig_pitch,
+                                         stream);
+}
+
+extern "C" int abub_trigger_search_gated_dev(const abub_trig_stack *stacks, const abub_trig_seg *segs, const uint8_t *const *valid,
+                                             int nstacks, int nsegs, int W, int H, void *desc, size_t desc_bytes,
+                                             abub_trig_result *out, double *sig_main, int sig_pitch, void *stream)
 {
     static_assert(sizeof(abub_trig_result) == 32 && sizeof(abub_trig_stack) == 24 && sizeof(abub_trig_seg) == 24, "record layout");
     if (!stacks || !out || !desc || nstacks < 0 || nsegs < 0 || (nsegs > 0 && !segs) || W <= 0 || H <= 0 ||
@@ -335,10 +374,15 @@
     abub_trig_stack *dst = (abub_trig_stack *)desc;
     abub_trig_seg *dsg = (abub_trig_seg *)((uint8_t *)desc + (((size_t)nstacks * sizeof(abub_trig_stack) + 255) & ~(size_t)255));
     HIPCHK(hipMemcpyAsync(dst, stacks, (size_t)nstacks * sizeof(abub_trig_stack), hipMemcpyHostToDevice, st));
+    const uint8_t **dvl = nullptr;
     if (nsegs > 0)
         HIPCHK(hipMemcpyAsync(dsg, segs, (size_t)nsegs * sizeof(abub_trig_seg), hipMemcpyHostToDevice, st));
+    if (nsegs > 0 && valid) {
+        dvl = (const uint8_t **)((uint8_t *)dsg + (((size_t)nsegs * sizeof(abub_trig_seg) + 255) & ~(size_t)255));
+        HIPCHK(hipMemcpyAsync(dvl, valid, (size_t)nsegs * sizeof(void *), hipMemcpyHostToDevice, st));
+    }
     hipLaunchKernelGGL(k_trigger_search, dim3(nstacks), dim3(64), 0, st, dst, dsg, nsegs, (int)((size_t)W * H), out, sig_main,
-                       sig_pitch);
+                       sig_pitch, (const uint8_t *const *)dvl);
     HIPCHK(hipGetLastError());
     return ABUB_OK;
 }
diff --git a/autobub3hs_amd/hip.py b/autobub3hs_amd/hip.py
--- a/autobub3hs_amd/hip.py
+++ b/autobub3hs_amd/hip.py
@@ -76,6 +76,24 @@
     return hist, (pieces, npieces, incomplete)
 
 
+def diff_hist_gated(frames, sigma6_, jobs, W, H, chain, run, hist=None, state=None):
+    _need_cuda(frames, sigma6_, jobs, run)
+    n = jobs.shape[0]
+    cap = int(_lib.lib().abub_k2_pieces_cap(n, W, H))
+    if hist is None:
+        hist = torch.empty((n, 256), dtype=torch.int32, device=frames.device)
+    if state is None:
+        state = (torch.empty((max(cap, 1), 2), dtype=torch.int32, device=frames.device),
+                 torch.zeros((1,), dtype=torch.int32, device=frames.device),
+                 torch.empty((n,), dtype=torch.uint8, device=frames.device))
+    pieces, npieces, incomplete = state
+    _lib.check(_lib.lib().abub_diff_hist_chained_gated_dev(_ptr(frames), _ptr(sigma6_), _ptr(jobs), n, W, H, _ptr(hist),
+                                                           int(chain[0]), int(chain[1]), _ptr(pieces), cap, _ptr(npieces),
+                                                           _ptr(incomplete), _ptr(run), _stream()),
+               "abub_diff_hist_chained_gated_dev")
+    return hist, state
+
+
 def diff_hist_pieces(frames, sigma6_, jobs, W, H, hist, state, want):
     _need_cuda(frames, sigma6_, jobs, want)
     pieces, npieces, _ = state
@@ -233,13 +251,17 @@
     nseg = sum(len(s["segs"]) for s in stacks)
     st = (_lib.TrigStack * max(n, 1))()
     sg = (_lib.TrigSeg * max(nseg, 1))()
+    vl = (C.c_void_p * max(nseg, 1))()
     k = 0
     dev = None
     for i, s in enumerate(stacks):
         st[i].seg0, st[i].nseg, st[i].F, st[i].tss = k, len(s["segs"]), s["F"], s["tss"]
         st[i].start, st[i].first_bad = s.get("start", 1), s.get("first_bad", s["F"])
-        for first, hist, pending in s["segs"]:
-            _need_cuda(hist, pending)
+        for seg in s["segs"]:
+            first, hist, pending = seg[:3]
+            valid = seg[3] if len(seg) > 3 else None
+            _need_cuda(hist, pending, valid)
+            vl[k] = _ptr(valid)
             dev = hist.device
             sg[k].hist, sg[k].pending, sg[k].first, sg[k].count = _ptr(hist), _ptr(pending), first, hist.shape[0]
             k += 1
@@ -251,8 +273,13 @@
     out = torch.zeros((max(n, 1), 8), dtype=torch.int32, device=dev)
     pitch = max([s["F"] for s in stacks] + [1])
     sm = torch.full((max(n, 1), pitch), float("nan"), dtype=torch.float64, device=dev) if sig_main else None
-    _lib.check(L.abub_trigger_search_dev(C.addressof(st), C.addressof(sg), n, nseg, W, H, _ptr(desc), desc.numel(), _ptr(out),
-                                         _ptr(sm), pitch, _stream()), "abub_trigger_search_dev")
+    if any(len(seg) > 3 for s in stacks for seg in s["segs"]):
+        _lib.check(L.abub_trigger_search_gated_dev(C.addressof(st), C.addressof(sg), C.addressof(vl), n, nseg, W, H, _ptr(desc),
+                                                   desc.numel(), _ptr(out), _ptr(sm), pitch, _stream()),
+                   "abub_trigger_search_gated_dev")
+    else:
+        _lib.check(L.abub_trigger_search_dev(C.addressof(st), C.addressof(sg), n, nseg, W, H, _ptr(desc), desc.numel(), _ptr(out),
+                                             _ptr(sm), pitch, _stream()), "abub_trigger_search_dev")
     rows = out.cpu().numpy()
     names = ("state", "status", "trig", "loc_thres", "need_frame", "evaluated")
     res = []
@@ -261,6 +288,12 @@
         r["sig"] = struct.unpack("<f", struct.pack("<i", int(rows[i, 6])))[0]
         res.append(r)
     return res, (sm[:n] if sig_main else None)
+
+
+def trigger_gate(res, first, count, run, evaluated, bit, slot=None):
+    _need_cuda(res, run, evaluated, slot)
+    _lib.check(_lib.lib().abub_trigger_gate_dev(_ptr(res), _ptr(slot), res.shape[0], first, count, _ptr(run), _ptr(evaluated),
+                                                bit, _stream()), "abub_trigger_gate_dev")
 
 
 def png_parse(data, W, H):
diff --git a/autobub3hs_amd/host.py b/autobub3hs_amd/host.py
--- a/autobub3hs_amd/host.py
+++ b/autobub3hs_amd/host.py
@@ -65,6 +65,7 @@
     "abh_pipe_contour_stats": (None, [_vp, _dp]),
     "abh_pipe_trigger_stats": (None, [_vp, _dp]),
     "abh_pipe_trigger_totals": (None, [_dp]),
+    "abh_pipe_chain_stats": (None, [_vp, _dp]),
     "abh_pipe_bellows": (None, [_vp, _dp]),
 }
 _lib = None
@@ -418,6 +419,11 @@
         d["k5_ms"] = v[4]
         return d
 
+    def chain_stats(self):
+        out = (C.c_double * 3)()
+        lib().abh_pipe_chain_stats(self._h, out)
+        return {"blocks_chained": int(out[0]), "stack_blocks_evaluated": int(out[1]), "host_fetch_rounds": int(out[2])}
+
     def trigger_stats(self):
         out = (C.c_double * 6)()
         lib().abh_pipe_trigger_stats(self._h, out)
diff --git a/autobub3hs_amd/host/pipeline.cpp b/autobub3hs_amd/host/pipeline.cpp
--- a/autobub3hs_amd/host/pipeline.cpp
+++ b/autobub3hs_amd/host/pipeline.cpp
@@ -270,6 +270,7 @@
     abub_trig_result trigRes{};
     const uint32_t *dbh[BatchEventData::MAXB] = {nullptr};
     const uint8_t *dinc[BatchEventData::MAXB] = {nullptr};
+    const uint8_t *dvalid[BatchEventData::MAXB] = {nullptr};
     bool vetoed = false;
 };
 
@@ -465,6 +466,7 @@
     double contK5Ms = 0;
     long long trigDevStacks = 0, trigHostStacks = 0, trigNeedFrames = 0, trigNeedFinal = 0, trigLaunches = 0;
     double trigK6Ms = 0;
+    long long chainBlocks = 0, chainEvaluated = 0, fetchRounds = 0;
 
     void reset() { *this = PipeStats(); }
     void merge(const PipeStats &g)
@@ -500,6 +502,9 @@
         trigNeedFrames += g.trigNeedFrames;
         trigNeedFinal += g.trigNeedFinal;
         trigK6Ms += g.trigK6Ms;
+        chainBlocks += g.chainBlocks;
+        chainEvaluated += g.chainEvaluated;
+        fetchRounds += g.fetchRounds;
     }
 };
 
@@ -547,12 +552,17 @@
         bool ready = false, inflight = false;
         PinnedArray<abub_trig_stack> st;
         PinnedArray<abub_trig_seg> sg;
+        PinnedArray<const uint8_t *> valid;
+        uint32_t nseg = 0;
         DeviceArray<uint8_t> desc;
         size_t descBytes = 0;
         Mirror<abub_trig_result> res;
         std::vector<int> list;
         Event ev[2];
     } trig;
+    bool chained = false;
+    DeviceArray<uint8_t> gate;
+    Mirror<uint32_t> evalMask, trigSlot;
     struct Veto {
         int capJobs = 0;
         size_t scratchBytes = 0;
@@ -596,6 +606,7 @@
     int contours = 0;
     int trigger = 0;
     bool trigOn = false;
+    int chain = 0;
     int trigMaxF = 0;
     std::mutex launchMu;
     std::vector<StackState> stacks;
@@ -661,7 +672,7 @@
     }
     int stackFrames(int s) const { return meta.empty() ? F : (int)meta[s].names.size(); }
     bool trigHostRoute(int s) const { return stackFrames(s) > trigMaxF; }
-    void launchSearch(Group &G, const std::vector<int> &list, hipStream_t stream)
+    void launchSearch(Group &G, const std::vector<int> &list, hipStream_t stream, bool fill = true, bool collect = true)
     {
         Group::Trigger &T = G.trig;
         if (list.empty())
@@ -672,6 +683,7 @@
         if (!T.ready) {
             T.st.allocate(ns);
             T.sg.allocate(nsg);
+            T.valid.allocate(nsg);
             T.descBytes = abub_trigger_search_desc_bytes((int)ns, (int)nsg);
             T.desc.allocate(T.descBytes);
             T.res.allocate(ns);
@@ -680,8 +692,8 @@
             T.ready = true;
         }
         const int nB = (int)blocks.size() - 1;
-        uint32_t nseg = 0;
-        for (size_t q = 0; q < list.size(); ++q) {
+        uint32_t nseg = fill ? 0 : T.nseg;
+        for (size_t q = 0; fill && q < list.size(); ++q) {
             const int s = list[q];
             const StackState &st_ = stacks[s];
             abub_trig_stack &d = T.st[q];
@@ -704,18 +716,23 @@
                     g.pending = st_.dinc[k];
                     g.first = blocks[k];
                     g.count = blocks[k + 1] - blocks[k];
+                    T.valid[nseg - 1] = st_.dvalid[k];
                 }
             d.nseg = nseg - d.seg0;
         }
-        HIPOK(hipEventRecord(T.ev[0].get(), stream));
-        check(abub_trigger_search_dev(T.st, T.sg, (int)list.size(), (int)nseg, W, H, T.desc, T.descBytes, T.res.d, nullptr, 0,
-                                      stream),
+        T.nseg = nseg;
+        if (collect)
+            HIPOK(hipEventRecord(T.ev[0].get(), stream));
+        check(abub_trigger_search_gated_dev(T.st, T.sg, T.valid, (int)list.size(), (int)nseg, W, H, T.desc, T.descBytes, T.res.d,
+                                            nullptr, 0, stream),
               "trigger search K6");
+        ++stats.trigLaunches;
+        if (!collect)
+            return;
         HIPOK(hipEventRecord(T.ev[1].get(), stream));
         T.res.toHost(list.size(), stream);
         T.list = list;
         T.inflight = true;
-        ++stats.trigLaunches;
     }
     void collectSearch(Group &G)
     {
@@ -732,14 +749,36 @@
         G.stats.trigK6Ms += ms;
         T.inflight = false;
     }
-    int launchBlock(Group::Block &B, int k, const std::vector<int> &list, const uint8_t *d_frames, const uint8_t *d_sigma6,
-                    hipStream_t stream)
+    void launchBlock(Group &G, Group::Block &B, int k, const std::vector<int> &list, const uint8_t *d_frames,
+                     const uint8_t *d_sigma6, hipStream_t stream, std::vector<std::pair<int, int>> *where = nullptr)
+    {
+        const int n = (int)list.size();
+        if (where)
+            where->assign((size_t)n, std::make_pair(0, 0));
+        if (blocks[k + 1] - blocks[k] <= 0 || n == 0)
+            return;
+        if (!(G.chained && k >= 1)) {
+            const int f = launchRun(G, B, k, list.data(), n, B.used, nullptr, true, d_frames, d_sigma6, stream);
+            B.used += n;
+            for (int q = 0; q < n && where; ++q)
+                (*where)[q] = std::make_pair(f, q);
+            return;
+        }
+        for (int a = 0; a < n;) {
+            int b = a + 1;
+            while (b < n && list[b] == list[b - 1] + 1)
+                ++b;
+            const int f = launchRun(G, B, k, list.data() + a, b - a, list[a] - G.s0, nullptr, true, d_frames, d_sigma6, stream);
+            for (int q = a; q < b && where; ++q)
+                (*where)[q] = std::make_pair(f, q - a);
+            a = b;
+        }
+    }
+    int launchRun(Group &G, Group::Block &B, int k, const int *list, int n, int first, const uint8_t *gate, bool copyHist,
+                  const uint8_t *d_frames, const uint8_t *d_sigma6, hipStream_t stream)
     {
         const int a = blocks[k], blen = blocks[k + 1] - blocks[k];
-        const int first = B.used, n = (int)list.size();
-        if (blen <= 0 || n == 0)
-            return first;
-        if (first + n > B.slots)
+        if (first < 0 || first + n > B.slots)
             throw std::runtime_error("RunPipeline: a frame block was requested twice for one stack");
         const size_t j0 = (size_t)first * blen;
         for (int q = 0; q < n; ++q)
@@ -758,21 +797,40 @@
             fe.deferred = true;
             fe.pieceOff = B.pieceUsed;
             B.pieceUsed += pcap;
-            check(abub_diff_hist_chained_deferred_dev(d_frames, d_sigma6, dj, nj, W, H, dh, blen, chainStride,
-                                                      B.pieces + fe.pieceOff, (uint32_t)pcap, B.pcount + B.fetches.size(),
-                                                      B.inc.d + j0, stream),
-                  "trigger search K2 (deferred pieces)");
+            if (gate)
+                check(abub_diff_hist_chained_gated_dev(d_frames, d_sigma6, dj, nj, W, H, dh, blen, chainStride,
+                                                       B.pieces + fe.pieceOff, (uint32_t)pcap, B.pcount + B.fetches.size(),
+                                                       B.inc.d + j0, gate, stream),
+                      "trigger search K2 (gated)");
+            else
+                check(abub_diff_hist_chained_deferred_dev(d_frames, d_sigma6, dj, nj, W, H, dh, blen, chainStride,
+                                                          B.pieces + fe.pieceOff, (uint32_t)pcap, B.pcount + B.fetches.size(),
+                                                          B.inc.d + j0, stream),
+                      "trigger search K2 (deferred pieces)");
             B.inc.toHost(nj, stream, j0);
         } else {
+            if (gate)
+                throw std::runtime_error("RunPipeline: a gated frame block needs the deferred pieces");
             check(chainStride > 0 ? abub_diff_hist_chained_dev(d_frames, d_sigma6, dj, nj, W, H, dh, blen, chainStride, stream)
                                   : abub_diff_hist_dev(d_frames, d_sigma6, dj, nj, W, H, dh, nullptr, 0, stream),
                   "trigger search K2");
         }
-        B.hist.toHost((size_t)nj * 256, stream, j0 * 256);
+        if (copyHist)
+            B.hist.toHost((size_t)nj * 256, stream, j0 * 256);
         B.fetches.push_back(fe);
-        B.used = first + n;
-        stats.jobsLaunched += nj;
-        return first;
+        if (!gate)
+            stats.jobsLaunched += nj;
+        return (int)B.fetches.size() - 1;
+    }
+    bool chainable(const Group &G) const
+    {
+        const int nB = (int)blocks.size() - 1, ns = G.s1 - G.s0;
+        if (!trigOn || !chain || nB < 2 || F <= 1 || !deferPieces || !abub_k2_gated_ok(W, H))
+            return false;
+        for (int k = 1; k < nB; ++k)
+            if (abub_k2_pieces_cap(ns * (blocks[k + 1] - blocks[k]), W, H) > G.blocks[k].pieceCap)
+                return false;
+        return true;
     }
 
     RunPipeline(int device_, int W_, int H_, int F_, int E_, int C_, const int *tss_, int nthreads_, const char *maskdir)
@@ -794,6 +852,8 @@
         contours = ect ? atoi(ect) != 0 : 0;
         const char *etr = getenv("ABUB_PIPE_TRIGGER");
         trigger = etr ? atoi(etr) != 0 : 0;
+        const char *ech = getenv("ABUB_PIPE_CHAIN");
+        chain = ech ? atoi(ech) != 0 : 0;
         int trigMaxSegs = 0;
         check(abub_trigger_search_limits(&trigMaxF, &trigMaxSegs), "abub_trigger_search_limits");
         if (trigMaxSegs < BatchEventData::MAXB)
@@ -849,6 +909,9 @@
                 B.inc.allocate(nj);
                 B.want.allocate(nj);
             }
+            G.gate.allocate((size_t)std::max(nB, 1) * ns);
+            G.evalMask.allocate(ns);
+            G.trigSlot.allocate(ns);
             G.jobs3.allocate(n3);
             G.hist3.allocate(n3 * 256);
             G.img.allocate(abub_fast_path(W) ? 256 : n3 * P);
@@ -918,20 +981,57 @@
             std::vector<int> all;
             for (int sI = G.s0; sI < G.s1; ++sI)
                 all.push_back(sI);
+            G.chained = false;
+            std::vector<int> dev;
+            for (int sI : all)
+                if (trigOn && !trigHostRoute(sI))
+                    dev.push_back(sI);
+            const bool chainIt = !dev.empty() && chainable(G);
+            hipStream_t s1 = stage1Stream.get();
             if (F > 1)
-                launchBlock(G.blocks[0], 0, all, d_frames, d_sigma6, stage1Stream.get());
+                launchRun(G, G.blocks[0], 0, all.data(), (int)all.size(), 0, nullptr, !chainIt || dev.size() != all.size(), d_frames,
+                          d_sigma6, s1);
+            G.blocks[0].used = (int)all.size();
             if (trigOn) {
                 G.trig.inflight = false;
-                std::vector<int> dev;
-                for (int sI : all)
-                    if (!trigHostRoute(sI)) {
-                        if (F > 1)
-                            bindBlockDevice(G.blocks[0], 0, stacks[sI], 0, sI - G.s0);
-                        dev.push_back(sI);
+                for (int sI : dev)
+                    if (F > 1)
+                        bindBlockDevice(G.blocks[0], 0, stacks[sI], 0, sI - G.s0);
+            }
+            if (chainIt) {
+                const int nB = (int)blocks.size() - 1, ns = G.s1 - G.s0;
+                HIPOK(hipMemsetAsync(G.gate, 0, (size_t)nB * ns, s1));
+                HIPOK(hipMemsetAsync(G.evalMask.d, 0, (size_t)ns * sizeof(uint32_t), s1));
+                for (size_t q = 0; q < dev.size(); ++q)
+                    G.trigSlot.h[q] = (uint32_t)(dev[q] - G.s0);
+                G.trigSlot.toDevice(dev.size(), s1);
+                for (int k = 1; k < nB; ++k) {
+                    Group::Block &B = G.blocks[k];
+                    B.fetches.push_back(Group::Fetch());
+                    B.fetches[0].first = 0;
+                    B.fetches[0].n = ns;
+                    B.fetches[0].deferred = true;
+                    for (int sI : dev) {
+                        bindBlockDevice(B, k, stacks[sI], 0, sI - G.s0);
+                        stacks[sI].dvalid[k] = G.gate + (size_t)k * ns + (sI - G.s0);
                     }
-                launchSearch(G, dev, stage1Stream.get());
-            }
-            HIPOK(hipEventRecord(G.stage1Done.get(), stage1Stream.get()));
+                    B.fetches.clear();
+                }
+                for (int k = 1; k < nB; ++k) {
+                    launchSearch(G, dev, s1, k == 1, false);
+                    check(abub_trigger_gate_dev(G.trig.res.d, G.trigSlot.d, (int)dev.size(), blocks[k], blocks[k + 1] - blocks[k],
+                                                G.gate + (size_t)k * ns, G.evalMask.d, k, s1),
+                          "trigger search gate");
+                    launchRun(G, G.blocks[k], k, all.data(), ns, 0, G.gate + (size_t)k * ns, false, d_frames, d_sigma6, s1);
+                    G.blocks[k].used = ns;
+                    ++stats.chainBlocks;
+                }
+                launchSearch(G, dev, s1, false, true);
+                G.evalMask.toHost((size_t)ns, s1);
+                G.chained = true;
+            } else if (trigOn)
+                launchSearch(G, dev, s1);
+            HIPOK(hipEventRecord(G.stage1Done.get(), s1));
         }
         std::vector<std::thread> th;
         for (int g = 1; g < ngroups; ++g)
@@ -1048,6 +1148,27 @@
         });
         HIPOK(hipEventSynchronize(G.stage1Done.get()));
         G.stats.stage1Ms = nowMs() - t0;
+        if (G.chained) {
+            long long jobs = 0;
+            for (int q = 0; q < ns; ++q) {
+                StackState &st_ = stacks[G.s0 + q];
+                for (int k = 1; k < (int)blocks.size() - 1; ++k) {
+                    if (!st_.dvalid[k])
+                        continue;
+                    st_.dvalid[k] = nullptr;
+                    if (G.evalMask.h[q] >> k & 1u) {
+                        bindBlock(G.blocks[k], k, st_, 0, q);
+                        jobs += blocks[k + 1] - blocks[k];
+                        ++G.stats.chainEvaluated;
+                    } else {
+                        st_.dbh[k] = nullptr;
+                        st_.dinc[k] = nullptr;
+                    }
+                }
+            }
+            std::lock_guard<std::mutex> lock(launchMu);
+            stats.jobsLaunched += jobs;
+        }
 
         std::vector<int> pending(ns);
         for (int k = 0; k < ns; ++k)
@@ -1133,17 +1254,17 @@
                 v[(size_t)d.fetchOf[d.needBlock]].push_back(sI);
             }
         }
-        std::vector<int> newFetch((size_t)nB, -1);
+        std::vector<std::vector<std::pair<int, int>>> where((size_t)nB);
+        ++G.stats.fetchRounds;
         {
             std::lock_guard<std::mutex> lock(launchMu);
             for (int k = 0; k < nB; ++k) {
                 Group::Block &B = G.blocks[k];
                 if (!byBlock[k].empty()) {
-                    launchBlock(B, k, byBlock[k], d_frames, d_sigma6, stream);
-                    newFetch[k] = (int)B.fetches.size() - 1;
+                    launchBlock(G, B, k, byBlock[k], d_frames, d_sigma6, stream, &where[k]);
                     if (trigOn)
                         for (size_t q = 0; q < byBlock[k].size(); ++q)
-                            bindBlockDevice(B, k, stacks[byBlock[k][q]], newFetch[k], (int)q);
+                            bindBlockDevice(B, k, stacks[byBlock[k][q]], where[k][q].first, where[k][q].second);
                 }
                 const size_t blen = (size_t)(blocks[k + 1] - blocks[k]);
                 for (size_t f = 0; f < byFetch[k].size(); ++f) {
@@ -1187,7 +1308,7 @@
         for (int k = 0; k < nB; ++k) {
             for (size_t q = 0; q < byBlock[k].size(); ++q) {
                 StackState &st_ = stacks[byBlock[k][q]];
-                bindBlock(G.blocks[k], k, st_, newFetch[k], (int)q);
+                bindBlock(G.blocks[k], k, st_, where[k][q].first, where[k][q].second);
                 st_.needMore = false;
             }
             const size_t blen = (size_t)(blocks[k + 1] - blocks[k]);
@@ -1892,7 +2013,7 @@
 int abh_pipe_set_option(void *p, const char *name, int value)
 {
     const std::string opt = name ? name : "";
-    if (opt != "blobs" && opt != "contours" && opt != "trigger") {
+    if (opt != "blobs" && opt != "contours" && opt != "trigger" && opt != "chain") {
         g_pipeErr = std::string("abh_pipe_set_option: unknown option ") + (name ? name : "(null)");
         return -1;
     }
@@ -1905,7 +2026,7 @@
         return -1;
     }
     abub::RunPipeline *rp = (abub::RunPipeline *)p;
-    (opt == "blobs" ? rp->blobs : opt == "contours" ? rp->contours : rp->trigger) = value;
+    (opt == "blobs" ? rp->blobs : opt == "contours" ? rp->contours : opt == "chain" ? rp->chain : rp->trigger) = value;
     return 0;
 }
 
@@ -1915,6 +2036,14 @@
     const double v[6] = {(double)st.trigDevStacks, (double)st.trigHostStacks, (double)st.trigLaunches, (double)st.trigNeedFrames,
                          (double)st.trigNeedFinal, st.trigK6Ms};
     std::memcpy(out, v, sizeof v);
+}
+
+void abh_pipe_chain_stats(void *p, double *out)
+{
+    const abub::PipeStats &st = ((abub::RunPipeline *)p)->stats;
+    out[0] = (double)st.chainBlocks;
+    out[1] = (double)st.chainEvaluated;
+    out[2] = (double)st.fetchRounds;
 }
 
 void abh_pipe_trigger_totals(double *out)
diff --git a/include/abub_hip.h b/include/abub_hip.h
--- a/include/abub_hip.h
+++ b/include/abub_hip.h
@@ -59,6 +59,10 @@
                                      int H, uint32_t *hist, uint8_t *diff, int chain_len, int chain_stride, void *stream);
 
 size_t abub_k2_pieces_cap(int njobs, int W, int H);
+int abub_diff_hist_chained_gated_dev(const uint8_t *frames, const uint8_t *sigma6, const abub_job *jobs, int njobs, int W,
+                                     int H, uint32_t *hist, int chain_len, int chain_stride, void *pieces,
+                                     uint32_t pieces_cap, uint32_t *npieces, uint8_t *incomplete, const uint8_t *run,
+                                     void *stream);
 int abub_diff_hist_chained_deferred_dev(const uint8_t *frames, const uint8_t *sigma6, const abub_job *jobs, int njobs, int W,
                                         int H, uint32_t *hist, int chain_len, int chain_stride, void *pieces,
                                         uint32_t pieces_cap, uint32_t *npieces, uint8_t *incomplete, void *stream);
@@ -68,6 +72,7 @@
 int abub_k2_set_option(const char *name, int value);
 
 int abub_k2_deferred_ok(int W, int H);
+int abub_k2_gated_ok(int W, int H);
 
 int abub_k3_set_option(const char *name, int value);
 
@@ -144,6 +149,11 @@
 int abub_trigger_search_dev(const abub_trig_stack *stacks, const abub_trig_seg *segs, int nstacks, int nsegs, int W, int H,
                             void *desc, size_t desc_bytes, abub_trig_result *out, double *sig_main, int sig_pitch,
                             void *stream);
+int abub_trigger_search_gated_dev(const abub_trig_stack *stacks, const abub_trig_seg *segs, const uint8_t *const *valid,
+                                  int nstacks, int nsegs, int W, int H, void *desc, size_t desc_bytes, abub_trig_result *out,
+                                  double *sig_main, int sig_pitch, void *stream);
+int abub_trigger_gate_dev(const abub_trig_result *res, const uint32_t *slot, int nstacks, int first, int count, uint8_t *run,
+                          uint32_t *evaluated, int bit, void *stream);
 int abub_trigger_clear_pending_dev(uint8_t *pending, const uint8_t *done, size_t n, void *stream);
 size_t abub_trigger_search_desc_bytes(int nstacks, int nsegs);
 int abub_trigger_search_limits(int *max_frames, int *max_segs);
```
